# SayanoAI/Comfy-RVC

Measured on AMD Instinct MI355X. Metric: audio-sec/wall-sec (xRT), 40k_v2 end-to-end VC, higher is better.
Workload: dtype f32; 1 GPU; Full VC 40k_v2 (HuBERT -> RMVPE -> SynthesizerTrnMs768NSFsid), 30 s 16 kHz clips, 12 per GPU per step (3 in flight), vc_single host array in -> int16 host array out (BASELINE.json configs[2]); clips_in_flight_per_gpu=3, weights=procedural (comfy-rvc_amd/synthetic.py), noise=device generator, seeded per clip, parallelism=clip-per-GPU x1 (3 lanes each), one RCCL gather of the step's int16 waveforms

## Files before the change

comfy-rvc_amd/_lib.py:

```python
import ctypes as C
import os

_HERE = os.path.dirname(os.path.abspath(__file__))
LIB_PATH = os.environ.get("RVC_HIP_LIB") or os.path.join(_HERE, "csrc", "librvc_hip.so")


class RvcHipError(RuntimeError):
    pass


def _load():
    if not os.path.isfile(LIB_PATH):
        raise RvcHipError(
            f"{LIB_PATH} is missing: build it with `python -c 'import __graft_entry__ as g; g.build()'` "
            "(or `make -C comfy-rvc_amd/csrc`).  There is no CPU fallback.")
    return C.CDLL(LIB_PATH)


lib = _load()

c_void_p, c_int, c_int64, c_float, c_char_p = C.c_void_p, C.c_int, C.c_int64, C.c_float, C.c_char_p
P = C.POINTER


# ... 147 lines not shown
    "rvc_synth_infer_window_halo": (c_int, [c_void_p, c_void_p, c_void_p, c_int, c_void_p, c_void_p, c_int, c_void_p, c_void_p, c_int64,
                                            c_void_p, P(SynthTaps), c_int64, c_int64, c_int]),
    "rvc_vc_segment_window": (c_int, [c_void_p, c_void_p, c_void_p, c_void_p, c_int64, c_int, c_void_p, c_void_p, c_int, c_float, c_int,
                                      c_void_p, c_void_p, c_void_p, c_int64, c_int64]),
    "rvc_vc_segment_feats_window": (c_int, [c_void_p, c_void_p, c_void_p, c_void_p, c_int64, c_int, c_void_p, c_void_p, c_int, c_float, c_int, c_void_p,
                                            c_void_p, c_void_p, c_int64, c_int64]),
    "rvc_vc_segment": (c_int, [c_void_p, c_void_p, c_void_p, c_void_p, c_int64, c_int, c_void_p, c_void_p, c_int, c_float, c_int,
                               c_void_p, c_void_p, c_void_p]),
    "rvc_vc_segment_feats": (c_int, [c_void_p, c_void_p, c_void_p, c_void_p, c_int64, c_int, c_void_p, c_void_p, c_int, c_float, c_int, c_void_p,
                                     c_void_p, c_void_p]),
    "rvc_index_create": (c_int, [c_void_p, c_void_p, c_int64, c_int, P(c_void_p)]),
    "rvc_index_create_ivf": (c_int, [c_void_p, c_void_p, c_int64, c_int, c_void_p, c_int, c_void_p, c_int, P(c_void_p)]),
    "rvc_index_nprobe": (c_int, [c_void_p]),
    "rvc_index_destroy": (c_int, [c_void_p]),
    "rvc_index_ntotal": (c_int64, [c_void_p]),
    "rvc_index_search": (c_int, [c_void_p, c_void_p, c_void_p, c_int64, c_void_p, c_void_p]),
    "rvc_index_blend": (c_int, [c_void_p, c_void_p, c_void_p, c_void_p, c_int64, c_float, c_void_p]),
    "rvc_kmeans_assign": (c_int, [c_void_p, c_void_p, c_void_p, c_int64, c_int, c_void_p, c_int, c_void_p, c_void_p]),
    "rvc_kmeans_update": (c_int, [c_void_p, c_void_p, c_void_p, c_int64, c_int, c_int, c_void_p, c_void_p]),
    "rvc_index_train": (c_int, [c_void_p, c_void_p, c_void_p, c_int64, c_int, c_void_p, c_int, c_int, c_void_p, c_void_p, c_void_p]),
    "rvc_preprocess": (c_int, [c_void_p, c_void_p, c_int, c_int64, c_void_p, c_void_p, c_void_p, c_int, c_void_p, c_void_p,
                             c_void_p, c_int, c_void_p, c_void_p]),
    "rvc_postprocess": (c_int, [c_void_p, c_void_p, c_int64, c_void_p, c_int, c_int, c_float, c_void_p]),
    "rvc_lfilter_hp": (c_int, [c_void_p, c_void_p, c_int, c_int64, c_void_p, c_void_p]),
    "rvc_frame_rms": (c_int, [c_void_p, c_void_p, c_int64, c_int, c_int, c_void_p, c_int64]),
    "rvc_slice_tags": (c_int, [c_void_p, c_int64, c_int64, C.c_double, c_int64, c_int64, c_int64, c_void_p, c_int64, P(c_int64)]),
    "rvc_cut_windows": (c_int, [c_void_p, c_void_p, c_int64, c_void_p, c_int, c_int, c_int, c_void_p, c_int, c_int, c_int, c_float, c_void_p, c_int64,
                                c_void_p, c_int64]),
    "rvc_gate_levels": (c_int, [c_void_p, c_void_p, c_int64, c_int, c_void_p, c_int64]),
    "rvc_gate_ranges": (c_int, [c_void_p, c_int64, c_int64, c_int64, c_int64, c_int64, C.c_double, c_void_p, c_int64, P(c_int64)]),
    "rvc_gate_apply": (c_int, [c_void_p, c_void_p, c_void_p, c_int64, c_void_p, c_int, c_int64]),
    "rvc_declick": (c_int, [c_void_p, c_void_p, c_int64, c_int, c_float, c_int, c_int, c_int, c_void_p, c_void_p]),
    "rvc_peak_normalize": (c_int, [c_void_p, c_void_p, c_int64, c_float, c_void_p]),
    "rvc_peak_limit": (c_int, [c_void_p, c_void_p, c_int64, c_float]),
    "rvc_merge_tracks": (c_int, [c_void_p, P(c_void_p), P(c_int64), c_int, c_int, c_void_p, c_int64]),
    "rvc_segment_energy": (c_int, [c_void_p, c_void_p, c_int64, c_int, c_void_p]),
    "rvc_spectrogram_batch": (c_int, [c_void_p, c_void_p, c_void_p, c_int64, c_void_p, c_int, c_int, c_int, c_float, c_int, c_void_p, c_int64]),
    "rvc_mel_filterbank_set": (c_int, [c_void_p, c_int, c_int, c_void_p, c_void_p, c_void_p]),
    "rvc_spec_to_mel_batch": (c_int, [c_void_p, c_void_p, c_void_p, c_int64, c_void_p, c_int, c_int, c_int, c_void_p, c_int64]),
    "rvc_spectrogram_batch_ms": (c_int, [c_void_p, c_void_p, c_void_p, c_int64, c_void_p, c_int, c_int, c_int, c_float, c_int, c_void_p, c_int64]),
    "rvc_mel_spectrogram_vjp": (c_int, [c_void_p, c_void_p, c_void_p, c_int64, c_void_p, c_int, c_int, c_int, c_float, c_int, c_int, c_void_p, c_int64,
                                        c_void_p]),
    "rvc_mel_spectrogram_vjp_launch_count": (c_int, []),
    "rvc_mel_loss_cotangents": (c_int, [c_void_p, c_int, P(c_void_p), P(c_void_p), P(c_int64), c_int, c_float, c_float, P(c_float), P(c_void_p)]),
    "rvc_multiscale_mel_loss": (c_int, [c_void_p, c_void_p, c_int, P(c_void_p), P(c_int64), P(c_int64), c_int, c_int64, P(C.c_int32), P(C.c_int32), c_int, c_int,
                                        c_void_p]),
    "rvc_hpss": (c_int, [c_void_p, c_void_p, c_int, c_int, c_int, c_void_p, c_void_p, c_int]),
    "rvc_hpss_l1": (c_int, [c_void_p, c_void_p, c_void_p, c_int, c_int, c_int, c_float, c_void_p]),
    "rvc_tsi_terms": (c_int, [c_void_p, c_void_p, c_void_p, c_int, c_int, c_int, c_float, c_void_p]),
    "rvc_op_gemm_split": (c_int, [c_void_p] * 7 + [c_int] * 4 + [c_float, c_int, c_float] + [c_int] * 5),
    "rvc_op_conv2d_split": (c_int, [c_void_p] * 7 + [c_int] * 9),
    "rvc_op_wn_in_gate_split": (c_int, [c_void_p] * 6 + [c_int] * 4),
    "rvc_op_gemm_split_qkv": (c_int, [c_void_p] * 6 + [c_int] * 4),
    "rvc_op_conv1d_s2_split": (c_int, [c_void_p] * 6 + [c_int] * 5),
    "rvc_op_conv1d_split": (c_int, [c_void_p] * 6 + [c_int] * 9),
    "rvc_op_conv1d": (c_int, [c_void_p, c_void_p, c_void_p, c_void_p, c_void_p, c_void_p] + [c_int] * 8 +
                      [c_int, c_float, c_int, c_float, c_int, c_float, c_int]),
    "rvc_op_conv_transpose1d": (c_int, [c_void_p, c_void_p, c_void_p, c_void_p, c_void_p] + [c_int] * 6 + [c_int, c_float, c_int]),
    "rvc_op_conv2d3x3": (c_int, [c_void_p, c_void_p, c_void_p, c_void_p, c_void_p, c_void_p] + [c_int] * 5),
    "rvc_op_conv_transpose2d": (c_int, [c_void_p, c_void_p, c_void_p, c_void_p, c_void_p] + [c_int] * 5),
    "rvc_op_gemm_tn": (c_int, [c_void_p, c_void_p, c_void_p, c_void_p] + [c_int] * 4),
    "rvc_conv1d_plan_create": (c_int, [c_void_p, c_void_p] + [c_int] * 7 + [P(c_void_p)]),
    "rvc_conv1d_plan_run": (c_int, [c_void_p, c_void_p, c_void_p, c_int, c_void_p, c_void_p, c_int, c_float, c_int, c_float]),
    "rvc_conv1d_plan_pair_run": (c_int, [c_void_p, c_void_p, c_void_p, c_void_p, c_int, c_void_p, c_float, c_int]),
    "rvc_conv1d_plan_resblock_run": (c_int, [P(c_void_p), c_void_p, c_void_p, c_int, c_void_p, c_float, c_int, P(c_int), c_void_p, c_void_p, c_void_p]),
    "rvc_conv1d_plan_pair_split_run": (c_int, [c_void_p, c_void_p, c_void_p, c_void_p, c_int, c_void_p, c_float, c_int]),
    "rvc_conv1d_plan_destroy": (c_int, [c_void_p]),
    "rvc_op_attention": (c_int, [c_void_p, c_void_p, c_void_p, c_void_p, c_void_p, c_void_p, c_int, c_int]),
    "rvc_op_attention_split": (c_int, [c_void_p] * 7 + [c_int, c_int]),
    "rvc_op_attention_split_rel": (c_int, [c_void_p] * 9 + [c_int, c_int, c_int]),
    "rvc_op_cbr2_small": (c_int, [c_void_p] * 7 + [c_int, c_int, c_int]),
    "rvc_op_layernorm_c_split": (c_int, [c_void_p] * 6 + [c_int, c_int]),
    "rvc_op_conv3_small": (c_int, [c_void_p] * 7 + [c_int] * 6),
    "rvc_op_gemm_split_swapped": (c_int, [c_void_p] * 4 + [c_int] * 5),
    "rvc_op_conv2d3x3_plus_1x1": (c_int, [c_void_p] * 7 + [c_int] * 6),
    "rvc_op_gemm_split_swapped_res": (c_int, [c_void_p] * 5 + [c_int] * 5),
    "rvc_op_attention_rel": (c_int, [c_void_p] * 8 + [c_int, c_int, c_void_p, c_void_p]),
    "rvc_op_layernorm_c": (c_int, [c_void_p] * 6 + [c_int, c_int]),
    "rvc_resample": (c_int, [c_void_p, c_void_p, c_int64, c_void_p, c_int, c_int, c_int, c_void_p, c_int64]),
    "rvc_set_conv_precision": (c_int, [c_int]),
    "rvc_set_pair_arithmetic": (c_int, [c_int]),
    "rvc_get_pair_arithmetic": (c_int, []),
    "rvc_conv1d_plan_pair_arithmetic": (c_int, [c_void_p, c_void_p, c_int]),
    "rvc_prof_dump_csv": (c_int, [c_char_p]),
    "rvc_prof_enable": (c_int, [c_int]),
    "rvc_prof_collect": (c_int, [P(C.c_double), P(C.c_double), P(c_int64)]),
    "rvc_prof_collect_ex": (c_int, [P(C.c_double), C.c_double, C.c_double]),
    "rvc_prof_cfg_name": (c_char_p, [c_int]),
    "rvc_op_disc_conv": (c_int, [c_void_p] * 5 + [c_int] * 8 + [c_float, P(c_int)]),
    "rvc_op_disc_conv_plan": (c_int, [c_int] * 8 + [P(c_int)]),
    "rvc_op_disc_conv_input_grad": (c_int, [c_void_p] * 6 + [c_int] * 7 + [c_float, P(c_int)]),
    "rvc_op_disc_conv_input_grad_plan": (c_int, [c_int] * 7 + [P(c_int)]),
    "rvc_op_disc_conv_weight_grad": (c_int, [c_void_p] * 4 + [c_int] * 8 + [P(c_int)]),
    "rvc_op_disc_conv_weight_grad_plan": (c_int, [c_int] * 8 + [P(c_int)]),
    "rvc_op_conv1d_input_grad": (c_int, [c_void_p] * 6 + [c_int] * 6 + [c_int64] * 4 + [c_float, c_float, c_int, P(c_int), P(c_int)]),
    "rvc_op_conv1d_input_grad_plan": (c_int, [c_int] * 6 + [c_int64, c_int64, P(c_int)]),
    "rvc_op_sine_source": (c_int, [c_void_p] * 5 + [c_int, c_int, c_float, c_float, c_float] + [c_void_p] * 3),
    "rvc_op_hubert_conv0": (c_int, [c_void_p, c_void_p, c_int64, c_void_p, c_void_p, c_void_p, c_int, c_int, c_void_p, c_void_p, c_int64]),
    "rvc_op_conv_to1": (c_int, [c_void_p, c_void_p, c_int64, c_void_p, c_int, c_int, c_int, c_int, c_float, c_int, c_void_p, P(c_int)]),
    "rvc_op_noise_add": (c_int, [c_void_p, c_void_p, c_int64, c_int, c_int, c_void_p, c_int64, c_int, c_int, c_int, c_void_p, c_void_p, P(c_int)]),
    "rvc_op_transpose": (c_int, [c_void_p, c_void_p, c_void_p, c_int, c_int, c_int64, c_int64, c_int, c_int64, c_int64]),
    "rvc_op_frames": (c_int, [c_void_p, c_void_p, c_void_p] + [c_int] * 6),
    "rvc_op_mel_to_unet": (c_int, [c_void_p, c_void_p, c_void_p, c_int, c_int, c_float, c_float]),
    "rvc_op_feats_prepare": (c_int, [c_void_p] * 5 + [c_int, c_int, c_int, c_float, c_int]),
    "rvc_op_wn_gate": (c_int, [c_void_p] * 5 + [c_int, c_int]),
    "rvc_op_pool2_pad": (c_int, [c_void_p, c_void_p, c_int64, c_int, c_int, c_int, c_int, c_void_p, c_void_p, c_int64]),
    "rvc_op_interleave2_pad": (c_int, [c_void_p, c_void_p, c_int64, c_int, c_int, c_int, c_void_p, c_int, c_void_p, c_int64]),
    "rvc_op_pad2d": (c_int, [c_void_p, c_void_p, c_int64, c_int, c_int, c_int, c_void_p, c_void_p, c_int64]),
    "rvc_op_unpad2d": (c_int, [c_void_p, c_void_p, c_int64, c_int, c_int, c_int, c_void_p, c_int64]),
    "rvc_op_gru_scan": (c_int, [c_void_p] * 6 + [c_int, P(c_int)]),
}

EXPERIMENT_SIGNATURES = {
    "rvc_debug_conv_timing": (c_int, [P(C.c_uint64), c_int]),
    "rvc_debug_x3p_check": (c_int, []),
    "rvc_debug_gemm_split_bench": (c_int, [c_void_p] + [c_int] * 8 + [P(c_float), c_int, c_int]),
}

for _name, (_res, _args) in SIGNATURES.items():
    _fn = getattr(lib, _name)
    _fn.restype = _res
    _fn.argtypes = _args
has_experiments = all(hasattr(lib, _n) for _n in EXPERIMENT_SIGNATURES)
if has_experiments:
    for _name, (_res, _args) in EXPERIMENT_SIGNATURES.items():
        _fn = getattr(lib, _name)
        _fn.restype = _res
        _fn.argtypes = _args


def require_experiments():
    if not has_experiments:
        raise RuntimeError(f"{LIB_PATH} is the product library: the rvc_debug_* hooks exist in -DRVC_EXPERIMENTS builds only - "
                           "bash tools/build_variant.sh exp && RVC_HIP_LIB=comfy-rvc_amd/csrc/variants/librvc_hip_exp.so python <tool>")


def check(status):
    if status != 0:
        raise RvcHipError(lib.rvc_last_error().decode("utf-8", "replace"))


def ptr(t):
    if t is None:
        return None
    if hasattr(t, "data_ptr"):
        return c_void_p(t.data_ptr())
    return c_void_p(t.ctypes.data)


class _DeviceSpan:

    def __init__(self, address, shape):
        self.__cuda_array_interface__ = {"shape": tuple(int(v) for v in shape), "typestr": "<f4", "data": (int(address), False), "version": 2, "strides": None}


def device_view(address, shape, device):
    import torch
    with torch.cuda.device(device):
        return torch.as_tensor(_DeviceSpan(address, shape), device=device).clone()


def current_stream():
    import torch
    return c_void_p(torch.cuda.current_stream().cuda_stream)


# ... 27 lines not shown
```

comfy-rvc_amd/csrc/conv_kernels.h:

```cpp
#pragma once
#include "rvc_internal.h"
#include <hip/hip_ext.h>

namespace rvc {

typedef float f32x16 __attribute__((ext_vector_type(16)));
typedef unsigned int u32x4 __attribute__((ext_vector_type(4)));

struct ConvArgsX : ConvArgs {
  long long ldW;
  int Wcols;
  int Wrows;
  int ksplit; float* partial; long long ldP;
  unsigned magRP, magPW;
  int ni; unsigned magNI;
  const unsigned char* Wx; int CoPx; int xbufs; int NC; int kreal; long long wxBatch;
  const unsigned char* Wx2; const float* bias1; int fuse_p2; float fuse_slope;
  const unsigned char* Xs; long long xsTp;
  unsigned char* Ys; long long ysTp; float ys_slope;
  int wbufs;
  int xcd_remap;
  int h2;
};

__device__ __forceinline__ __amdgpu_buffer_rsrc_t make_rsrc(const void* base, unsigned bytes) {
  return __builtin_amdgcn_make_buffer_rsrc(const_cast<void*>(base), 0, (int)bytes, 0x00020000);
}
constexpr unsigned kOOB = 0x80000000u;
__device__ __forceinline__ float buf_load(__amdgpu_buffer_rsrc_t r, unsigned voff, unsigned soff = 0) {
  return __uint_as_float(__builtin_amdgcn_raw_buffer_load_b32(r, (int)voff, (int)soff, 0));
}
__device__ __forceinline__ void buf_dma(__amdgpu_buffer_rsrc_t rs, unsigned char* lds_dst, int voffset, int soffset) {
  __builtin_amdgcn_raw_ptr_buffer_load_lds(rs, (__attribute__((address_space(3))) void*)lds_dst, 16, voffset, soffset, 0, 0);
}

template <int WM, int WN, int AM, int AN, int G, bool HAS_R, bool HAS_ACC>
__device__ __forceinline__ void dense_epilogue_t(const ConvArgsX& p, f32x16 (&acc)[AM][AN], int z, int co0, int n0, int wm, int wn, int li, int lh) {
  const float* __restrict__ bias = p.bias ? p.bias + (long long)z * p.bBatch : nullptr;
  const float* R = HAS_R ? p.R + (long long)z * p.rBatch : nullptr;
  float* Y = p.Y + (long long)z * p.yBatch;
  const float lslope = p.act == ACT_NONE ? 1.f : (p.act == ACT_RELU ? 0.f : p.act_slope);
  const float oscale = p.out_scale;
  const bool plain = p.orows == p.Co;
  const __amdgpu_buffer_rsrc_t yrs = make_rsrc(Y, (unsigned)p.orows * (unsigned)p.ldY * 4u);
  const __amdgpu_buffer_rsrc_t rrs = make_rsrc(HAS_R ? R : Y, HAS_R ? (unsigned)p.orows * (unsigned)p.ldR * 4u : 0u);
  const bool abr = p.act_before_res != 0;
  constexpr bool need_loads = HAS_R || HAS_ACC;
  auto row_info = [&](int am, int r, bool& mok, float& bv, unsigned& yrow, unsigned& rrow) {
    const int m = co0 + (wm * AM + am) * 32 + (r & 3) + 8 * (r >> 2) + 4 * lh;
    mok = m < p.Co;
    const int co = plain ? m : m % p.orows;
    bv = (bias && mok) ? bias[co] : 0.f;
    yrow = (unsigned)co * (unsigned)p.ldY; rrow = (unsigned)co * (unsigned)p.ldR;
  };
  static_assert(16 % G == 0, "group size");
#pragma unroll
  for (int am = 0; am < AM; ++am) {
    float rv[G][AN], yv[G][AN], rvn[G][AN], yvn[G][AN];
#pragma unroll
    for (int j = 0; j < G; ++j)
#pragma unroll
      for (int an = 0; an < AN; ++an) { rv[j][an] = 0.f; yv[j][an] = 0.f; rvn[j][an] = 0.f; yvn[j][an] = 0.f; }
    auto load_group = [&](int r0, float (&rr)[G][AN], float (&yy)[G][AN]) {
#pragma unroll
      for (int j = 0; j < G; ++j) {
        bool mok; float bv; unsigned yrow, rrow;
        row_info(am, r0 + j, mok, bv, yrow, rrow);
#pragma unroll
        for (int an = 0; an < AN; ++an) {
          const int n = n0 + (wn * AN + an) * 32 + li;
          const bool ok = mok && n < p.Tout;
          if constexpr (HAS_R) rr[j][an] = buf_load(rrs, ok ? (rrow + (unsigned)n) * 4u : kOOB);
          if constexpr (HAS_ACC) yy[j][an] = buf_load(yrs, ok ? (yrow + (unsigned)n) * 4u : kOOB);
        }
      }
    };
    if constexpr (need_loads) load_group(0, rv, yv);
#pragma unroll
    for (int r0 = 0; r0 < 16; r0 += G) {
      if constexpr (need_loads) { if (r0 + G < 16) load_group(r0 + G, rvn, yvn); }
#pragma unroll
      for (int j = 0; j < G; ++j) {
        bool mok; float bv; unsigned yrow, rrow;
        row_info(am, r0 + j, mok, bv, yrow, rrow);
#pragma unroll
        for (int an = 0; an < AN; ++an) {
          const int n = n0 + (wn * AN + an) * 32 + li;
          const bool ok = mok && n < p.Tout;
          float v = acc[am][an][r0 + j] + bv;
          if (abr) v = fmaxf(v, v * lslope) + rv[j][an];
          else { v += rv[j][an]; v = fmaxf(v, v * lslope); }
          v = v * oscale + yv[j][an];
          __builtin_amdgcn_raw_buffer_store_b32(__float_as_uint(v), yrs, (int)(ok ? (yrow + (unsigned)n) * 4u : kOOB), 0, 0);
        }
      }
#pragma unroll
      for (int j = 0; j < G; ++j)
#pragma unroll
        for (int an = 0; an < AN; ++an) { rv[j][an] = rvn[j][an]; yv[j][an] = yvn[j][an]; }
    }
  }
}
template <int WM, int WN, int AM, int AN, int G = 1>
__device__ __forceinline__ void dense_epilogue(const ConvArgsX& p, f32x16 (&acc)[AM][AN], int z, int co0, int n0, int wm, int wn, int li, int lh) {
  const bool has_r = p.R != nullptr, has_acc = p.accumulate != 0;
  if (has_r && has_acc) dense_epilogue_t<WM, WN, AM, AN, G, true, true>(p, acc, z, co0, n0, wm, wn, li, lh);
  else if (has_r) dense_epilogue_t<WM, WN, AM, AN, (AM * AN >= 8 ? 2 * G : G) <= 16 ? (AM * AN >= 8 ? 2 * G : G) : 16, true, false>(p, acc, z, co0, n0, wm, wn, li, lh);
  else if (has_acc) dense_epilogue_t<WM, WN, AM, AN, G, false, true>(p, acc, z, co0, n0, wm, wn, li, lh);
  else dense_epilogue_t<WM, WN, AM, AN, G, false, false>(p, acc, z, co0, n0, wm, wn, li, lh);
}

struct TileCfg { int WM, WN, AM, AN; };
TileCfg choose_tile(int M, long long N, int batch);
int tile_cfg_id(const TileCfg& t);

constexpr int kProfCfgs = 24;
struct ProfTicket { hipEvent_t a = nullptr, b = nullptr; bool on = false; };
ProfTicket conv_prof_begin(hipStream_t s);
struct ProfKernelEvents { hipEvent_t ka = nullptr, kb = nullptr; bool armed = false; int launches = 0; };
ProfKernelEvents& prof_kernel_events();
template <class K, class A>
inline void conv_launch(K kern, dim3 grid, dim3 block, size_t lds, hipStream_t s, const A& a) {
  ProfKernelEvents& pe = prof_kernel_events();
  if (pe.armed && pe.launches++ == 0) hipExtLaunchKernelGGL(kern, grid, block, lds, s, pe.ka, pe.kb, 0, a);
  else hipLaunchKernelGGL(kern, grid, block, lds, s, a);
}
void conv_prof_end(ProfTicket& t, hipStream_t s, double flops, int cfg, double bytes = 0.0, const ConvArgsX* shape = nullptr, long long blocks = 0,
                   int fused = 0);
int conv_prof_dump_csv(const char* path);
double conv_alg_bytes(const ConvArgsX& a, int batch);
int conv_prof_collect_ex(double* out , double ridge_fp32, double ridge_x3);

void splitk_reduce_launch(const ConvArgsX& a, int S, int batch, hipStream_t s);

int device_cu_count();
inline int x3_xcd_remap() { static const int v = exp_int("RVC_X3_XCD", 1); return v; }
typedef void (*ConvLaunchFn)(const ConvArgsX&, dim3, size_t, hipStream_t);
struct ConvPlan {
  ConvArgsX a;
  long long plan_T = 0;
  ConvLaunchFn launch = nullptr;
  dim3 grid; size_t lds = 0;
  int prof_cfg = 0, prof_fused = 0;
  double alg_bytes = 0.0, flops = 0.0;
};
bool conv_x3_plan(const ConvArgsX& a0, int batch, long long Tplan, ConvPlan& p);
void conv_plan_launch(const ConvPlan& p, hipStream_t s);
bool conv_x3p_plan(ConvPlan& p, int AM, int AN);
int conv_x3p_check_read();
bool conv_x3q_plan(ConvPlan& p, int AM, int AN);
bool conv_x3g_plan(ConvPlan& p);
bool conv_x3pf_plan(ConvPlan& p);
bool conv_rbh_plan(ConvPlan& p);
bool conv_x3_pair_plan(const ConvLayer& c1, const ConvLayer& c2, const float* X, long long ldX, int T, long long Tplan, float* Y, long long ldY,
                       const ConvEpilogue& e2, int h2, ConvPlan& p);

struct Rb3Args {
  const float* X; long long ldX; float* Y; long long ldY;
  const unsigned char* W[6];
  const float* B[6];
  int CoPx;
  int T, halo, NO;
  float pre_slope, mid_slope, out_scale;
  const float* nsrc; const float* nw; const float* nb;
};
struct Rb3Plan {
  Rb3Args a; void (*launch)(const Rb3Args&, dim3, size_t, hipStream_t) = nullptr; dim3 grid; size_t lds = 0;
  int C = 0, k = 0, accumulate = 0;
};
bool conv_rb3_plan(const ConvLayer* const* c1, const ConvLayer* const* c2, const float* X, long long ldX, int T, long long Tplan, float* Y, long long ldY,
                   float pre_slope, float out_scale, int accumulate, int h2, const float* nsrc, const float* nw, const float* nb, Rb3Plan& p);
void conv_rb3_launch(const Rb3Plan& p, hipStream_t s);

}
```

comfy-rvc_amd/csrc/conv_mfma.hip:

```cpp
#include "conv_kernels.h"
#include "phase_timing.h"
#include <atomic>
#include <tuple>

#ifndef RVC_EPI_TWOPHASE
#define RVC_EPI_TWOPHASE 0
#endif

namespace rvc {

RVC_PHASE_TABLE_REGISTER;

constexpr int kWSlots = 32;
__host__ __device__ constexpr int x_slots(int BN, int MODE) {
  return MODE == 2 ? (BN >= 512 ? 26 : (BN >= 256 ? 18 : 14)) : (BN >= 512 ? 36 : (BN >= 256 ? 20 : (BN >= 128 ? 32 : 16)));
}

template <int WM, int WN, int AM, int AN, int MODE>
__global__ __launch_bounds__(256) void conv_mfma_kernel(const ConvArgsX p) {
  constexpr int BM = WM * AM * 32, BN = WN * AN * 32;
  constexpr int XS = x_slots(BN, MODE);
  extern __shared__ __attribute__((aligned(16))) float smem[];
  const int CK = p.CK, WROW = p.WROW;
  float* Xs = smem;
// ... 271 lines not shown
  int blocks = (int)((n + 255) / 256); if (blocks > 8192) blocks = 8192;
  hipLaunchKernelGGL(act_res_kernel, dim3(blocks), dim3(256), 0, s, y, r, rows, T, ldY, ldR, act, slope, act_before_res);
}

__global__ void splitk_reduce_kernel(const float* __restrict__ P, int S, int batch, int M, int N, long long ldP, const float* __restrict__ bias, int bBatch,
                                     const float* __restrict__ R, long long ldR, long long rBatch, float* __restrict__ Y, long long ldY, long long yBatch,
                                     int orows, float lslope, int abr, float oscale, int accumulate) {
  const long long total = (long long)batch * M * N;
  long long i = (long long)blockIdx.x * blockDim.x + threadIdx.x;
  const long long st = (long long)gridDim.x * blockDim.x;
  for (; i < total; i += st) {
    const int n = (int)(i % N); const long long t = i / N; const int m = (int)(t % M); const int z = (int)(t / M);
    float v = 0.f;
    for (int k = 0; k < S; ++k) v += P[(((long long)z * S + k) * M + m) * ldP + n];
    const int co = m % orows;
    if (bias) v += bias[(long long)z * bBatch + co];
    const float rv = R ? R[(long long)z * rBatch + (long long)co * ldR + n] : 0.f;
    if (abr) v = fmaxf(v, v * lslope) + rv; else { v += rv; v = fmaxf(v, v * lslope); }
    const long long o = (long long)z * yBatch + (long long)co * ldY + n;
    v *= oscale;
    if (accumulate) v += Y[o];
    Y[o] = v;
  }
}

void splitk_reduce_launch(const ConvArgsX& a, int S, int batch, hipStream_t s) {
  const long long total = (long long)batch * a.Co * a.Tout;
  int blocks = (int)((total + 255) / 256); if (blocks > 4096) blocks = 4096;
  const float lslope = a.act == ACT_NONE ? 1.f : (a.act == ACT_RELU ? 0.f : a.act_slope);
  { ProfKernelEvents& pe = prof_kernel_events(); if (pe.armed) ++pe.launches; }
  hipLaunchKernelGGL(splitk_reduce_kernel, dim3(blocks), dim3(256), 0, s, a.partial, S, batch, a.Co, a.Tout, a.ldP, a.bias, a.bBatch, a.R, a.ldR,
                     a.rBatch, a.Y, a.ldY, a.yBatch, a.orows, lslope, a.act_before_res, a.out_scale, a.accumulate);
}

std::vector<PhaseTableReader>& phase_table_readers() { static std::vector<PhaseTableReader> v; return v; }
void conv_timing_read(unsigned long long* out8, bool reset) {
  for (int i = 0; i < 8; ++i) out8[i] = 0;
  for (PhaseTableReader read : phase_table_readers()) {
    unsigned long long t[8]; read(t, reset);
    for (int i = 0; i < 8; ++i) out8[i] += t[i];
  }
}
void* dev_alloc(size_t bytes) {
  void* d = nullptr;
  RVC_HIP_CHECK(hipMalloc(&d, bytes));
  return d;
}
void* dev_upload(const void* host, size_t bytes) {
  void* d = dev_alloc(bytes ? bytes : sizeof(float));
  if (bytes) {
    const hipError_t e = hipMemcpy(d, host, bytes, hipMemcpyHostToDevice);
    if (e != hipSuccess) { dev_free(d); RVC_HIP_CHECK(e); }
  }
  return d;
}
void dev_free(void* p) { if (p) (void)hipFree(p); }

namespace {
struct ScratchBuf { void* p = nullptr; size_t cap = 0; };
using ScratchKey = std::tuple<int, hipStream_t, int>;
std::map<ScratchKey, ScratchBuf>& scratch_pool() { static std::map<ScratchKey, ScratchBuf> pool; return pool; }
std::mutex& scratch_mu() { static std::mutex mu; return mu; }
struct Scratch { void* p; bool grew; };
Scratch scratch_get(hipStream_t s, int slot, size_t bytes, size_t grow_to) {
  int dev = 0;
  RVC_HIP_CHECK(hipGetDevice(&dev));
  ScratchBuf* b;
  { std::lock_guard<std::mutex> lk(scratch_mu()); b = &scratch_pool()[ScratchKey{dev, s, slot}]; }
  if (bytes <= b->cap) return {b->p, false};
  RVC_HIP_CHECK(hipStreamSynchronize(s));
  if (b->p) (void)hipFree(b->p);
  b->p = nullptr; b->cap = 0;
  RVC_HIP_CHECK(hipMalloc(&b->p, grow_to));
  b->cap = grow_to;
  return {b->p, true};
}
}
void* stream_scratch(hipStream_t s, int slot, size_t bytes) { return scratch_get(s, slot, bytes, bytes + bytes / 4 + (1 << 20)).p; }
void* stream_scratch_zeroed(hipStream_t s, int slot, size_t bytes, bool* fresh) {
  const Scratch r = scratch_get(s, slot, bytes, bytes);
  if (r.grew) RVC_HIP_CHECK(hipMemsetAsync(r.p, 0, bytes, s));
  if (fresh) *fresh = r.grew;
  return r.p;
}
void stream_scratch_release(int device) {
  std::lock_guard<std::mutex> lk(scratch_mu());
  auto& pool = scratch_pool();
  for (auto it = pool.begin(); it != pool.end();) {
    if (std::get<0>(it->first) == device) { if (it->second.p) (void)hipFree(it->second.p); it = pool.erase(it); } else ++it;
  }
}

void Arena::ensure(size_t bytes) {
  if (bytes <= cap) return;
  if (base) { RVC_HIP_CHECK(hipDeviceSynchronize()); (void)hipFree(base); base = nullptr; cap = 0; }
  size_t want = bytes + bytes / 8 + (1 << 20);
  RVC_HIP_CHECK(hipMalloc(&base, want));
  cap = want; ++gen;
}
void Arena::release() { if (base) (void)hipFree(base); base = nullptr; cap = 0; ++gen; }

static int pick_ck(int V, int ktaps, int stride) {
  int ck = ktaps >= 4 ? 8 : (ktaps >= 2 ? 16 : 64);
  if (stride > 1) { ck = ((ck + stride - 1) / stride) * stride; if (ck & 1) ck *= 2; }
  if (V < ck) { ck = stride > 1 ? ((V + stride - 1) / stride) * stride : V; if (ck & 1) ck += (stride > 1 ? stride : 1); if (ck < 2) ck = 2; }
  return ck;
}

static void upload_layer(ConvLayer& L, const std::vector<float>& packed, const float* bias, int nbias) {
  L.Wd_ = dev_upload(packed.data(), packed.size());
  L.bd_ = bias ? dev_upload(bias, nbias) : nullptr;
}

static uint16_t bf16_rne(float f) {
  uint32_t u; memcpy(&u, &f, 4);
  if ((u & 0x7fffffffu) > 0x7f800000u) return (uint16_t)((u >> 16) | 0x40);
  return (uint16_t)((u + 0x7fffu + ((u >> 16) & 1u)) >> 16);
}
static float bf16_to_f32(uint16_t h) { uint32_t u = (uint32_t)h << 16; float f; memcpy(&f, &u, 4); return f; }
static thread_local bool g_x3_default = false;
static thread_local int g_precision = 1;
bool conv_x3_set_default(bool on) { const bool prev = g_x3_default; g_x3_default = on; return prev; }
int conv_set_precision(int mode) { const int prev = g_precision; if (mode >= 0) g_precision = mode; return prev; }
static void pack_x3_grouped(ConvLayer& L, const float* w , int groups, int Cog, int Cig, int k) {
  L.CoPx = (Cog + 63) & ~63;
  const int nch = Cig / 16;
  L.wxBatch = (long long)nch * k * 2 * L.CoPx * 16;
  std::vector<uint16_t> P((size_t)groups * L.wxBatch, 0);
  for (int g = 0; g < groups; ++g)
    for (int co = 0; co < Cog; ++co)
      for (int ci = 0; ci < Cig; ++ci)
        for (int u = 0; u < k; ++u) {
          const float v = w[((size_t)(g * Cog + co) * Cig + ci) * k + u];
          const uint16_t hi = bf16_rne(v), lo = bf16_rne(v - bf16_to_f32(hi));
          const int chunk = ci >> 4, c16 = ci & 15;
          const size_t base = (((size_t)chunk * k + u) * 2 * 2 + (size_t)(c16 >> 3)) * L.CoPx + co;
          uint16_t* Q = P.data() + (size_t)g * L.wxBatch;
          Q[base * 8 + (c16 & 7)] = hi;
          Q[(base + 2 * (size_t)L.CoPx) * 8 + (c16 & 7)] = lo;
        }
  RVC_HIP_CHECK(hipMalloc(&L.Wx_, P.size() * sizeof(uint16_t)));
  RVC_HIP_CHECK(hipMemcpy(L.Wx_, P.data(), P.size() * sizeof(uint16_t), hipMemcpyHostToDevice));
}
void x3_weight_image(const float* w, int Co, int Ci, int k, int CoPx, std::vector<uint16_t>& P) {
  P.assign((size_t)(Ci / 16) * k * 2 * CoPx * 16, 0);
  for (int co = 0; co < Co; ++co)
    for (int ci = 0; ci < Ci; ++ci)
      for (int u = 0; u < k; ++u) {
        const float v = w[((size_t)co * Ci + ci) * k + u];
        const uint16_t hi = bf16_rne(v), lo = bf16_rne(v - bf16_to_f32(hi));
        const int chunk = ci >> 4, c16 = ci & 15;
        const size_t base = (((size_t)chunk * k + u) * 2 * 2 + (size_t)(c16 >> 3)) * CoPx + co;
        P[base * 8 + (c16 & 7)] = hi;
        P[(base + 2 * (size_t)CoPx) * 8 + (c16 & 7)] = lo;
      }
}
static void pack_x3(ConvLayer& L, const float* w, int Co, int Ci, int k) {
  L.CoPx = (Co + 127) & ~127;
  const int nch = Ci / 16;
  L.wxBatch = (long long)nch * k * 2 * L.CoPx * 16;
  std::vector<uint16_t> P;
  x3_weight_image(w, Co, Ci, k, L.CoPx, P);
  RVC_HIP_CHECK(hipMalloc(&L.Wx_, P.size() * sizeof(uint16_t)));
  RVC_HIP_CHECK(hipMemcpy(L.Wx_, P.data(), P.size() * sizeof(uint16_t), hipMemcpyHostToDevice));
}

// ... 389 lines not shown
      const long long total = (long long)batch * a.Co * a.Tout;
      (void)total;
      splitk_reduce_launch(a, S, batch, s);
    }
    conv_prof_end(rec, s, flops, cfg_id, conv_alg_bytes(a, batch), &a, (long long)grid.x * grid.y * grid.z);
  };
#define RVC_LAUNCH(ID_, WM_, WN_, AM_, AN_)                                                     \
  if (t.WM == WM_ && t.WN == WN_ && t.AM == AM_ && t.AN == AN_) {                               \
    cfg_id = ID_ + (mode == 2 ? 7 : 0);                                                         \
    rec = conv_prof_begin(s);                                                                   \
    if (mode == 2) launch_cfg<WM_, WN_, AM_, AN_, 2>(a, grid, lds, s);                          \
    else if (a.stride > 1) launch_cfg<WM_, WN_, AM_, AN_, 3>(a, grid, lds, s);                  \
    else launch_cfg<WM_, WN_, AM_, AN_, 1>(a, grid, lds, s);                                    \
    finish();                                                                                   \
    return;                                                                                     \
  }
  RVC_LAUNCH(0, 1, 4, 1, 4)
  RVC_LAUNCH(1, 1, 4, 1, 2)
  RVC_LAUNCH(2, 1, 4, 1, 1)
  RVC_LAUNCH(3, 2, 2, 2, 2)
  RVC_LAUNCH(4, 2, 2, 1, 4)
  RVC_LAUNCH(5, 2, 2, 1, 2)
  RVC_LAUNCH(6, 2, 2, 1, 1)
#undef RVC_LAUNCH
  throw Error("no tile configuration matched");
}

static bool simple_act(int act) { return act == ACT_NONE || act == ACT_LRELU || act == ACT_RELU; }
static ConvEpilogue split_epilogue(const ConvEpilogue& e, bool& post) {
  post = !simple_act(e.act);
  if (!post) return e;
  RVC_REQUIRE(e.out_scale == 1.f && !e.accumulate, "GELU/tanh/sigmoid/log epilogues do not combine with scale/accumulate");
  ConvEpilogue c = e;
  c.act = ACT_NONE; c.act_slope = 0.f; c.R = nullptr; c.ldR = 0;
  return c;
}
static void fill_epilogue(ConvArgsX& a, const ConvEpilogue& e) {
  a.R = e.R; a.ldR = e.ldR; a.pre_act = e.pre_act; a.pre_slope = e.pre_slope; a.act = e.act; a.act_slope = e.act_slope;
  a.act_before_res = e.act_before_res; a.out_scale = e.out_scale; a.accumulate = e.accumulate;
  a.Xs = e.xs_in; a.xsTp = e.xs_tp; a.Ys = e.ys_out; a.ysTp = e.ys_tp; a.ys_slope = e.ys_slope;
}

int conv1d_out_len(const ConvLayer& L, int Tin) {
  if (L.tconv_u > 0) return (Tin - 1) * L.tconv_u - 2 * L.pad + L.k;
  return (Tin + 2 * L.pad - L.dil * (L.k - 1) - 1) / L.stride + 1;
}

void conv1d_run(const ConvLayer& L, hipStream_t s, const float* X, long long ldX, int Tin, float* Y, long long ldY,
                const ConvEpilogue& e0) {
  RVC_REQUIRE(L.mode == 1 && L.Wd_, "conv1d_run on an uninitialised / non-1D layer");
  bool post; const ConvEpilogue e = split_epilogue(e0, post);
  ConvArgsX a{};
  a.X = X; a.W = L.Wd_; a.bias = L.bd_; a.Y = Y;
  fill_epilogue(a, e);
  a.Ci = L.Ci; a.Co = L.Co; a.CoP = L.CoP; a.Tin = Tin; a.Wd = 0; a.ktaps = L.ktaps; a.dil = L.dil; a.stride = L.stride;
  a.CK = L.CK; a.nchunk = L.nchunk;
  a.ldX = ldX; a.ldY = ldY; a.up2 = 0;
  a.ldW = L.CoP; a.Wcols = L.CoP; a.Wrows = L.nchunk * L.ktaps * L.CK;
  if (e.bias_override) a.bias = e.bias_override;
  int Tout = conv1d_out_len(L, Tin);
  if (e.tout_limit > 0 && e.tout_limit < Tout) { RVC_REQUIRE(L.tconv_u == 0, "tout_limit on a transposed conv"); Tout = e.tout_limit; }
  auto gemm_cols = [&](int tout) { return L.tconv_u > 0 ? (tout + L.tconv_u - 1) / L.tconv_u : tout; };
  a.Tout = gemm_cols(Tout);
  RVC_REQUIRE(e.plan_tin == 0 || (e.plan_tin >= Tin && !e.tout_limit), "plan_tin is the input length of the whole sequence this launch is a column window of");
  const long long Tplan = e.plan_tin > 0 ? gemm_cols(conv1d_out_len(L, e.plan_tin)) : a.Tout;
  if (L.tconv_u > 0) {
    a.pad = L.conv_pad;
    a.ostride = L.tconv_u; a.orows = L.co_real;
    RVC_REQUIRE(ldY == Tout, "interleaved ConvTranspose1d store needs a dense output (ldY == Tout)");
    RVC_REQUIRE(e.R == nullptr, "residual not supported on the interleaved store");
  } else {
    a.pad = L.pad; a.ostride = 1; a.orows = L.Co;
  }
  a.xBatch = (long long)L.Ci * ldX; a.wBatch = L.wBatch; a.yBatch = (long long)L.Co * ldY; a.rBatch = (long long)L.Co * e.ldR;
  a.bBatch = L.Co;
  const double flops = L.tconv_u > 0 ? 2.0 * Tin * L.Ci * L.co_real * L.k
                                     : 2.0 * L.groups * (double)L.Co * a.Tout * L.Ci * L.k;
  a.Wx = reinterpret_cast<const unsigned char*>(L.Wx_); a.CoPx = L.CoPx; a.wxBatch = L.wxBatch; a.kreal = L.tconv_u > 0 ? L.ktaps : L.k;
  if (e.h2) {
    RVC_REQUIRE(L.Wh_ && (e.xs_in || e.ys_out), "fp16x2 arithmetic is for the two halves of a split-resident ResBlock pair (conv1d_pair_h2_eligible)");
    a.Wx = reinterpret_cast<const unsigned char*>(L.Wh_); a.h2 = 1;
  }
  ConvPlan p;
  if (L.Wx_ && conv_x3_plan(a, L.groups, Tplan, p)) { p.flops = flops; conv_plan_launch(p, s); }
  else {
    RVC_REQUIRE(!e.xs_in && !e.ys_out, "split-resident tensors need the bf16x3 kernel (check conv1d_split_eligible first)");
    run_conv(a, 1, L.groups, Tplan, s, flops);
  }
  if (post) {
    RVC_REQUIRE(L.tconv_u == 0, "post-activation on a transposed conv");
    act_res_inplace(s, Y, e0.R, L.groups * L.Co, Tout, ldY, e0.ldR, e0.act, e0.act_slope, e0.act_before_res);
  }
}

bool conv1d_pair_h2_eligible(const ConvLayer& c1, const ConvLayer& c2, int Tin, int h2) {
  if (!h2 || !c1.Wh_ || !c2.Wh_) return false;
  return conv1d_split_eligible(c1, Tin, SPLIT_PRODUCER, 1) && conv1d_split_eligible(c2, Tin, SPLIT_CONSUMER, 1);
}

static bool plan_split_role(const ConvLayer& L, int Tin, SplitRole role, int h2, ConvPlan& p) {
  if (L.mode != 1 || !L.Wx_ || (h2 && !L.Wh_) || L.tconv_u || L.stride != 1 || L.groups != 1 || (L.Co & 31) || (L.Ci & 15)) return false;
  if (conv1d_out_len(L, Tin) != Tin || L.pad > kSplitMargin) return false;
  ConvArgsX a{};
  a.Ci = L.Ci; a.Co = L.Co; a.CoP = L.CoP; a.Tin = Tin; a.Wd = 0; a.ktaps = L.ktaps; a.dil = L.dil; a.stride = 1; a.pad = L.pad;
  a.Tout = conv1d_out_len(L, Tin); a.ostride = 1; a.orows = L.Co; a.ldX = Tin; a.ldY = a.Tout; a.ldR = a.Tout;
  a.Wx = reinterpret_cast<const unsigned char*>(L.Wx_); a.CoPx = L.CoPx; a.kreal = L.k; a.h2 = h2;
  if (role == SPLIT_CONSUMER) a.R = reinterpret_cast<const float*>(L.Wx_);
  if (role == SPLIT_PRODUCER) { a.Ys = reinterpret_cast<unsigned char*>(L.Wx_); a.ysTp = split_image_tp(Tin); a.pre_act = ACT_LRELU; a.pre_slope = 0.1f; }
  else { a.Xs = reinterpret_cast<const unsigned char*>(L.Wx_); a.xsTp = split_image_tp(Tin); }
  return conv_x3_plan(a, 1, a.Tout, p);
}
bool conv1d_split_eligible(const ConvLayer& L, int Tin, SplitRole role, int h2) { ConvPlan p; return plan_split_role(L, Tin, role, h2, p); }

int conv1d_residual_period(const ConvLayer& L, int Tin, int h2) {
  ConvPlan p;
  if (!plan_split_role(L, Tin, SPLIT_CONSUMER, h2, p) || (p.prof_fused >> 4) != 6) return 1;
  const int id = p.prof_cfg - 14;
  return id == 3 ? 128 : 256;
}

void gemm_tn_run(hipStream_t s, const float* A, long long ldA, long long aBatch, const float* B, long long ldB, long long bBatch,
                 float* Y, long long ldY, long long yBatch, int M, int N, int K, int batch, const float* bias, int biasBatch,
                 const ConvEpilogue& e) {
  RVC_REQUIRE(simple_act(e.act), "gemm_tn_run supports identity / ReLU / leaky ReLU epilogues");
  ConvArgsX a{};
  a.X = B; a.W = A; a.bias = bias; a.Y = Y;
  fill_epilogue(a, e);
  a.Ci = K; a.Co = M; a.CoP = M; a.Tin = N; a.Tout = N; a.Wd = 0; a.ktaps = 1; a.dil = 1; a.stride = 1; a.pad = 0;
  a.CK = K >= 64 ? 64 : ((K + 1) & ~1); a.nchunk = (K + a.CK - 1) / a.CK;
  a.ldX = ldB; a.ldY = ldY; a.up2 = 0; a.ostride = 1; a.orows = M;
  a.ldW = ldA; a.Wcols = M; a.Wrows = K;
  a.xBatch = bBatch; a.wBatch = aBatch; a.yBatch = yBatch; a.rBatch = 0; a.bBatch = biasBatch;
  run_conv(a, 1, batch, N, s, 2.0 * M * (double)N * K * batch);
}

void conv2d_run(const ConvLayer& L, hipStream_t s, const float* X, long long ldX, int H, int Wd, float* Y, long long ldY,
                const ConvEpilogue& e) {
  RVC_REQUIRE(simple_act(e.act), "conv2d_run supports identity / ReLU / leaky ReLU epilogues");
  RVC_REQUIRE(L.mode == 2 && L.Wd_, "conv2d_run on an uninitialised / non-2D layer");
  RVC_REQUIRE((Wd & (Wd - 1)) == 0 && Wd >= 2, "width must be a power of two");
  ConvArgsX a{};
  a.X = X; a.W = L.Wd_; a.bias = L.bd_; a.Y = Y;
  fill_epilogue(a, e);
  a.Ci = L.Ci; a.Co = L.Co; a.CoP = L.CoP; a.Tin = H; a.Tout = H * Wd; a.Wd = Wd; a.ktaps = 9; a.dil = 1; a.stride = 1; a.pad = 1;
  a.CK = L.CK; a.nchunk = L.nchunk;
  a.ldX = ldX; a.ldY = ldY; a.up2 = L.up2; a.ostride = 1; a.orows = L.up2 ? L.co_real : L.Co;
  a.ldW = L.CoP; a.Wcols = L.CoP; a.Wrows = L.nchunk * 9 * L.CK;
  a.xBatch = 0; a.wBatch = 0; a.yBatch = 0; a.rBatch = 0; a.bBatch = 0;
  const double flops = 2.0 * H * (double)Wd * 9 * L.Ci * (L.up2 ? L.co_real : L.Co);
  a.Wx = reinterpret_cast<const unsigned char*>(L.Wx_); a.CoPx = L.CoPx; a.wxBatch = L.wxBatch; a.kreal = 9;
  if (L.up2 && L.Wx_ && !e.R && !e.accumulate) {
    ConvArgsX d = a;
    float* tmp = (float*)stream_scratch(s, 4, (size_t)L.Co * H * Wd * sizeof(float));
    d.Y = tmp; d.ldY = (long long)H * Wd; d.up2 = 0; d.orows = L.Co; d.bias = L.bd4_;
    ConvPlan p;
    if (conv_x3_plan(d, 1, d.Tout, p)) {
      p.flops = flops; conv_plan_launch(p, s);
      const long long n = (long long)L.Co * H * Wd;
      int blocks = (int)((n + 255) / 256); if (blocks > 8192) blocks = 8192;
      hipLaunchKernelGGL(interleave2x2_kernel, dim3(blocks), dim3(256), 0, s, tmp, Y, L.co_real, H, Wd);
      return;
    }
  }
  ConvPlan p;
  if (L.Wx_ && !L.up2 && conv_x3_plan(a, 1, a.Tout, p)) { p.flops = flops; conv_plan_launch(p, s); }
  else run_conv(a, 2, 1, a.Tout, s, flops);
}

}
```

comfy-rvc_amd/csrc/conv_x3.hip:

```cpp
#include "conv_x3_dev.h"

#ifndef RVC_X3_SCHED
#define RVC_X3_SCHED 0
#endif

namespace rvc {

RVC_PHASE_TABLE_REGISTER;

template <int WM, int WN, int AM, int AN, bool FUSE = false, bool XSPLIT = false, bool YSPLIT = false>
__global__ __launch_bounds__(WM * WN * 64, WM * WN == 8 ? 1 : ((WM == 2 && WN == 2 && AM == 2 && AN == 2 && !FUSE) ? 3 : 2)) void conv_x3_kernel(const ConvArgsX p) {
  constexpr int NW = WM * WN, NT = NW * 64;
  constexpr int BM = WM * AM * 32, BN = WN * AN * 32, XS = XSPLIT ? 1 : ((FUSE && BM == 64) ? 7 : (FUSE ? 5 : x3_slots(BN, NW))), RB = BM / 32;
  extern __shared__ __attribute__((aligned(1024))) unsigned char smem3[];
  const int P = p.WROW;
  const int NC = p.NC;
  const int st = p.stride;
  const int Pm = XSPLIT ? ((P + 63) & ~63) : (P + st - 1) / st;
  const int xplane = st * Pm * 32;
  const int xhalf = xplane >> 1;
  const int xbuf = NC * 2 * xplane;
  const int wbuf = NC * p.KT * 2 * BM * 32;
  unsigned char* Xs = smem3;
  unsigned char* Ws = smem3 + ((p.xbufs * xbuf + 1023) & ~1023);
// ... 324 lines not shown
    const __amdgpu_buffer_rsrc_t prs = make_rsrc(Pp, (unsigned)p.Co * (unsigned)p.ldP * 4u);
#pragma unroll
    for (int am = 0; am < AM; ++am)
#pragma unroll
      for (int r = 0; r < 16; ++r) {
        const int m = co0 + (wm * AM + am) * 32 + (r & 3) + 8 * (r >> 2) + 4 * lh;
#pragma unroll
        for (int an = 0; an < AN; ++an) {
          const int n = n0 + (wn * AN + an) * 32 + li;
          const bool ok = m < p.Co && n < p.Tout;
          __builtin_amdgcn_raw_buffer_store_b32(__float_as_uint(acc[am][an][r]), prs, (int)(ok ? ((unsigned)m * (unsigned)p.ldP + (unsigned)n) * 4u : kOOB), 0, 0);
        }
      }
  } else if (YSPLIT) {
    ysplit_epilogue<WM, WN, AM, AN>(p, acc, co0, n0, wm, wn, li, lh);
  } else if (p.ostride == 1) {
    if constexpr (FUSE) {
      ConvArgsX pe = p;
      pe.Tout = min(p.Tout, n0 + BN - 2 * P2);
      dense_epilogue<WM, WN, AM, AN, (AM * AN >= 8 ? 4 : 8)>(pe, acc, z, co0, n0, wm, wn, li, lh);
    } else {
      dense_epilogue<WM, WN, AM, AN, (AM * AN >= 8 ? (AN >= 8 ? 2 : 4) : (XSPLIT ? 4 : 8))>(p, acc, z, co0, n0, wm, wn, li, lh);
    }
  } else {
    const float* __restrict__ bias = p.bias;
    float* Y = p.Y;
    const float lslope = p.act == ACT_NONE ? 1.f : (p.act == ACT_RELU ? 0.f : p.act_slope);
#pragma unroll
    for (int am = 0; am < AM; ++am) {
#pragma unroll
      for (int r = 0; r < 16; ++r) {
        const int m = co0 + (wm * AM + am) * 32 + (r & 3) + 8 * (r >> 2) + 4 * lh;
        if (m >= p.Co) continue;
        const int co = m / p.ostride, ph = m - co * p.ostride;
        const float bv = bias ? bias[co] : 0.f;
#pragma unroll
        for (int an = 0; an < AN; ++an) {
          const int n = n0 + (wn * AN + an) * 32 + li;
          const long long to = (long long)n * p.ostride + ph;
          if (n >= p.Tout || to >= p.ldY) continue;
          const long long oidx = (long long)co * p.ldY + to;
          float v = acc[am][an][r] + bv;
          v = fmaxf(v, v * lslope) * p.out_scale;
          if (p.accumulate) v += Y[oidx];
          Y[oidx] = v;
        }
      }
    }
  }
  tm.lap(5); tm.add(0, 1); tm.flush();
}

template <int WM, int WN, int AM, int AN, bool FUSE = false, bool XSPLIT = false, bool YSPLIT = false>
static void launch_x3(const ConvArgsX& a, dim3 grid, size_t lds, hipStream_t s) {
  auto kern = conv_x3_kernel<WM, WN, AM, AN, FUSE, XSPLIT, YSPLIT>;
  RVC_ALLOW_BIG_LDS(kern);
  conv_launch(kern, grid, dim3(WM * WN * 64), lds, s, a);
}

template <int AM, int AN>
static ConvLaunchFn select_x3_io(const ConvArgsX& a) {
  if (a.Xs) return &launch_x3<2, 2, AM, AN, false, true>;
  if (a.Ys) return &launch_x3<2, 2, AM, AN, false, false, true>;
  return &launch_x3<2, 2, AM, AN>;
}
static ConvLaunchFn select_x3(const ConvArgsX& a, int id) {
  switch (id) {
    case 0: return &launch_x3<1, 4, 1, 4>;
    case 1: return &launch_x3<1, 4, 1, 2>;
    case 2: return &launch_x3<1, 4, 1, 1>;
    case 3: return select_x3_io<2, 2>(a);
    case 4: return select_x3_io<1, 4>(a);
    case 5: return &launch_x3<2, 2, 1, 2>;
    case 7: return select_x3_io<2, 4>(a);
    default: return &launch_x3<2, 2, 1, 1>;
  }
}

void conv_plan_launch(const ConvPlan& p, hipStream_t s) {
  ConvArgsX a = p.a;
  if (a.Xs) RVC_REQUIRE(a.xsTp >= split_image_tp(a.Tin), "split-resident input image is shorter than split_image_tp(T)");
  if (a.Ys) RVC_REQUIRE(a.ysTp >= split_image_tp(a.Tout), "split-resident output image is shorter than split_image_tp(T)");
  if (a.ksplit > 1) a.partial = (float*)stream_scratch(s, 0, (size_t)a.ksplit * a.Co * a.ldP * sizeof(float));
  ProfTicket tk = conv_prof_begin(s);
  p.launch(a, p.grid, p.lds, s);
  if (a.ksplit > 1) splitk_reduce_launch(a, a.ksplit, 1, s);
  conv_prof_end(tk, s, p.flops, p.prof_cfg, p.alg_bytes, &a, (long long)p.grid.x * p.grid.y * p.grid.z, p.prof_fused);
}

bool conv_x3_plan(const ConvArgsX& a0, int batch, long long Tplan, ConvPlan& p) {
  if (!a0.Wx) return false;
  const bool xs = a0.Xs != nullptr;
  if ((xs || a0.Ys) && (a0.Wd > 0 || a0.stride != 1 || a0.ostride != 1 || (a0.Co & 31) || batch != 1)) return false;
  if (xs && a0.pre_act != ACT_NONE) return false;
  if ((xs || a0.Ys) && (a0.pad > kSplitMargin || a0.Tout != a0.Tin)) return false;
  const int KH2 = a0.KW > 0 ? a0.KH : 3, KW2 = a0.KW > 0 ? a0.KW : 3;
  if (a0.Wd > 0 && (a0.ktaps != KH2 * KW2 || a0.stride != 1)) return false;
  if ((a0.stride != 1 && a0.dil != 1) || a0.up2 || (a0.ostride != 1 && a0.R) || (a0.Ci & 15) || batch != 1) return false;
  if (!(a0.act == ACT_NONE || a0.act == ACT_LRELU || a0.act == ACT_RELU) || !(a0.pre_act == ACT_NONE || a0.pre_act == ACT_LRELU)) return false;
  if ((double)a0.orows * (double)a0.ldY * 4.0 >= 2147483648.0 || (double)a0.orows * (double)a0.ldR * 4.0 >= 2147483648.0 ||
      (double)a0.Ci * (double)a0.ldX * 4.0 >= 2147483648.0) return false;
  p = ConvPlan{};
  p.plan_T = Tplan;
  ConvArgsX& a = p.a;
  a = a0;
  if (a.Wd == 0) a.ktaps = a0.kreal;
  auto planned = [&](int cfg, int fused) { p.prof_cfg = cfg; p.prof_fused = fused; p.alg_bytes = conv_alg_bytes(a, batch); return true; };
  if (batch == 1 && a.up2 == 0 && !a.h2) {
    if (conv_x3g_plan(p)) return planned(14 + ((a.Co > 64 && a.Ci * a.ktaps > 1024) ? 3 : 5), 2 << 4);
  }
  TileCfg t = choose_tile(a.Co, Tplan, batch);
  {
    static const int wide_blk = exp_int("RVC_X3_WIDE", 600);
    auto blocks = [&](int bm, int bn) { return (long long)((a.Co + bm - 1) / bm) * ((Tplan + bn - 1) / bn); };
    if (wide_blk > 0 && a.stride == 1 && a.Wd == 0) {
      static const int wide_xs7 = exp_int("RVC_X3_WIDE_XS7", 1);
      static const int wide_k3 = exp_int("RVC_X3_WIDE_K3", 2);
      if (a.Co > 64 && blocks(128, 256) >= wide_blk && (a.ktaps > 3 || (wide_k3 >= 1 && a.ostride == 1)) &&
          !(xs && a.ktaps <= 7 && !(a.ktaps <= 3 && wide_k3 >= 2) && !(a.ktaps == 7 && wide_xs7))) t = TileCfg{2, 2, 2, 4};
    }
  }
  int id = tile_cfg_id(t);
  if (t.WM == 2 && t.WN == 2 && t.AM == 2 && t.AN == 4) id = 7;
  const int NW = t.WM * t.WN;
  if (id < 0) return false;
  if ((xs || a0.Ys) && !(id == 3 || id == 4 || id == 7)) return false;
  if (xs && a0.Ys) return false;
  const int BM = t.WM * t.AM * 32, BN = t.WN * t.AN * 32;
  const long long nblk = ((Tplan + BN - 1) / BN) * ((a.Co + BM - 1) / BM);
  static const int min_blk = exp_int("RVC_X3_MINBLK", 250);
  static const int min_blk2d = exp_int("RVC_X3_MINBLK2D", 20);
  if (nblk < (a.Wd > 0 ? min_blk2d : min_blk)) return false;
  if (t.WM == 2 && t.WN == 2 && batch == 1) {
    const bool s2_up = a.stride == 2 && a.ktaps == 3 && a.Co >= 128 && !(t.AM == 2 && t.AN == 2) &&
                       (long long)((a.Co + 127) / 128) * ((Tplan + 127) / 128) >= 150;
    const int pam = s2_up ? 2 : t.AM, pan = s2_up ? 2 : t.AN;
    if (!s2_up && conv_x3q_plan(p, t.AM, t.AN)) return planned(14 + id, 6 << 4);
    if (a.h2) return false;
    if (conv_x3p_plan(p, pam, pan)) return planned(14 + (s2_up ? 3 : id), 1 << 4);
  }
  if (a.h2) return false;
  static const int x3_split_blk = exp_int("RVC_X3_SPLITK_BLK", 600);
  int P = (BN - 1) * a.stride + (a.ktaps - 1) * a.dil + 1;
  if (a.Wd > 0) {
    a.BWd = BN < a.Wd ? BN : a.Wd; a.BH = BN < a.Wd ? 1 : BN / a.Wd; a.PW = a.BWd + KW2 - 1;
    P = (a.BH + KH2 - 1) * a.PW;
    a.magPW = (unsigned)((0x100000000ULL + a.PW - 1) / a.PW);
  }
  const int Pm = xs ? ((P + 63) & ~63) : (P + a.stride - 1) / a.stride;
  a.ni = (P + 63) / 64;
  const int nchunk = a.Ci / 16;
  int NC = a.ktaps == 1 ? 4 : (a.ktaps <= 3 ? 2 : 1);
  while (NC > 1 && (nchunk % NC != 0 || (!xs && (NC * 2 * a.ni + NW - 1) / NW > x3_slots(BN, NW)))) NC >>= 1;
  if (!xs && (NC * 2 * a.ni + NW - 1) / NW > x3_slots(BN, NW)) return false;
  static const int budget_kb = exp_int("RVC_X3_LDS_KB", 53);
  const int budget = budget_kb * 1024;
  static const int wbufs_env = exp_int("RVC_X3_WBUFS", 2);
  int NS = wbufs_env < 2 ? 2 : (wbufs_env > 4 ? 4 : wbufs_env);
  int xbufs = 2, xbytes = 0, ktmax = 0;
  for (;;) {
    const int per_tap = NS * NC * 2 * BM * 32;
    xbufs = 2; xbytes = (xbufs * NC * 2 * a.stride * Pm * 32 + 1023) & ~1023;
    ktmax = (budget - xbytes) / per_tap;
    if (!xs && ktmax < 2 && a.ktaps > ktmax && a.ktaps > 1) { xbufs = 1; xbytes = (NC * 2 * a.stride * Pm * 32 + 1023) & ~1023; ktmax = (budget - xbytes) / per_tap; }
    if (ktmax >= 1) break;
    if (NS > 2) { --NS; continue; }
// ... 87 lines not shown
```

comfy-rvc_amd/csrc/conv_x3q.hip:

```cpp
#include "conv_x3_dev.h"

namespace rvc {

RVC_PHASE_TABLE_REGISTER;
RVC_X3P_CHECK_REGISTER;

struct QTile { int co0, n0, bx; bool edge, valid; };
template <bool SWAP, bool H2 = false>
__device__ __forceinline__ f32x16 q_mfma(const u32x4& w, const u32x4& x, const f32x16& c) {
  if constexpr (H2) return __builtin_amdgcn_mfma_f32_32x32x16_f16(__builtin_bit_cast(f16x8, w), __builtin_bit_cast(f16x8, x), c, 0, 0, 0);
  else if constexpr (SWAP) return __builtin_amdgcn_mfma_f32_32x32x16_bf16(__builtin_bit_cast(bf16x8, x), __builtin_bit_cast(bf16x8, w), c, 0, 0, 0);
  else return __builtin_amdgcn_mfma_f32_32x32x16_bf16(__builtin_bit_cast(bf16x8, w), __builtin_bit_cast(bf16x8, x), c, 0, 0, 0);
}
typedef float f32x4q __attribute__((ext_vector_type(4)));

template <int AM, int AN, int KT, int R, bool XSPLIT, bool YSPLIT, bool RADD, bool H2>
__global__ __launch_bounds__(256, (AM * AN >= 8) ? 2 : 3) void conv_x3q_kernel(const ConvArgsX p) {
  static_assert(!(YSPLIT && RADD), "an image output has no residual");
  static_assert(XSPLIT != YSPLIT, "c1 of a pair (fp32 in, image out) or c2 (image in, fp32 out)");
  constexpr int WM = 2, WN = 2, NW = 4;
  constexpr int BM = WM * AM * 32, BN = WN * AN * 32, RB = BM / 32;
  constexpr int XS = 3;
  constexpr int NPW = H2 ? 1 : 2 * RB / NW;
  constexpr int NPX = (BN + 64) / 64;
  constexpr int wslot = (H2 ? 1 : 2) * BM * 32;
  constexpr int NBLK = AM * AN;
  constexpr int TR = KT / 2;
  static_assert(KT >= XS && (RB == 2 || RB == 4), "geometry");
  struct Q {
    static constexpr int nA(int t) { return XSPLIT ? 0 : 8 * x3_cv(t, KT, XS); }
    static constexpr int nD(int t) { return (XSPLIT && tap_mod(t, KT) == KT - 1) ? NPX : 0; }
    static constexpr int nE(int t) { return (RADD && tap_mod(t, KT) == TR) ? 16 : 0; }
    static constexpr int tot(int t) { return nA(t) + NPW + nD(t) + nE(t); }
    static constexpr int sum() { int n = 0; for (int t = 0; t < KT; ++t) n += tot(t); return n; }
    static constexpr int w(int t) { int n = nD(t - (R - 2)) + nE(t - (R - 2)); for (int j = 1; j <= R - 3; ++j) n += tot(t - (R - 2) + j); return n + nA(t); }
  };
  constexpr int EP = (YSPLIT || RADD) ? 4 * AM * AN : 16 * AM * AN;

  extern __shared__ __attribute__((aligned(1024))) unsigned char smemq[];
  const int P = p.WROW;
  const int Pm = (P + 7) & ~7;
  const int xplane = Pm * 32, xhalf = xplane >> 1, xbuf = 2 * xplane;
  unsigned char* Xs = smemq;
  unsigned char* Ws = smemq + ((2 * xbuf + 1023) & ~1023);
  float* Bs = reinterpret_cast<float*>(Ws + R * wslot);
  unsigned char* Ss = reinterpret_cast<unsigned char*>(Bs) + ((p.Co * 4 + 255) & ~255);

  const int tid0 = threadIdx.x;
  int lane = tid0 & 63;
  const int wave = __builtin_amdgcn_readfirstlane(tid0 >> 6);
  const int wm = wave / WN, wn = wave % WN;
  const int li = lane & 31, lh = lane >> 5;
  const int nck = p.nchunk;
  const int ni = p.ni;
  const int dil16 = p.dil * 16;
  const float pre_slope = p.pre_act == ACT_LRELU ? p.pre_slope : 1.f;
  const __amdgpu_buffer_rsrc_t xrs = make_rsrc(p.X, XSPLIT ? 0u : (unsigned)p.Ci * (unsigned)p.ldX * 4u);
  const __amdgpu_buffer_rsrc_t rrs = make_rsrc(RADD ? (const void*)p.R : (const void*)p.Y, RADD ? (unsigned)p.Co * (unsigned)p.ldR * 4u : 0u);

  const unsigned nty = (unsigned)(p.Co / BM), ntiles = (unsigned)((p.Tout + BN - 1) / BN) * nty;
  auto geom = [&](int it) -> QTile {
    const unsigned L = blockIdx.x + (unsigned)it * gridDim.x;
    QTile t;
    t.valid = L < ntiles;
    const unsigned tile = !t.valid ? 0u : (p.xcd_remap ? xcd_tile(L, ntiles) : L);
    const int tx = (int)(tile / nty), ty = (int)(tile - (unsigned)tx * nty);
    t.co0 = ty * BM; t.n0 = tx * BN; t.bx = t.n0 - p.pad;
    t.edge = XSPLIT && (t.bx < 0 || t.bx + P > p.Tin);
    return t;
  };
  const int nit = (int)((ntiles - blockIdx.x + gridDim.x - 1) / gridDim.x);

  PhaseTimer<PhaseClock::cycle> tm;
#ifdef RVC_X3P_CHECK
  int issued = 0, mk_w[8] = {0, 0, 0, 0, 0, 0, 0, 0}, mk_x[XS] = {0, 0, 0}, mk_r = 0, uwc = 0, mk_xs[2] = {0, 0};
#endif

  for (int m = tid0; m < p.Co; m += NW * 64) Bs[m] = p.bias ? p.bias[m] : 0.f;

  const int NU = nck * KT;
  const unsigned wstep = (unsigned)p.CoPx * (H2 ? 32u : 64u);
  const __amdgpu_buffer_rsrc_t wrs = make_rsrc(p.Wx, (unsigned)NU * wstep);
  const int wrow_h2 = RB == 4 ? wave * 64 + lane : wave * 32 + (lane & 31);
  const int wvoff = H2 ? ((wrow_h2 / BM) * p.CoPx + (wrow_h2 % BM)) * 16
                       : ((wave / RB) * p.CoPx * 32) + (((((wave % RB) * 64 + lane) / BM) * p.CoPx + (((wave % RB) * 64 + lane) % BM)) * 16);
  QTile cur = geom(0), nxt = geom(1);
  unsigned wsoff = (unsigned)cur.co0 * 16u;
  int slw = 0, uw = 0;
  int wtile_co0_next = nxt.valid ? nxt.co0 : cur.co0;
  auto issue_w = [&]() {
    if constexpr (H2) {
      unsigned char* dst = Ws + slw * wslot + wave * (RB == 4 ? 1024 : 512);
      if (RB == 4 || lane < 32)
        buf_dma(wrs, dst, wvoff, (int)wsoff);
    } else {
      unsigned char* dst = Ws + slw * wslot + wave * 1024;
      buf_dma(wrs, dst, wvoff, (int)wsoff);
      if constexpr (RB == 4)
        buf_dma(wrs, dst + NW * 1024, wvoff, (int)(wsoff + (unsigned)p.CoPx * 32u));
    }
    ++uw;
    if (uw == NU) { uw = 0; wsoff = (unsigned)wtile_co0_next * 16u; } else wsoff += wstep;
    slw = slw + 1 == R ? 0 : slw + 1;
    X3P_ISSUED(NPW);
#ifdef RVC_X3P_CHECK
    mk_w[uwc & 7] = issued; ++uwc;
#endif
  };

  float xr[XS][8];
  auto slot_geom = [&](int s, int& hb, int& q) -> bool {
    const int t = wave + NW * s;
    hb = t >= ni ? 1 : 0;
    q = (t - hb * ni) * 64 + lane;
    return t < 2 * ni && q < P;
  };
  auto load_slot = [&](int s, const QTile& tl, int chunk) {
    int hb, q;
    const bool ok = slot_geom(s, hb, q) && tl.valid;
    const int x = tl.bx + q;
    const unsigned voff = (ok && x >= 0 && x < p.Tin) ? (unsigned)x * 4u : kOOB;
    const unsigned c0 = (unsigned)(chunk * 16 + hb * 8);
#pragma unroll
    for (int j = 0; j < 8; ++j) xr[s][j] = buf_load(xrs, voff, (c0 + j) * (unsigned)p.ldX * 4u);
    X3P_ISSUED(8);
#ifdef RVC_X3P_CHECK
    mk_x[s] = issued;
#endif
  };
  auto store_slot = [&](int s, int xb) {
    int hb, q;
    if (slot_geom(s, hb, q)) {
      u32x4 hi, lo;
#pragma unroll
      for (int j = 0; j < 4; ++j) {
        const float a = xr[s][2 * j], b = xr[s][2 * j + 1];
        unsigned h_, l_;
        if constexpr (H2) split2h(fmaxf(a, a * pre_slope), fmaxf(b, b * pre_slope), h_, l_);
        else split2(fmaxf(a, a * pre_slope), fmaxf(b, b * pre_slope), h_, l_);
        hi[j] = h_; lo[j] = l_;
      }
      unsigned char* d = Xs + xb * xbuf + hb * xhalf + q * 16;
      *reinterpret_cast<u32x4*>(d) = hi;
      *reinterpret_cast<u32x4*>(d + xplane) = lo;
    }
  };
  const __amdgpu_buffer_rsrc_t xsr = make_rsrc(XSPLIT ? (const void*)p.Xs : (const void*)p.Wx, XSPLIT ? (unsigned)((long long)(p.Ci / 16) * 4 * p.xsTp * 16) : 0u);
  auto issue_x = [&](const QTile& tl, int chunk, int xb) {
    constexpr int pph = (BN + 64) / 64;
#pragma unroll
    for (int i = 0; i < NPX; ++i) {
      const int pi = wave + NW * i;
      const int hp = pi / pph, j = pi - hp * pph;
      const unsigned row = (unsigned)((chunk * 4 + hp) * (int)p.xsTp + (tl.bx + kSplitMargin) + j * 64);
      unsigned char* dst = Xs + xb * xbuf + hp * xhalf + j * 1024;
      if (j * 64 + lane < Pm)
        buf_dma(xsr, dst, lane * 16, (int)(row * 16u));
    }
    X3P_ISSUED(NPX);
#ifdef RVC_X3P_CHECK
    mk_xs[xb] = issued;
#endif
  };
  auto zero_edges = [&](const QTile& tl, int xb) {
    for (int q = tid0; q < P; q += NW * 64) {
      const int t = tl.bx + q;
      if (t >= 0 && t < p.Tin) continue;
#pragma unroll
      for (int pl = 0; pl < 2; ++pl) {
        unsigned char* r = Xs + xb * xbuf + pl * xplane + q * 16;
        *reinterpret_cast<u32x4*>(r) = u32x4{0u, 0u, 0u, 0u}; *reinterpret_cast<u32x4*>(r + xhalf) = u32x4{0u, 0u, 0u, 0u};
      }
    }
  };
  float rst[16];
  auto load_res = [&](const QTile& tl, int b) {
    if constexpr (RADD) {
      const int am = b / AN, an = b - am * AN;
      const int n = tl.n0 + (wn * AN + an) * 32 + li;
      const int mb = tl.co0 + (wm * AM + am) * 32 + 4 * lh;
      const unsigned voff = (tl.valid && b < NBLK && n < p.Tout) ? ((unsigned)mb * (unsigned)p.ldR + (unsigned)n) * 4u : kOOB;
#pragma unroll
      for (int r = 0; r < 16; ++r) rst[r] = buf_load(rrs, voff, (unsigned)((r & 3) + 8 * (r >> 2)) * (unsigned)p.ldR * 4u);
      X3P_ISSUED(16);
#ifdef RVC_X3P_CHECK
      mk_r = issued;
#endif
    }
  };

  const int aoff = lh * (BM * 16) + ((wm * AM) * 32 + li) * 16;
  const int boff = lh * xhalf + ((wn * AN) * 32 + li) * 16;

  if constexpr (XSPLIT) {
    issue_x(cur, 0, 0);
    issue_x(cur, 1, 1);
  } else {
#pragma unroll
    for (int s = 0; s < XS; ++s) load_slot(s, cur, 0);
    wait_vmcnt<0>();
#pragma unroll
    for (int s = 0; s < XS; ++s) store_slot(s, 0);
#pragma unroll
    for (int s = 0; s < XS; ++s) load_slot(s, cur, 1);
  }
#pragma unroll
  for (int i = 0; i < R - 1; ++i) issue_w();
  load_res(cur, 0);
  wait_vmcnt<0>();
#pragma unroll
  for (int s = 0; s < XS; ++s)
#pragma unroll
    for (int j = 0; j < 8; ++j) asm volatile("" : "+v"(xr[s][j]));
  lds_barrier();
  if (XSPLIT && cur.edge) { zero_edges(cur, 0); lds_barrier(); }

  f32x16 acc[AM][AN];
  u32x4 ah[AM], al[AM], bh[AN], bl[AN];
  {
    const unsigned char* wa = Ws + aoff;
    const unsigned char* xa = Xs + boff;
#pragma unroll
    for (int am = 0; am < AM; ++am) ah[am] = *reinterpret_cast<const u32x4*>(wa + am * 512);
#pragma unroll
    for (int an = 0; an < AN; ++an) bl[an] = *reinterpret_cast<const u32x4*>(xa + xplane + an * 512);
  }

  int sl = 0, xb = 0;
  tm.lap(1);
  for (int it = 0; it < nit; ++it) {
#pragma unroll
    for (int am = 0; am < AM; ++am) {
      f32x4q bv[4];
#pragma unroll
      for (int g = 0; g < 4; ++g) bv[g] = RADD ? *reinterpret_cast<const f32x4q*>(Bs + cur.co0 + (wm * AM + am) * 32 + 4 * lh + 8 * g) : f32x4q{0.f, 0.f, 0.f, 0.f};
#pragma unroll
      for (int an = 0; an < AN; ++an)
#pragma unroll
        for (int r = 0; r < 16; ++r) acc[am][an][r] = bv[r >> 2][r & 3];
    }
    for (int c = 0; c < nck; ++c) {
      const bool c0 = c == 0;
      const bool in1 = c + 1 < nck, in2 = c + 2 < nck;
      const QTile& t1 = in1 ? cur : nxt;
      const QTile& t2 = in2 ? cur : nxt;
      const int ch2 = in2 ? c + 2 : c + 2 - nck;
      auto unit = [&](auto tc) {
        constexpr int T = decltype(tc)::value;
        constexpr bool last_tap = T + 1 == KT;
        {
          const unsigned char* xa = Xs + xb * xbuf + T * dil16 + boff;
#pragma unroll
          for (int an = 0; an < AN; ++an) bh[an] = *reinterpret_cast<const u32x4*>(xa + an * 512);
        }
        __builtin_amdgcn_sched_barrier(0);
#pragma unroll
        for (int am = 0; am < AM; ++am)
#pragma unroll
          for (int an = 0; an < AN; ++an)
            acc[am][an] = q_mfma<false, H2>(ah[am], bl[an], acc[am][an]);
        if constexpr (!H2) {
          const unsigned char* wa = Ws + sl * wslot + BM * 32 + aoff;
#pragma unroll
          for (int am = 0; am < AM; ++am) al[am] = *reinterpret_cast<const u32x4*>(wa + am * 512);
        }
        if constexpr (!XSPLIT) {
          auto stage = [&](auto sc) {
            constexpr int s = decltype(sc)::value;
            if constexpr ((s * KT) / XS == T) {
              constexpr int NS = Q::sum() - 8;
              if (c0) { if (it > 0) X3P_CHECK(vm6(NS + EP), issued - mk_x[s]); wait_vmcnt<vm6(NS + EP)>(); }
              else { X3P_CHECK(vm6(NS), issued - mk_x[s]); wait_vmcnt<vm6(NS)>(); }
              store_slot(s, xb ^ 1);
              load_slot(s, t2, ch2);
            }
          };
          static_for<0, XS>(stage);
        }
        __builtin_amdgcn_sched_barrier(0);
#pragma unroll
        for (int am = 0; am < AM; ++am)
#pragma unroll
          for (int an = 0; an < AN; ++an)
            acc[am][an] = q_mfma<false, H2>(ah[am], bh[an], acc[am][an]);
        __builtin_amdgcn_sched_barrier(0);
        {
          constexpr int NWT = Q::w(T);
#ifdef RVC_X3P_CHECK
          const int exact = issued - mk_w[(uwc - (R - 2)) & 7];
#endif
          tm.lap(2);
          if (c0 && T < R - 2) { if (it > 0) X3P_CHECK(vm6(NWT + EP), exact); wait_vmcnt<vm6(NWT + EP)>(); }
          else { X3P_CHECK(vm6(NWT), exact); wait_vmcnt<vm6(NWT)>(); }
          static_assert(!XSPLIT || R - 2 <= KT - 1, "weight ring deeper than a chunk: the input chunk's DMA would not be covered by the weight wait");
          if constexpr (XSPLIT && last_tap) { if (it > 0 || c > 0) X3P_CHECK(vm6(NWT), issued - mk_xs[xb ^ 1]); }
          tm.lap(3);
          lds_barrier();
          tm.lap(4);
          const int sn = sl + 1 == R ? 0 : sl + 1;
          if (XSPLIT && last_tap && t1.edge) { zero_edges(t1, xb ^ 1); lds_barrier(); }
          issue_w();
          if constexpr (XSPLIT && last_tap) issue_x(t2, ch2, xb);
          const unsigned char* wa = Ws + sn * wslot + aoff;
          const unsigned char* xa = Xs + (last_tap ? xb ^ 1 : xb) * xbuf + xplane + (last_tap ? 0 : (T + 1) * dil16) + boff;
#pragma unroll
          for (int am = 0; am < AM; ++am) ah[am] = *reinterpret_cast<const u32x4*>(wa + am * 512);
#pragma unroll
          for (int an = 0; an < AN; ++an) bl[an] = *reinterpret_cast<const u32x4*>(xa + an * 512);
          sl = sn;
        }
        if constexpr (RADD && T == TR) {
          constexpr int NR = Q::sum() - 16;
          if (c0) { if (it > 0) X3P_CHECK(vm6(NR + EP), issued - mk_r); wait_vmcnt<vm6(NR + EP)>(); }
          else { X3P_CHECK(vm6(NR), issued - mk_r); wait_vmcnt<vm6(NR)>(); }
          auto radd = [&](auto bc) {
            constexpr int b = decltype(bc)::value, am = b / AN, an = b % AN;
            f32x16& A = acc[am][an];
            float (&V)[16] = rst;
            const int cc = c;
#define X3Q_ADD8(o)                                                                                                                                   \
            asm volatile("s_cmp_lg_u32 %16, %17\n\ts_cbranch_scc1 .Lx3q_skip_%=\n\ts_nop 15\n\ts_nop 7\n\t"                                                 \
                         "v_add_f32 %0, %0, %8\n\tv_add_f32 %1, %1, %9\n\tv_add_f32 %2, %2, %10\n\tv_add_f32 %3, %3, %11\n\t"                              \
                         "v_add_f32 %4, %4, %12\n\tv_add_f32 %5, %5, %13\n\tv_add_f32 %6, %6, %14\n\tv_add_f32 %7, %7, %15\n\ts_nop 3\n.Lx3q_skip_%=:"      \
                         : "+v"(A[o + 0]), "+v"(A[o + 1]), "+v"(A[o + 2]), "+v"(A[o + 3]), "+v"(A[o + 4]), "+v"(A[o + 5]), "+v"(A[o + 6]), "+v"(A[o + 7])    \
                         : "v"(V[o + 0]), "v"(V[o + 1]), "v"(V[o + 2]), "v"(V[o + 3]), "v"(V[o + 4]), "v"(V[o + 5]), "v"(V[o + 6]), "v"(V[o + 7]),           \
                           "s"(cc), "n"(b) : "scc")
            X3Q_ADD8(0);
            X3Q_ADD8(8);
#undef X3Q_ADD8
          };
          static_for<0, NBLK>(radd);
          load_res(t1, in1 ? c + 1 : 0);
        }
        __builtin_amdgcn_sched_barrier(0);
        if constexpr (!H2) {
#pragma unroll
          for (int am = 0; am < AM; ++am)
#pragma unroll
            for (int an = 0; an < AN; ++an)
              acc[am][an] = q_mfma<false>(al[am], bh[an], acc[am][an]);
        }
      };
      static_for<0, KT>(unit);
      xb ^= 1;
    }

    tm.lap(2);
    if constexpr (YSPLIT) {
      const float sl2 = p.ys_slope;
      const __amdgpu_buffer_rsrc_t ysr = make_rsrc(p.Ys, (unsigned)((long long)(p.Co / 16) * 4 * p.ysTp * 16));
#pragma unroll
      for (int am = 0; am < AM; ++am)
#pragma unroll
        for (int an = 0; an < AN; ++an) {
          const int n = cur.n0 + (wn * AN + an) * 32 + li;
          const int mb = cur.co0 + (wm * AM + am) * 32;
          const long long pos = (long long)n + kSplitMargin;
#pragma unroll
          for (int g2 = 0; g2 < 2; ++g2) {
            const f32x4q ba = *reinterpret_cast<const f32x4q*>(Bs + mb + 16 * g2 + 4 * lh);
            const f32x4q bb = *reinterpret_cast<const f32x4q*>(Bs + mb + 16 * g2 + 4 * lh + 8);
            unsigned hA[2], lA[2], hB[2], lB[2];
#pragma unroll
            for (int e2 = 0; e2 < 2; ++e2) {
              float a0 = acc[am][an][8 * g2 + 2 * e2] + ba[2 * e2], a1 = acc[am][an][8 * g2 + 2 * e2 + 1] + ba[2 * e2 + 1];
              float b0 = acc[am][an][8 * g2 + 4 + 2 * e2] + bb[2 * e2], b1 = acc[am][an][8 * g2 + 5 + 2 * e2] + bb[2 * e2 + 1];
              if constexpr (H2) {
                split2h(fmaxf(a0, a0 * sl2), fmaxf(a1, a1 * sl2), hA[e2], lA[e2]);
                split2h(fmaxf(b0, b0 * sl2), fmaxf(b1, b1 * sl2), hB[e2], lB[e2]);
              } else {
                split2(fmaxf(a0, a0 * sl2), fmaxf(a1, a1 * sl2), hA[e2], lA[e2]);
                split2(fmaxf(b0, b0 * sl2), fmaxf(b1, b1 * sl2), hB[e2], lB[e2]);
              }
            }
            u32x4 hi, lo;
#pragma unroll
            for (int e2 = 0; e2 < 2; ++e2) {
              typedef unsigned u32x2_t __attribute__((ext_vector_type(2)));
              const u32x2_t sh = __builtin_amdgcn_permlane32_swap(hA[e2], hB[e2], false, false);
              const u32x2_t sl3 = __builtin_amdgcn_permlane32_swap(lA[e2], lB[e2], false, false);
              hi[e2] = sh.x; hi[2 + e2] = sh.y; lo[e2] = sl3.x; lo[2 + e2] = sl3.y;
            }
            const long long chunk = (mb >> 4) + g2;
            const unsigned off = n < p.Tout ? (unsigned)(((chunk * 4 + lh) * p.ysTp + pos) * 16) : kOOB;
            __builtin_amdgcn_raw_buffer_store_b128(hi, ysr, (int)off, 0, 0);
            __builtin_amdgcn_raw_buffer_store_b128(lo, ysr, (int)off, (int)(unsigned)(p.ysTp * 32), 0);
          }
        }
      X3P_ISSUED(4 * AM * AN);
    } else if constexpr (RADD) {
      const __amdgpu_buffer_rsrc_t yrs = make_rsrc(p.Y, (unsigned)p.Co * (unsigned)p.ldY * 4u);
      const float oscale = p.out_scale;
      const bool has_acc = p.accumulate != 0;
      float* stg = reinterpret_cast<float*>(Ss + wave * 1024);
      const int rl = lane >> 3, cq = lane & 7;
#pragma unroll
      for (int am = 0; am < AM; ++am)
#pragma unroll
        for (int an = 0; an < AN; ++an) {
          const int n = cur.n0 + (wn * AN + an) * 32 + 4 * cq;
#pragma unroll
          for (int g = 0; g < 4; ++g) {
#pragma unroll
            for (int e = 0; e < 4; ++e) stg[(4 * lh + e) * 32 + li] = acc[am][an][4 * g + e] * oscale;
            const int m = cur.co0 + (wm * AM + am) * 32 + 8 * g + rl;
            const unsigned row = (unsigned)m * (unsigned)p.ldY;
            f32x4q v = *reinterpret_cast<const f32x4q*>(stg + rl * 32 + 4 * cq);
            if (has_acc) {
              const u32x4 y = __builtin_amdgcn_raw_buffer_load_b128(yrs, (int)(n < p.Tout ? (row + (unsigned)n) * 4u : kOOB), 0, 0);
#pragma unroll
              for (int e = 0; e < 4; ++e) v[e] += __uint_as_float(y[e]);
            }
            u32x4 o;
#pragma unroll
            for (int e = 0; e < 4; ++e) o[e] = __float_as_uint(v[e]);
            __builtin_amdgcn_raw_buffer_store_b128(o, yrs, (int)(n + 3 < p.Tout ? (row + (unsigned)n) * 4u : kOOB), 0, 0);
            if (n < p.Tout && n + 3 >= p.Tout) {
#pragma unroll
              for (int e = 0; e < 3; ++e)
                if (n + e < p.Tout) __builtin_amdgcn_raw_buffer_store_b32(o[e], yrs, (int)((row + (unsigned)(n + e)) * 4u), 0, 0);
            }
#ifdef RVC_X3P_CHECK
#pragma unroll
            for (int e = 0; e < 3; ++e) if (__ballot(n < p.Tout && n + 3 >= p.Tout && n + e < p.Tout)) X3P_ISSUED(1);
#endif
          }
        }
      X3P_ISSUED(4 * AM * AN + (p.accumulate ? 4 * AM * AN : 0));
    } else {
      dense_epilogue<WM, WN, AM, AN, 4>(p, acc, 0, cur.co0, cur.n0, wm, wn, li, lh);
      X3P_ISSUED(EP);
    }
    tm.lap(5); tm.add(0, 1);
    cur = nxt; nxt = geom(it + 2);
    wtile_co0_next = nxt.valid ? nxt.co0 : cur.co0;
  }
  wait_vmcnt<0>();
  tm.flush();
}


template <int AM, int AN, int KT, int R, bool XSPLIT, bool YSPLIT, bool RADD, bool H2>
static void launch_x3q(const ConvArgsX& a, dim3 grid, size_t lds, hipStream_t s) {
  auto kern = conv_x3q_kernel<AM, AN, KT, R, XSPLIT, YSPLIT, RADD, H2>;
  RVC_ALLOW_BIG_LDS(kern);
  conv_launch(kern, grid, dim3(256), lds, s, a);
}
template <int AM, int AN, int KT, int R>
static ConvLaunchFn select_x3q_io(const ConvArgsX& a, int mode) {
  constexpr bool c2_ok = R - 2 <= KT - 1;
  if (mode == 0) return a.h2 ? &launch_x3q<AM, AN, KT, R, false, true, false, true> : &launch_x3q<AM, AN, KT, R, false, true, false, false>;
  if constexpr (c2_ok) return a.h2 ? &launch_x3q<AM, AN, KT, R, true, false, true, true> : &launch_x3q<AM, AN, KT, R, true, false, true, false>;
  throw Error("conv_x3q: weight ring deeper than a chunk on an image-in launch");
}
template <int AM, int AN, int R>
static ConvLaunchFn select_x3q_k(const ConvArgsX& a, int mode) {
  if (a.ktaps == 3) return select_x3q_io<AM, AN, 3, R>(a, mode);
  if (a.ktaps == 7) return select_x3q_io<AM, AN, 7, R>(a, mode);
  return select_x3q_io<AM, AN, 11, R>(a, mode);
}
template <int AM, int AN>
static ConvLaunchFn select_x3q_r(const ConvArgsX& a, int R, int mode) {
  if (R >= 5) return select_x3q_k<AM, AN, 5>(a, mode);
  if constexpr (AM == 2 && AN == 4) return select_x3q_k<AM, AN, 4>(a, mode);
  else return R == 4 ? select_x3q_k<AM, AN, 4>(a, mode) : select_x3q_k<AM, AN, 3>(a, mode);
}

bool conv_x3q_plan(ConvPlan& p, int AM, int AN) {
  ConvArgsX& a = p.a;
  const bool xs = a.Xs != nullptr, ys = a.Ys != nullptr;
  if (a.Wd > 0 || (a.Ci & 15) || a.Ci < 48 || xs == ys || a.stride != 1 || a.ostride != 1 || a.orows != a.Co) return false;
  if (!(a.ktaps == 3 || a.ktaps == 7 || a.ktaps == 11)) return false;
  if (!((AM == 2 && AN == 4) || (AM == 1 && AN == 4) || (AM == 2 && AN == 2))) return false;
  const int BM = 64 * AM, BN = 64 * AN;
  if (a.Co % BM || a.Co > 1024) return false;
  if (xs && !(a.R != nullptr && a.act == ACT_NONE)) return false;
  if (ys && (a.R || a.accumulate)) return false;
  if ((double)(a.Co / 16) * 4.0 * (double)a.ysTp * 16.0 >= 2147483648.0 || (double)(a.Ci / 16) * 4.0 * (double)a.xsTp * 16.0 >= 2147483648.0) return false;
  const int mode = ys ? 0 : 1;
  const int P = BN + (a.ktaps - 1) * a.dil;
  if (P > 384 || P > BN + 64) return false;
  const int Pm = (P + 7) & ~7;
  const int xbytes = (2 * 2 * Pm * 32 + 1023) & ~1023;
  const int wslot = (a.h2 ? 1 : 2) * BM * 32;
  const int per_cu = AM * AN >= 8 ? 2 : 3;
  const size_t budget = (size_t)(160 * 1024 / per_cu) & ~(size_t)2047;
  const size_t fixed = (size_t)xbytes + (size_t)((a.Co * 4 + 255) & ~255) + (mode == 1 ? 4096 : 0);
  const int rmin = (AM == 2 && AN == 4) ? 4 : 3;
  int R = (mode == 1 && a.ktaps == 3) ? 4 : 5;
  while (R > rmin && fixed + (size_t)R * wslot > budget) --R;
  const size_t lds = fixed + (size_t)R * wslot;
  if (lds > budget) return false;
  const long long ntiles = (long long)((a.Tout + BN - 1) / BN) * (a.Co / BM);
  const int ncu = device_cu_count();
  static const int wg_env = exp_int("RVC_X3Q_WGS", 0);
  static const int min_rounds = exp_int("RVC_X3Q_MINROUNDS", 0);
  const long long slots = (long long)(wg_env > 0 ? wg_env : per_cu) * ncu;
  const long long ptiles = ((p.plan_T + BN - 1) / BN) * (a.Co / BM);
  if (ptiles < min_rounds * slots || ptiles < 8) return false;
  RVC_REQUIRE(ntiles >= 8, "column window too narrow for the kernel its whole sequence runs on");
  const long long G = ntiles <= slots ? ntiles : (slots & ~7LL);
  if (G < 8) return false;
  a.WROW = P; a.ni = (P + 63) / 64; a.nchunk = a.Ci / 16; a.NC = 1; a.KT = 1; a.xbufs = 2; a.ksplit = 1; a.partial = nullptr; a.wbufs = R;
  a.xcd_remap = x3_xcd_remap();
  p.grid = dim3((unsigned)G, 1, 1);
  p.lds = lds;
  if (AM == 2 && AN == 4) p.launch = select_x3q_r<2, 4>(a, R, mode);
  else if (AM == 1 && AN == 4) p.launch = select_x3q_r<1, 4>(a, R, mode);
  else p.launch = select_x3q_r<2, 2>(a, R, mode);
  return true;
}

}
```

comfy-rvc_amd/csrc/model_synth.hip:

```cpp
#include "model_encoder.h"
#include "models.h"
#include "conv_kernels.h"

namespace rvc {

static OwnedConvLayer make_conv1d(const TensorStore& ts, const std::string& p, int stride, int pad, int dil, bool wn, bool bias = true,
                             float wscale = 1.f, int row0 = 0, int rows = -1, std::vector<float>* keep = nullptr) {
  std::vector<float> w; std::vector<long long> shape;
  if (wn) { const HostTensor& v = ts.get(p + ".weight_v"); w = weight_norm0(v, ts.get(p + ".weight_g")); shape = v.shape; }
  else { const HostTensor& v = ts.get(p + ".weight"); w = v.data; shape = v.shape; }
  RVC_REQUIRE(shape.size() == 3, p + ": expected a [Co][Ci][k] weight");
  int Co = (int)shape[0], Ci = (int)shape[1], k = (int)shape[2];
  std::vector<float> b;
  if (bias) b = ts.get(p + ".bias").data;
  if (rows < 0) rows = Co;
  const size_t per = (size_t)Ci * k;
  std::vector<float> ws(w.begin() + row0 * per, w.begin() + (size_t)(row0 + rows) * per);
  if (wscale != 1.f) for (auto& x : ws) x *= wscale;
  std::vector<float> bs;
  if (bias) { bs.assign(b.begin() + row0, b.begin() + row0 + rows); if (wscale != 1.f) for (auto& x : bs) x *= wscale; }
  OwnedConvLayer L;
  conv1d_layer_init(L, ws.data(), bias ? bs.data() : nullptr, rows, Ci, k, stride, pad, dil, 1);
  if (keep) *keep = std::move(ws);
  return L;
}

struct WNStack {
  int n = 0;
  std::vector<OwnedConvLayer> in, res, skip;
  std::vector<OwnedConvLayer> in_gate;
  std::vector<OwnedConvLayer> rs;
  DevVec cond_w, cond_b;
};
struct FlowLayer {
  OwnedConvLayer pre, post;
  OwnedConvLayer post_neg;
  WNStack wn;
};
struct Posterior {
  bool built = false;
  int spec = 0, Kp = 0;
  OwnedConvLayer pre, proj;
  WNStack wn;
};
struct ResBlock { OwnedConvLayer c1[3], c2[3]; };
struct GenStage { OwnedConvLayer up, noise; DevVec noise_w, noise_b; int u = 1, k = 1, noise_k = 1, noise_s = 1; ResBlock rb[3]; };

struct GenHostWeights { std::vector<float> pre; std::vector<std::vector<float>> up, noise, c1, c2; };
struct GenBwdImages {
  bool built = false;
  DevBuf<uint16_t> pre; std::vector<DevBuf<uint16_t>> up, c1, c2; std::vector<DevVec> noise;
  size_t bytes = 0;
};
struct FlowHostWeights { std::vector<float> pre, post, in[3], rs[3]; };
struct FlowBwdImages { bool built = false; DevBuf<uint16_t> pre[4], post[4], in[4][3], rs[4][3]; size_t bytes = 0; };
struct GenKept { bool on = false; std::vector<DevVec> up_v, up_g, c1_v, c1_g, c2_v, c2_g; size_t bytes = 0; };
struct DecParam { std::string name; std::vector<long long> shape; };
struct SynthWeights {
  DevVec emb_phone_wT, emb_phone_b, emb_pitch, emb_g;
  std::vector<EncoderLayer> enc;
  OwnedConvLayer proj;
  FlowLayer flow[4];
  Posterior post_enc;
  OwnedConvLayer conv_pre;
  DevVec dec_cond_w, dec_cond_b, conv_post_w;
  std::vector<GenStage> stages;
  float lin_w = 1.f, lin_b = 0.f;
  GenHostWeights gen_host; GenBwdImages gen_bwd;
  FlowHostWeights flow_host[4]; FlowBwdImages flow_bwd;
  GenKept kept; std::vector<DecParam> dec_params; std::map<std::string, int> dec_index;
  ZeroedBlock imgs;
};
struct Synth : SynthWeights {
  Ctx* ctx = nullptr;
  Arena arena;
  TensorStore ts;
  bool ready = false;
  int inter = 192, hidden = 192, filt = 768, n_heads = 2, n_layers = 6, ksz = 3, gin = 256, n_spk = 1, sr = 40000, feat_dim = 768;
  int up_init = 512; std::vector<int> rb_k, up_rates, up_k; std::vector<std::vector<int>> rb_d;
  int upp = 1;
  int spec_channels = 0, segment = 0;
  bool keep_params = false;
  DevVec wgrad_part;
  bool f0 = true;
};

Synth* synth_create(Ctx* ctx, const SynthConfig& c) {
  std::unique_ptr<Synth> S(new Synth());
  S->ctx = ctx;
  S->inter = c.inter_channels; S->hidden = c.hidden_channels; S->filt = c.filter_channels; S->n_heads = c.n_heads;
  S->n_layers = c.n_layers; S->ksz = c.kernel_size; S->gin = c.gin_channels; S->n_spk = c.spk_embed_dim; S->sr = c.sr;
  S->feat_dim = c.feat_dim; S->up_init = c.upsample_initial_channel;
  S->spec_channels = c.spec_channels; S->segment = c.segment_size;
  RVC_REQUIRE(c.n_resblock_kernels == 3, "ResBlock1 x3 expected");
  for (int i = 0; i < 3; ++i) { S->rb_k.push_back(c.resblock_kernel_sizes[i]); S->rb_d.push_back({c.resblock_dilations[i][0], c.resblock_dilations[i][1], c.resblock_dilations[i][2]}); }
  S->upp = 1;
  for (int i = 0; i < c.n_upsamples; ++i) { S->up_rates.push_back(c.upsample_rates[i]); S->up_k.push_back(c.upsample_kernel_sizes[i]); S->upp *= c.upsample_rates[i]; }
  RVC_REQUIRE(S->hidden % S->n_heads == 0, "heads must divide hidden");
  RVC_REQUIRE(S->hidden / S->n_heads == 96, "hidden_channels / n_heads must be 96, got " + std::to_string(S->hidden / S->n_heads));
  return S.release();
}
void synth_destroy(Synth* S) { delete S; }
void synth_set_tensor(Synth* S, const char* name, const float* d, const long long* shape, int ndim) { S->ts.set(name, d, shape, ndim); }
int synth_upp(const Synth* S) { return S->upp; }
int synth_feat_dim(const Synth* S) { return S->feat_dim; }
bool synth_has_f0(const Synth* S) { return S->f0; }
bool synth_has_posterior(const Synth* S) { return S->ready && S->post_enc.built; }
void synth_keep_parameters(Synth* S, bool on) {
  RVC_REQUIRE(!S->ready, "synth_keep_parameters: set the switch before finalize");
  S->keep_params = on;
}

int synth_dec_halo_frames(const Synth* S) {
  long long h = 3;
  for (int i = (int)S->up_rates.size() - 1; i >= 0; --i) {
    long long rb = 0;
    for (size_t j = 0; j < S->rb_k.size(); ++j) {
      long long r = 0;
      for (int d : S->rb_d[j]) r += (long long)(S->rb_k[j] - 1) / 2 * d + (S->rb_k[j] - 1) / 2;
      rb = std::max(rb, r);
    }
    h += rb;
    const long long u = S->up_rates[i], ku = S->up_k[i], p = (ku - u) / 2;
    h = std::max((h + ku - 1 - p) / u, (h + p + u - 1) / u);
  }
  return (int)(h + 3);
}

static void make_wn(const TensorStore& ts, const std::string& p, int n, int C, WNStack& W, FlowHostWeights* keep = nullptr) {
  W.n = n;
  W.in.resize(n); W.in_gate.resize(n); W.skip.resize(n); W.res.resize(n - 1); W.rs.resize(n - 1);
  for (int i = 0; i < n; ++i) {
    W.in[i] = make_conv1d(ts, p + "in_layers." + std::to_string(i), 1, 2, 1, true, true, 1.f, 0, -1, keep ? &keep->in[i] : nullptr);
    if ((C & 15) == 0) {
      const std::string q = p + "in_layers." + std::to_string(i);
      const HostTensor& v = ts.get(q + ".weight_v");
      const std::vector<float> w = weight_norm0(v, ts.get(q + ".weight_g"));
      const std::vector<float>& b = ts.get(q + ".bias").data;
      const int Ci = (int)v.shape[1], k = (int)v.shape[2];
      RVC_REQUIRE((int)v.shape[0] == 2 * C, q + ": expected 2 H rows");
      std::vector<float> wp(w.size()), bp(b.size());
      for (int r = 0; r < 2 * C; ++r) {
        const int src = wn_gate_row_order(r, C);
        std::copy(w.begin() + (size_t)src * Ci * k, w.begin() + (size_t)(src + 1) * Ci * k, wp.begin() + (size_t)r * Ci * k);
        bp[r] = b[src];
      }
      conv1d_layer_init(W.in_gate[i], wp.data(), bp.data(), 2 * C, Ci, k, 1, 2, 1, 1);
    }
    const std::string rs = p + "res_skip_layers." + std::to_string(i);
    if (i < n - 1) {
      W.res[i] = make_conv1d(ts, rs, 1, 0, 1, true, true, 1.f, 0, C);
      W.skip[i] = make_conv1d(ts, rs, 1, 0, 1, true, true, 1.f, C, C);
      W.rs[i] = make_conv1d(ts, rs, 1, 0, 1, true, true, 1.f, 0, -1, keep ? &keep->rs[i] : nullptr);
    } else {
      W.skip[i] = make_conv1d(ts, rs, 1, 0, 1, true, true, 1.f, 0, -1, keep ? &keep->rs[i] : nullptr);
    }
  }
  W.cond_w.upload(weight_norm0(ts.get(p + "cond_layer.weight_v"), ts.get(p + "cond_layer.weight_g")));
  W.cond_b.upload(ts.get(p + "cond_layer.bias").data);
  RVC_REQUIRE(W.cond_b.n == (size_t)2 * C * n, p + "cond_layer: expected 2 H n rows");
}

void synth_finalize(Synth* S) {
  S->ready = false; static_cast<SynthWeights&>(*S) = {};
  const TensorStore& ts = S->ts;
// ... 233 lines not shown
  return stats;
}

struct WnBufs { float* hw; float* xin; float* acts; unsigned char* hw_s; unsigned char* acts_s; };
struct WnRecord { float* x[3]; float* a[3]; };
static void wn_run_record(hipStream_t s, const WNStack& W, const float* gcond, bool gs, const WnBufs& b, int C, int T, const WnRecord& rec) {
  const long long tp = split_image_tp(T);
  float* h = b.hw; float* wo = b.hw + (size_t)C * T;
  unsigned char* wo_s = gs ? b.hw_s + split_image_bytes(C, T) : nullptr;
  ConvEpilogue E0;
  RVC_REQUIRE(W.n == 3, "a recorded WaveNet stack has 3 layers");
  if (gs) fill(s, wo, 0.f, (long long)C * T);
  for (int i = 0; i < W.n; ++i) {
    RVC_HIP_CHECK(hipMemcpyAsync(rec.x[i], h, (size_t)C * T * sizeof(float), hipMemcpyDeviceToDevice, s));
    if (gs) conv_x3s_run(W.in[i], s, b.hw_s, tp, T, rec.a[i], T, E0); else conv1d_run(W.in[i], s, h, T, T, rec.a[i], T, E0);
    wn_gate_record(s, rec.a[i], gcond + (size_t)i * 2 * C, gs ? nullptr : b.acts, gs ? b.acts_s : nullptr, tp, kSplitMargin, C, T);
    if (gs) {
      if (i < W.n - 1) { ConvEpilogue Ea; Ea.R = b.hw; Ea.ldR = T; Ea.ys_out = b.hw_s; Ea.ys_tp = tp; conv_x3s_run(W.rs[i], s, b.acts_s, tp, T, b.hw, T, Ea); }
      else { ConvEpilogue Ea; Ea.R = wo; Ea.ldR = T; Ea.ys_out = wo_s; Ea.ys_tp = tp; conv_x3s_run(W.skip[i], s, b.acts_s, tp, T, wo, T, Ea); }
    } else {
      ConvEpilogue Es; Es.accumulate = (i > 0);
      conv1d_run(W.skip[i], s, b.acts, T, T, wo, T, Es);
      if (i < W.n - 1) { ConvEpilogue Er; Er.R = h; Er.ldR = T; conv1d_run(W.res[i], s, b.acts, T, T, h, T, Er); }
    }
  }
}
static void wn_run(hipStream_t s, const WNStack& W, const float* gcond, bool gs, const WnBufs& b, int C, int T, const WnRecord* rec = nullptr) {
  if (rec) return wn_run_record(s, W, gcond, gs, b, C, T, *rec);
  const long long tp = split_image_tp(T);
  float* h = b.hw; float* wo = b.hw + (size_t)C * T;
  ConvEpilogue E0;
  if (gs) {
    unsigned char* wo_s = b.hw_s + split_image_bytes(C, T);
    fill(s, wo, 0.f, (long long)C * T);
    for (int i = 0; i < W.n; ++i) {
      if (W.in_gate[i].Wx_ && conv_x3s_eligible(W.in_gate[i])) {
        ConvEpilogue Eg; Eg.ys_out = b.acts_s; Eg.ys_tp = tp; Eg.gate_h = C; Eg.gate_g = gcond + (size_t)i * 2 * C;
        conv_x3s_run(W.in_gate[i], s, b.hw_s, tp, T, nullptr, T, Eg);
      } else {
        conv_x3s_run(W.in[i], s, b.hw_s, tp, T, b.xin, T, E0);
        wn_gate_split(s, b.xin, gcond + (size_t)i * 2 * C, b.acts_s, tp, kSplitMargin, C, T);
      }
      if (i < W.n - 1) { ConvEpilogue Ea; Ea.R = b.hw; Ea.ldR = T; Ea.ys_out = b.hw_s; Ea.ys_tp = tp; conv_x3s_run(W.rs[i], s, b.acts_s, tp, T, b.hw, T, Ea); }
      else { ConvEpilogue Ea; Ea.R = wo; Ea.ldR = T; Ea.ys_out = wo_s; Ea.ys_tp = tp; conv_x3s_run(W.skip[i], s, b.acts_s, tp, T, wo, T, Ea); }
    }
    return;
  }
  for (int i = 0; i < W.n; ++i) {
    conv1d_run(W.in[i], s, h, T, T, b.xin, T, E0);
    wn_gate(s, b.xin, gcond + (size_t)i * 2 * C, b.acts, C, T);
    ConvEpilogue Es; Es.accumulate = (i > 0);
    conv1d_run(W.skip[i], s, b.acts, T, T, wo, T, Es);
    if (i < W.n - 1) { ConvEpilogue Er; Er.R = h; Er.ldR = T; conv1d_run(W.res[i], s, b.acts, T, T, h, T, Er); }
  }
}

static void coupling_run(Synth* S, hipStream_t s, FlowLayer& F, const float* gcond, bool gs, const SplitImgs& im, const WnBufs& b, float* cur, int T, bool reverse,
                         const WnRecord* rec = nullptr) {
  const int C = S->hidden, half = S->inter / 2;
  const long long tp = split_image_tp(T);
  float* h = b.hw; float* wo = b.hw + (size_t)C * T;
  float* x1 = cur + (size_t)half * T;
  ConvEpilogue E0;
  if (gs) {
    split_image_from_f32(s, cur, T, half, T, im.x0_s, tp);
    unsigned char* wo_s = b.hw_s + split_image_bytes(C, T);
    ConvEpilogue Eh; Eh.ys_out = b.hw_s; Eh.ys_tp = tp;
    conv_x3s_run(F.pre, s, im.x0_s, tp, T, h, T, Eh);
    wn_run(s, F.wn, gcond, gs, b, C, T, rec);
    ConvEpilogue Ep; Ep.R = x1; Ep.ldR = T;
    conv_x3s_run(reverse ? F.post_neg : F.post, s, wo_s, tp, T, x1, T, Ep);
    return;
  }
  conv1d_run(F.pre, s, cur, T, T, h, T, E0);
  wn_run(s, F.wn, gcond, gs, b, C, T, rec);
  ConvEpilogue Ep; Ep.out_scale = reverse ? -1.f : 1.f; Ep.accumulate = 1;
  conv1d_run(F.post, s, wo, T, T, x1, T, Ep);
}

static void gen_tail(Synth* S, hipStream_t s, Arena& A, bool gs, unsigned char* z_s, const float* z, const float* har, const float* pre_bias, int T, int g0, int W,
                     int h2, float* out, const SynthTaps* taps) {
  const int IC = S->inter;
  const bool dry = A.dry;
  auto plan_tin = [&](int tin_full) { return W != T ? tin_full : 0; };
  const long long Nw = (long long)W * S->upp;
  const float* har_w = har ? har + (size_t)g0 * S->upp : nullptr;
  float* zw = (!gs && W != T) ? A.alloc<float>((size_t)IC * W) : nullptr;
  float* cur = A.alloc<float>((size_t)S->up_init * W);
  if (!dry) {
    ConvEpilogue Eb; Eb.bias_override = pre_bias;
    const long long tpw = split_image_tp(W);
    Eb.plan_tin = plan_tin(T);
    if (gs) { split_image_from_f32(s, z + g0, T, IC, W, z_s, tpw); conv_x3s_run(S->conv_pre, s, z_s, tpw, W, cur, W, Eb); }
    else if (zw) {
      RVC_HIP_CHECK(hipMemcpy2DAsync(zw, (size_t)W * sizeof(float), z + g0, (size_t)T * sizeof(float), (size_t)W * sizeof(float), IC, hipMemcpyDeviceToDevice, s));
      conv1d_run(S->conv_pre, s, zw, W, W, cur, W, Eb);
    } else conv1d_run(S->conv_pre, s, z, T, T, cur, T, Eb);
  }
  int Tc = W, Tfull_c = T;
  const int nu = (int)S->stages.size();
  for (int i = 0; i < nu; ++i) {
    GenStage& st = S->stages[i];
    const int Cc = S->up_init >> (i + 1);
    const int Tn = Tc * st.u, Tfull_n = Tfull_c * st.u;
    float* up = A.alloc<float>((size_t)Cc * Tn);
    float* t1 = A.alloc<float>((size_t)Cc * Tn);
    float* ya = A.alloc<float>((size_t)Cc * Tn);
    float* yb = A.alloc<float>((size_t)Cc * Tn);
    float* xs = A.alloc<float>((size_t)Cc * Tn);
    float* fr = (S->f0 && st.noise_k > 1) ? A.alloc<float>((size_t)st.noise_k * Tn) : nullptr;
    const GenPairs gp = gen_stage_pairs(st, Tfull_n, h2);
    unsigned char* t1s = gp.any_split ? A.alloc<unsigned char>(split_image_bytes(Cc, Tn)) : nullptr;
    if (!dry) {
      RVC_REQUIRE(conv1d_out_len(st.up, Tc) == Tn, "ConvTranspose1d geometry must give T_out = u * T_in");
      ConvEpilogue Eu; Eu.plan_tin = plan_tin(Tfull_c); Eu.pre_act = ACT_LRELU; Eu.pre_slope = 0.1f;
      conv1d_run(st.up, s, cur, Tc, Tc, up, Tn, Eu);
      ConvEpilogue En; En.plan_tin = plan_tin(Tfull_n); En.accumulate = 1;
      bool noise_in_rb3 = S->f0 && st.noise_k == 1 && st.noise_w.p != nullptr && Nw == (long long)Tn && !(taps && i == 0);
      Rb3Plan rb3[3]; bool rb3_ok[3];
      auto plan_rb3 = [&](bool noise) {
        bool all = true;
        for (int j = 0; j < 3; ++j) {
          const ConvLayer* r1[3] = {&st.rb[j].c1[0], &st.rb[j].c1[1], &st.rb[j].c1[2]};
          const ConvLayer* r2[3] = {&st.rb[j].c2[0], &st.rb[j].c2[1], &st.rb[j].c2[2]};
          rb3_ok[j] = conv_rb3_plan(r1, r2, up, Tn, Tn, Tfull_n, xs, Tn, 0.1f, 1.f / 3.f, j > 0, h2, noise ? har_w : nullptr, noise ? st.noise_w.p : nullptr,
                                    noise ? st.noise_b.p : nullptr, rb3[j]);
          all = all && rb3_ok[j];
        }
        return all;
      };
      if (!plan_rb3(noise_in_rb3) && noise_in_rb3) { noise_in_rb3 = false; plan_rb3(false); }
      if (noise_in_rb3) {
      } else if (!S->f0) {
      } else if (st.noise_w.p && noise_add(s, up, Tn, Cc, Tn, har_w, Nw, st.noise_k, st.noise_s, st.noise_k > 1 ? st.noise_s / 2 : 0, st.noise_w.p, st.noise_b.p)) {
      } else if (st.noise_k > 1) {
        frames(s, har_w, fr, (int)Nw, st.noise_k, st.noise_s, st.noise_s / 2, Tn, 0);
        conv1d_run(st.noise, s, fr, Tn, Tn, up, Tn, En);
      } else {
        conv1d_run(st.noise, s, har_w, Tn, Tn, up, Tn, En);
      }
      if (taps && i == 0) tap(A, s, taps->gen_ups0, up, (size_t)Cc * Tn);
      for (int j = 0; j < 3; ++j) {
        const float* in = up;
        if (rb3_ok[j]) { conv_rb3_launch(rb3[j], s); continue; }
        for (int m = 0; m < 3; ++m) {
          ConvEpilogue E2; E2.plan_tin = plan_tin(Tfull_n); E2.pre_act = ACT_LRELU; E2.pre_slope = 0.1f; E2.R = in; E2.ldR = Tn;
          float* dst = (m == 0) ? ya : (m == 1 ? yb : xs);
          if (m == 2) { E2.out_scale = 1.f / 3.f; E2.accumulate = (j > 0); }
          ConvPlan pp;
          if (conv_x3_pair_plan(st.rb[j].c1[m], st.rb[j].c2[m], in, Tn, Tn, Tfull_n, dst, Tn, E2, h2, pp)) conv_plan_launch(pp, s);
          else {
            ConvEpilogue E1; E1.plan_tin = plan_tin(Tfull_n); E1.pre_act = ACT_LRELU; E1.pre_slope = 0.1f;
            if (gp.split_pair[j][m]) {
              E1.ys_out = t1s; E1.ys_tp = split_image_tp(Tn); E1.ys_slope = E2.pre_slope;
              E1.h2 = gp.h2_pair[j][m] ? 1 : 0;
              conv1d_run(st.rb[j].c1[m], s, in, Tn, Tn, nullptr, Tn, E1);
              ConvEpilogue E2s = E2; E2s.pre_act = ACT_NONE; E2s.xs_in = t1s; E2s.xs_tp = E1.ys_tp; E2s.h2 = E1.h2;
              conv1d_run(st.rb[j].c2[m], s, nullptr, Tn, Tn, dst, Tn, E2s);
            } else {
              conv1d_run(st.rb[j].c1[m], s, in, Tn, Tn, t1, Tn, E1);
              conv1d_run(st.rb[j].c2[m], s, t1, Tn, Tn, dst, Tn, E2);
            }
          }
          in = dst;
        }
      }
      if (taps && i == nu - 1) tap(A, s, taps->gen_last, xs, (size_t)Cc * Tn);
    }
    cur = xs; Tc = Tn; Tfull_c = Tfull_n;
  }
  if (!dry) conv_to1(s, cur, Tc, S->conv_post_w.p, S->up_init >> nu, 7, 3, Tc, 0.01f, 1, out + (size_t)g0 * S->upp);
}

struct GenTape {
  struct Tensor { size_t off; int rows; long long cols; bool flow = false; };
  const Synth* S = nullptr; int seg = 0; bool recorded = false;
  bool backward_done = false;
  std::map<std::string, Tensor> t;
  DevVec mem; float* fr = nullptr;
  DevVec flow_mem; int flow_T = 0; bool flow_recorded = false; int flow_fwd_marks = 0, flow_bwd_marks = 0;
  bool timing = false; std::vector<hipEvent_t> ev; int fwd_marks = 0, bwd_marks = 0, wgrad_marks = 0;
  GenTape() = default;
  GenTape(const GenTape&) = delete; GenTape& operator=(const GenTape&) = delete;
  ~GenTape() { for (hipEvent_t e : ev) (void)hipEventDestroy(e); }
  void mark(hipStream_t s, int slot) {
    if (!timing) return;
    while ((int)ev.size() <= slot) { hipEvent_t e; RVC_HIP_CHECK(hipEventCreate(&e)); ev.push_back(e); }
    RVC_HIP_CHECK(hipEventRecord(ev[slot], s));
  }
  float* ptr(const std::string& name) const {
    auto it = t.find(name);
    RVC_REQUIRE(it != t.end(), "the tape holds no tensor '" + name + "'");
    return (it->second.flow ? flow_mem.p : mem.p) + it->second.off;
  }
};
constexpr int kFlowMark0 = 32;
constexpr int kWgradMark0 = 16;
static std::string rb_name(int i, int j, const char* what, int m) { return "rb" + std::to_string(i) + "." + std::to_string(j) + "." + what + std::to_string(m); }
static void tape_check(const Synth* S, const GenTape* tape) {
  RVC_REQUIRE(tape->S == S, "the tape was created from another synthesizer handle");
  RVC_REQUIRE(tape->seg == S->segment && S->gen_bwd.built, "the tape was created for another segment_size (the handle was finalized again)");
}

void gen_bwd_conv_image(const float* w, int Co, int Ci, int k, std::vector<uint16_t>& P) {
  RVC_REQUIRE(Co >= 16 && Co % 16 == 0 && Ci >= 1 && k >= 1 && k <= 16, "decoder convolution does not fit the data-gradient kernel");
  std::vector<float> wt((size_t)Co * Ci * k);
  for (int co = 0; co < Co; ++co)
    for (int ci = 0; ci < Ci; ++ci)
      for (int t = 0; t < k; ++t) wt[((size_t)ci * Co + co) * k + t] = w[((size_t)co * Ci + ci) * k + (k - 1 - t)];
  x3_weight_image(wt.data(), Ci, Co, k, (Ci + 127) & ~127, P);
}
void gen_bwd_up_image(const float* w, int Cin, int Cout, int k, std::vector<uint16_t>& P) {
  RVC_REQUIRE(Cout >= 16 && Cout % 16 == 0 && Cin >= 1 && k >= 1 && k <= 16, "up-sampler does not fit the data-gradient kernel");
  x3_weight_image(w, Cin, Cout, k, (Cin + 127) & ~127, P);
}

static void gen_bwd_build(Synth* S) {
  GenBwdImages& B = S->gen_bwd; GenHostWeights& H = S->gen_host;
  if (B.built) return;
  const int nu = (int)S->stages.size();
  RVC_REQUIRE(!H.pre.empty() && (int)H.up.size() == nu, "the decoder's folded weights were not kept (no posterior was loaded at finalize)");
  GenBwdImages N;
  auto conv_image = [&](const std::vector<float>& w, int Co, int Ci, int k, DevBuf<uint16_t>& img) {
    RVC_REQUIRE(w.size() == (size_t)Co * Ci * k, "decoder convolution: weight size");
    std::vector<uint16_t> P;
    gen_bwd_conv_image(w.data(), Co, Ci, k, P);
    img.upload(P); N.bytes += P.size() * sizeof(uint16_t);
  };
  conv_image(H.pre, S->up_init, S->inter, 7, N.pre);
  N.up.resize(nu); N.noise.resize(nu); N.c1.resize((size_t)nu * 9); N.c2.resize((size_t)nu * 9);
  for (int i = 0; i < nu; ++i) {
    const GenStage& st = S->stages[i];
    const int cin = S->up_init >> i, cout = S->up_init >> (i + 1);
    RVC_REQUIRE(H.up[i].size() == (size_t)cin * cout * st.k, "up-sampler: weight size");
    std::vector<uint16_t> P;
    gen_bwd_up_image(H.up[i].data(), cin, cout, st.k, P);
    N.up[i].upload(P); N.bytes += P.size() * sizeof(uint16_t);
    if (S->f0) { N.noise[i].upload(H.noise[i]); N.bytes += H.noise[i].size() * sizeof(float); }
    for (int j = 0; j < 3; ++j)
      for (int m = 0; m < 3; ++m) {
// ... 674 lines not shown
```

comfy-rvc_amd/csrc/rvc_api.hip:

```cpp
#include "models.h"
#include "conv_kernels.h"

namespace rvc {
static thread_local std::string g_err;
void set_error(const std::string& msg) { g_err = msg; }
}

using namespace rvc;

struct rvc_ctx { Ctx c; };
static std::mutex g_ctx_mu;
static std::map<int, int> g_ctx_count;
struct rvc_hubert { Hubert* m; rvc_ctx* ctx; };
struct rvc_rmvpe { Rmvpe* m; rvc_ctx* ctx; };
struct rvc_synth { Synth* m; rvc_ctx* ctx; };
struct rvc_conv1d_plan { OwnedConvLayer L; };

#define RVC_TRY try {
#define RVC_CATCH                                                            \
  return 0;                                                                  \
  }                                                                          \
  catch (const std::exception& e) { rvc::set_error(e.what()); return 1; }    \
  catch (...) { rvc::set_error("unknown error"); return 2; }

// ... 1364 lines not shown
  ConvEpilogue e; e.act = relu ? ACT_RELU : ACT_NONE;
  conv2d_run(L, (hipStream_t)stream, x, (long long)H * W, H, W, y, 4LL * H * W, e);
  check_launch();
  RVC_HIP_CHECK(hipStreamSynchronize((hipStream_t)stream));
  RVC_CATCH
}
int rvc_op_gemm_tn(void* stream, const float* a, const float* b, float* y, int M, int N, int K, int batch) {
  RVC_TRY
  ConvEpilogue e;
  gemm_tn_run((hipStream_t)stream, a, M, (long long)K * M, b, N, (long long)K * N, y, N, (long long)M * N, M, N, K, batch, nullptr, 0, e);
  check_launch();
  RVC_CATCH
}
int rvc_conv1d_plan_create(const float* w, const float* bias, int Ci, int Co, int k, int stride, int pad, int dil, int groups,
                           rvc_conv1d_plan** out) {
  RVC_TRY
  std::unique_ptr<rvc_conv1d_plan> p(new rvc_conv1d_plan());
  conv1d_layer_init(p->L, w, bias, Co, Ci, k, stride, pad, dil, groups);
  *out = p.release();
  RVC_CATCH
}
int rvc_conv1d_plan_run(rvc_conv1d_plan* p, void* stream, const float* x, int Tin, const float* res, float* y, int pre_act, float pre_slope,
                        int act, float act_slope) {
  RVC_TRY
  RVC_REQUIRE(p, "null argument");
  ConvEpilogue e; e.pre_act = pre_act; e.pre_slope = pre_slope; e.act = act; e.act_slope = act_slope;
  const int Tout = conv1d_out_len(p->L, Tin);
  e.R = res; e.ldR = Tout;
  conv1d_run(p->L, (hipStream_t)stream, x, Tin, Tin, y, Tout, e);
  check_launch();
  RVC_CATCH
}
int rvc_conv1d_plan_pair_run(rvc_conv1d_plan* c1, rvc_conv1d_plan* c2, void* stream, const float* x, int T, float* y, float out_scale,
                             int accumulate) {
  RVC_TRY
  RVC_REQUIRE(c1 && c2 && x && y, "null argument");
  ConvEpilogue e; e.pre_act = ACT_LRELU; e.pre_slope = 0.1f; e.R = x; e.ldR = T; e.out_scale = out_scale; e.accumulate = accumulate;
  ConvPlan p;
  RVC_REQUIRE(conv_x3_pair_plan(c1->L, c2->L, x, T, T, T, y, T, e, conv_set_pair_arithmetic(-1), p),
              "this pair of layers is not eligible for the fused ResBlock kernel (needs bf16x3 images, C = 32, equal odd k, long T)");
  conv_plan_launch(p, (hipStream_t)stream);
  check_launch();
  RVC_CATCH
}
int rvc_conv1d_plan_resblock_run(rvc_conv1d_plan* const* plans6, void* stream, const float* x, int T, float* y, float out_scale, int accumulate,
                                 int* ran_out, const float* noise_src, const float* noise_w, const float* noise_b) {
  RVC_TRY
  RVC_REQUIRE(plans6 && x && y && ran_out, "null argument");
  const ConvLayer* c1[3]; const ConvLayer* c2[3];
  for (int i = 0; i < 3; ++i) {
    RVC_REQUIRE(plans6[2 * i] && plans6[2 * i + 1], "null plan");
    c1[i] = &plans6[2 * i]->L; c2[i] = &plans6[2 * i + 1]->L;
  }
  Rb3Plan p;
  *ran_out = conv_rb3_plan(c1, c2, x, T, T, T, y, T, 0.1f, out_scale, accumulate, conv_set_pair_arithmetic(-1), noise_src, noise_w, noise_b, p) ? 1 : 0;
  if (*ran_out) conv_rb3_launch(p, (hipStream_t)stream);
  check_launch();
  RVC_CATCH
}
int rvc_conv1d_plan_pair_split_run(rvc_conv1d_plan* c1, rvc_conv1d_plan* c2, void* stream, const float* x, int T, float* y, float out_scale,
                                   int accumulate) {
  RVC_TRY
  RVC_REQUIRE(c1 && c2 && x && y, "null argument");
  RVC_REQUIRE(conv1d_split_eligible(c1->L, T, SPLIT_PRODUCER) && conv1d_split_eligible(c2->L, T, SPLIT_CONSUMER), "layers not eligible for split-resident tensors at this length");
  hipStream_t s = (hipStream_t)stream;
  unsigned char* img = (unsigned char*)stream_scratch(s, 5, split_image_bytes(c1->L.Co, T));
  ConvEpilogue E1; E1.pre_act = ACT_LRELU; E1.pre_slope = 0.1f; E1.ys_out = img; E1.ys_tp = split_image_tp(T); E1.ys_slope = 0.1f;
  E1.h2 = conv1d_pair_h2_eligible(c1->L, c2->L, T, conv_set_pair_arithmetic(-1)) ? 1 : 0;
  conv1d_run(c1->L, s, x, T, T, nullptr, T, E1);
  ConvEpilogue E2; E2.R = x; E2.ldR = T; E2.out_scale = out_scale; E2.accumulate = accumulate; E2.xs_in = img; E2.xs_tp = E1.ys_tp; E2.h2 = E1.h2;
  conv1d_run(c2->L, s, nullptr, T, T, y, T, E2);
  check_launch();
  RVC_CATCH
}
int rvc_conv1d_plan_pair_arithmetic(rvc_conv1d_plan* c1, rvc_conv1d_plan* c2, int T) {
  if (!c1 || !c2) return -1;
  try {
    const int h2 = conv_set_pair_arithmetic(-1);
    if (conv1d_pair_h2_eligible(c1->L, c2->L, T, h2)) return 1;
    ConvEpilogue e; e.pre_act = ACT_LRELU; e.pre_slope = 0.1f; e.ldR = T;
    ConvPlan p;
    return conv_x3_pair_plan(c1->L, c2->L, nullptr, T, T, T, nullptr, T, e, h2, p) && p.a.h2 ? 1 : 0;
  } catch (...) { return -1; }
}
int rvc_conv1d_plan_destroy(rvc_conv1d_plan* p) { delete p; return 0; }
int rvc_op_attention(void* stream, const float* q, const float* k, const float* v_rm, const float* bv, float* out, int heads, int T) {
  RVC_TRY
  attention_fused((hipStream_t)stream, q, k, T, v_rm, (long long)heads * 64, bv, out, T, heads, 64, T);
  check_launch();
  RVC_CATCH
}
int rvc_op_attention_rel(void* stream, const float* q, const float* k, const float* v_rm, const float* bv, const float* rel, float* pb,
                         float* out, int heads, int T, const float* ek, const float* ev) {
  RVC_TRY
  attention_rel_fused((hipStream_t)stream, q, k, T, v_rm, (long long)heads * 96, bv, rel, pb, 10, out, T, heads, 96, T, ek, ev);
  check_launch();
  RVC_CATCH
}
int rvc_op_layernorm_c(void* stream, const float* x, const float* res, const float* gamma, const float* beta, float* y, int C, int T) {
  RVC_TRY
  layernorm_c((hipStream_t)stream, x, res, gamma, beta, y, C, T, T, 1e-5f);
  check_launch();
  RVC_CATCH
}
int rvc_op_layernorm_c_split(void* stream, const float* x, const float* gamma, const float* beta, float* y, float* y_img_f32, int C, int T) {
  RVC_TRY
  RVC_REQUIRE(x && gamma && beta && y_img_f32 && C > 0 && (C & 15) == 0 && T > 0, "bad argument");
  hipStream_t s = (hipStream_t)stream;
  DevBytes img;
  const long long tp = split_image_tp(T);
  img.alloc(split_image_bytes(C, T));
  layernorm_c_split(s, x, gamma, beta, y, img.p, tp, kSplitMargin, C, T, T, 1e-5f);
  split_image_to_f32(s, img.p, tp, C, T, y_img_f32, T);
  check_launch();
  RVC_HIP_CHECK(hipStreamSynchronize(s));
  RVC_CATCH
}
int rvc_op_sine_source(void* stream, const float* f0, const float* noise, float* har, float* sine, int T, int upp, float sr, float lw, float lb,
                       float* rad_out, float* tmp_out, float* phase_out) {
  RVC_TRY
  hipStream_t st = (hipStream_t)stream;
  const long long N = (long long)T * upp;
  RVC_REQUIRE(T > 0 && upp > 0, "bad argument");
  const size_t nb = (size_t)((N + 1023) / 1024);
  const size_t tb = ((size_t)T * sizeof(float) + 255) & ~size_t(255);
  char* scr = (char*)stream_scratch(st, 2, 2 * tb + nb * sizeof(double));
  float* rad = (float*)scr; float* tmp = (float*)(scr + tb); double* bsum = (double*)(scr + 2 * tb);
  sine_source(st, f0, noise, har, sine, rad, tmp, bsum, T, upp, sr, lw, lb, phase_out);
  if (rad_out) RVC_HIP_CHECK(hipMemcpyAsync(rad_out, rad, T * sizeof(float), hipMemcpyDeviceToDevice, st));
  if (tmp_out) RVC_HIP_CHECK(hipMemcpyAsync(tmp_out, tmp, T * sizeof(float), hipMemcpyDeviceToDevice, st));
  RVC_HIP_CHECK(hipStreamSynchronize(st));
  check_launch();
  RVC_CATCH
}

struct Image2d { DevBytes b; long long tp = 0; int margin = 0; };
static Image2d image2d_alloc(hipStream_t s, int C, int H, int W) {
  Image2d im;
  im.margin = split_geom_2d(W).margin;
  im.tp = im.margin + (long long)H * (W + 2) + 704 + 64;
  const size_t bytes = (size_t)(C / 16) * 4 * im.tp * 16;
  im.b.alloc(bytes);
  RVC_HIP_CHECK(hipMemsetAsync(im.b.p, 0xff, bytes, s));
  return im;
}
static void image2d_to_f32(hipStream_t s, const Image2d& im, int C, long long P, float* y, long long ld) {
  split_image_to_f32(s, im.b.p + (size_t)(im.margin - kSplitMargin) * 16, im.tp, C, (int)P, y, ld);
}

int rvc_op_hubert_conv0(void* stream, const float* audio, int64_t L, const float* w, const float* gamma, const float* beta, int C, int T1, float* out, float* out_img_f32,
                        int64_t ld) {
  RVC_TRY
  RVC_REQUIRE(audio && w && gamma && beta && (out || out_img_f32) && C > 0 && T1 > 0 && L > 0 && ld >= T1, "bad argument");
  hipStream_t s = (hipStream_t)stream;
  DevBuf<double> partial; DevBuf<float> stat; DevBytes img;
  partial.alloc(hubert_conv0_scratch_doubles(C, T1)); stat.alloc((size_t)2 * C);
  if (out) hubert_conv0_gn_gelu(s, audio, L, w, gamma, beta, C, T1, 1e-5f, out, ld, partial.p, stat.p);
  if (out_img_f32) {
    RVC_REQUIRE((C & 15) == 0, "the image needs C % 16 == 0");
    const long long tp = split_s2_tp(T1); const int H = split_s2_h(T1);
    img.alloc(split_s2_bytes(C, T1));
    RVC_HIP_CHECK(hipMemsetAsync(img.p, 0xff, split_s2_bytes(C, T1), s));
    hubert_conv0_gn_gelu_img(s, audio, L, w, gamma, beta, C, T1, 1e-5f, img.p, tp, kSplitMargin, H, partial.p, stat.p);
    split_image_deint_to_f32(s, img.p, tp, H, C, T1, out_img_f32, ld);
  }
  check_launch();
// ... 218 lines not shown
```

comfy-rvc_amd/csrc/rvc_internal.h:

```cpp
#pragma once
#include <atomic>
#include <hip/hip_runtime.h>
#include <cstdint>
#include <cstdio>
#include <cstdlib>
#include <cmath>
#include <cstring>
#include <map>
#include <mutex>
#include <string>
#include <vector>
#include <stdexcept>

namespace rvc {

void set_error(const std::string& msg);
struct Error : std::runtime_error { using std::runtime_error::runtime_error; };

#define RVC_HIP_CHECK(expr)                                                                       \
  do {                                                                                            \
    hipError_t _e = (expr);                                                                       \
    if (_e != hipSuccess)                                                                         \
      throw rvc::Error(std::string(#expr) + " failed: " + hipGetErrorString(_e) + " (" + __FILE__ + \
                       ":" + std::to_string(__LINE__) + ")");                                     \
  } while (0)

#define RVC_REQUIRE(cond, msg)                                                                    \
  do {                                                                                            \
    if (!(cond)) throw rvc::Error(std::string("requirement failed: ") + #cond + " : " + (msg));   \
  } while (0)

inline int knob_int(const char* name, int def) { const char* e = getenv(name); return e ? atoi(e) : def; }
#ifdef RVC_EXPERIMENTS
inline int exp_int(const char* name, int def) { return knob_int(name, def); }
#define RVC_EXP_STR(name) getenv(name)
#else
#define exp_int(name, def) (def)
#define RVC_EXP_STR(name) ((const char*)nullptr)
#endif

enum Act : int { ACT_NONE = 0, ACT_LRELU = 1, ACT_RELU = 2, ACT_GELU = 3, ACT_TANH = 4, ACT_SIGMOID = 5, ACT_LOGCLAMP = 6 };

struct ConvArgs {
  const float* X; const float* W; const float* bias; const float* R; float* Y;
  int Ci;
  int Co;
  int CoP;
  int Tin;
  int Tout;
  int Wd;
  int ktaps;
  int dil, stride, pad;
  int CK;
  int KT;
  int nchunk;
  int WROW;
  int PW, BWd, BH;
  long long xBatch, wBatch, yBatch, rBatch; int bBatch;
  long long ldX, ldY, ldR;
  int pre_act; float pre_slope;
  int act; float act_slope;
  int act_before_res;
  float out_scale; int accumulate;
  int ostride, orows;
  int up2;
  int KH, KW, PH, PWL;
};

struct ConvLayer {
  float* Wd_ = nullptr;
  float* bd_ = nullptr;
  float* bd4_ = nullptr;
  int mode = 1;
  int Ci = 0, Co = 0, CoP = 0, groups = 1;
  int k = 1, stride = 1, dil = 1, pad = 0;
  int ktaps = 1, CK = 8, KT = 1, nchunk = 1;
  int tconv_u = 0;
  int co_real = 0;
  int up2 = 0;
  int conv_pad = 0;
  long long wBatch = 0;
  int kh = 3, kw = 3, ph = 1, pwl = 1;
  uint16_t* Wx_ = nullptr;
  int CoPx = 0; long long wxBatch = 0;
  uint16_t* Wh_ = nullptr;
  int seg2_chunks = 0;
};

struct ConvEpilogue {
  const float* R = nullptr; long long ldR = 0;
  int pre_act = ACT_NONE; float pre_slope = 0.f;
  int act = ACT_NONE; float act_slope = 0.f;
  int act_before_res = 0;
  float out_scale = 1.f; int accumulate = 0;
  const float* bias_override = nullptr;
  int tout_limit = 0;
  int plan_tin = 0;
  const unsigned char* xs_in = nullptr; long long xs_tp = 0;
  unsigned char* ys_out = nullptr; long long ys_tp = 0; float ys_slope = 1.f;
  unsigned char* vt_out = nullptr; long long vt_tp = 0; int vt_row0 = 0;
  int gate_h = 0; const float* gate_g = nullptr;
  int ys_deint_h = 0;
  int h2 = 0;
};
constexpr int kSplitMargin = 64;
inline long long split_image_tp(long long T) { return (T + kSplitMargin + 704 + 63) & ~63LL; }
inline size_t split_image_bytes(int C, long long T) { return (size_t)(C / 16) * 2 * (size_t)split_image_tp(T) * 32; }
enum SplitRole : int { SPLIT_CONSUMER = 0, SPLIT_PRODUCER = 1 };
bool conv1d_split_eligible(const ConvLayer& L, int Tin, SplitRole role = SPLIT_CONSUMER, int h2 = 0);
bool conv1d_pair_h2_eligible(const ConvLayer& c1, const ConvLayer& c2, int Tin, int h2);
int conv1d_residual_period(const ConvLayer& L, int Tin, int h2);
int conv_set_pair_arithmetic(int mode);


void conv1d_layer_init(ConvLayer& L, const float* w , const float* bias, int Co, int Ci, int k,
                       int stride, int pad, int dil, int groups);
void tconv1d_layer_init(ConvLayer& L, const float* w , const float* bias, int Ci, int Co, int k, int u, int pad);
void conv2d3x3_layer_init(ConvLayer& L, const float* w , const float* bias, int Co, int Ci);
void conv2d1x1_layer_init(ConvLayer& L, const float* w , const float* bias, int Co, int Ci);
void tconv2d_layer_init(ConvLayer& L, const float* w , const float* bias, int Ci, int Co);
void conv2d_kx_layer_init(ConvLayer& L, const float* w , const float* bias, int Co, int Ci, int KH, int KW, int PH, int PWL);
bool conv_x3_set_default(bool on);
int conv_set_precision(int mode);
struct ConvBuildScope {
  int prev_mode; bool prev_default;
  explicit ConvBuildScope(int precision) : prev_mode(conv_set_precision(-1)), prev_default(conv_x3_set_default(true)) {
    if (precision >= 0) conv_set_precision(precision);
  }
  ~ConvBuildScope() { conv_x3_set_default(prev_default); conv_set_precision(prev_mode); }
  ConvBuildScope(const ConvBuildScope&) = delete; ConvBuildScope& operator=(const ConvBuildScope&) = delete;
};

int conv1d_out_len(const ConvLayer& L, int Tin);
void conv1d_run(const ConvLayer& L, hipStream_t s, const float* X, long long ldX, int Tin, float* Y, long long ldY,
                const ConvEpilogue& e);
void gemm_tn_run(hipStream_t s, const float* A, long long ldA, long long aBatch, const float* B, long long ldB, long long bBatch,
                 float* Y, long long ldY, long long yBatch, int M, int N, int K, int batch, const float* bias, int biasBatch,
                 const ConvEpilogue& e);
void conv2d_run(const ConvLayer& L, hipStream_t s, const float* X, long long ldX, int H, int Wd, float* Y, long long ldY,
                const ConvEpilogue& e);

struct SplitGeom { int ktaps = 1; int toff[16] = {0}; int padw = 0; int margin = kSplitMargin;
                   long long seg2_off = 0;
                   int s2_h = 0; };
void conv_layer_append_x3(ConvLayer& dst, const ConvLayer& extra);
SplitGeom split_geom_2d(int Wd, int KH = 3, int KW = 3, int PH = 1, int PWL = 1);
inline int split_s2_h(long long Tin) { return (int)(((Tin + 1) / 2 + 64 + 63) & ~63LL); }
inline long long split_s2_tp(long long Tin) { return (kSplitMargin + 2LL * split_s2_h(Tin) + 704 + 63) & ~63LL; }
inline size_t split_s2_bytes(int C, long long Tin) { return (size_t)(C / 16) * 2 * (size_t)split_s2_tp(Tin) * 32; }
SplitGeom split_geom_s2(int k, long long Tin);
bool conv_x3s_s2_eligible(const ConvLayer& L);
inline int wn_gate_row_order(int p, int H) { const int b = p >> 5, q = p & 31; return q < 16 ? 16 * b + q : H + 16 * b + (q - 16); }
void split_image_deint_from_f32(hipStream_t s, const float* X, long long ldX, int C, int T, unsigned char* img, long long tp, int H);
void split_image_deint_to_f32(hipStream_t s, const unsigned char* img, long long tp, int H, int C, int T, float* Y, long long ldY);
bool conv_x3s_eligible(const ConvLayer& L);
void conv_x3s_run(const ConvLayer& L, hipStream_t s, const unsigned char* Xs, long long xsTp, int T, float* Y, long long ldY, const ConvEpilogue& e,
                  const SplitGeom* geom = nullptr);
void conv_x3s_run_swapped(const ConvLayer& L, int row0, int rows, hipStream_t s, const unsigned char* Xs, long long xsTp, int T, unsigned char* Ys, long long ysTp,
                          float* Yrm = nullptr, long long ldYrm = 0,
                          const float* Rrm = nullptr, long long ldRrm = 0);
void split_image_from_tm(hipStream_t s, const float* x, int C, int T, int M, unsigned char* img, long long tp);
void conv_x3s_force(int ksplit, int am, int an);
void x3_weight_image(const float* w, int Co, int Ci, int k, int CoPx, std::vector<uint16_t>& P);
struct ConvX3dArgs {
  const float* X; const unsigned char* Wx; const float* bias; float* Y;
  int Ci, Co, CoPx, H, Hout, p, k, stride, pad, S; float slope;
};
struct ConvX3dPlan { ConvX3dArgs a; dim3 grid; int units = 1; size_t lds = 0; double flops = 0.0; };
bool conv_x3d_plan(const ConvX3dArgs& a, ConvX3dPlan& p);
void conv_x3d_launch(const ConvX3dPlan& p, hipStream_t s);
struct ConvX3dBwdArgs {
  const float* D; const unsigned char* Wx[3]; const float* Cot; const float* A; float* Y;
  int R, RPx, Ck, Hd, H, p, ostride, off0, nph, S; int nt[3]; int Hj[3]; int tile0[4]; float slope;
};
struct ConvX3dBwdPlan { ConvX3dBwdArgs a; dim3 grid; int units = 1; size_t lds = 0; double flops = 0.0; };
bool conv_x3d_bwd_plan(const ConvX3dBwdArgs& a, ConvX3dBwdPlan& p);
void conv_x3d_bwd_launch(const ConvX3dBwdPlan& p, hipStream_t s);
int disc_bwd_weight_images(const float* w, int Co, int Ci, int k, int stride, int pad, std::vector<uint16_t> (&img)[3], int (&nt)[3]);
void disc_bwd_geometry(ConvX3dBwdArgs& a, int Ci, int Co, int k, int stride, int pad, int H, int Hd, int p, int S, float slope);
struct ConvGenBwdArgs {
  const float* D; long long ldD; int Td; const unsigned char* Wx; const float* A; const float* Res; float* Y; long long ldY;
  int R, RPx, Ck, N, nt, cstride, tstep, off0; float slope, scale; int accumulate;
};
struct ConvGenBwdPlan { ConvGenBwdArgs a; dim3 grid; int bm = 128, units = 1; size_t lds = 0; double flops = 0.0; };
bool conv_gen_bwd_plan(const ConvGenBwdArgs& a, ConvGenBwdPlan& p);
void conv_gen_bwd_launch(const ConvGenBwdPlan& p, hipStream_t s);
void gen_bwd_conv_image(const float* w, int Co, int Ci, int k, std::vector<uint16_t>& P);
void gen_bwd_up_image(const float* w, int Cin, int Cout, int k, std::vector<uint16_t>& P);
void gen_tanh_bwd(hipStream_t s, const float* dy, const float* y, float* d, long long n);
void gen_post_bwd(hipStream_t s, const float* d, const float* w, const float* x, float* dx, int C, int k, int pad, long long T, float slope, float scale);
void gen_noise_bwd(hipStream_t s, const float* D, const float* w, float* dhar, float* out2, int C, int k, int stride, int pad, long long T, long long N, int accumulate);
void gen_row_sums(hipStream_t s, const float* D, int C, long long T, float* out, float* out2);
void gen_cond_bwd(hipStream_t s, const float* W, const float* dcond, int C, int G, float* out, float* out2);
struct ConvFlowBwdArgs {
  const float* D; long long ldD; int Td; const float* A; int H; const unsigned char* Wx; const float* Res; float* Y; long long ldY;
  int R, RPx, Ck, N, nt, off0, len;
};
struct ConvFlowBwdPlan { ConvFlowBwdArgs a; dim3 grid; int units = 1; size_t lds = 0; };
bool conv_flow_bwd_plan(const ConvFlowBwdArgs& a, ConvFlowBwdPlan& p);
void conv_flow_bwd_launch(const ConvFlowBwdPlan& p, hipStream_t s);
void flow_unflip(hipStream_t s, const float* x, float* y, float* dm, int C, int T, int len);
void flow_gate_bwd(hipStream_t s, const float* dacts, const float* a, float* da, float* dgc, int H, int T, int len);
void flow_cond_bwd(hipStream_t s, const float* const (&W)[4], const float* const (&dgc)[4], int C, int G, float* out, float* out2);
void wn_gate_record(hipStream_t s, float* a, const float* g, float* out, unsigned char* img, long long tp, int margin, int H, int T);
struct ConvX3dWgradArgs {
  const float* D; const float* X; float* part;
  int Ci, Co, H, Hout, p, k, stride, pad, S; int cps, per, total;
};
struct ConvX3dWgradPlan { ConvX3dWgradArgs a; dim3 grid; int splits = 1; size_t lds = 0, part_floats = 0; double flops = 0.0; };
bool conv_x3d_wgrad_plan(const ConvX3dWgradArgs& a, ConvX3dWgradPlan& p);
void conv_x3d_wgrad_launch(const ConvX3dWgradPlan& p, hipStream_t s);
struct DiscWgradFinishArgs { const float* part; const float* D; const float* v; const float* g; float* gw; float* gg; float* gb; long long pstride; int splits, S, Co, N, L; };
void disc_wgrad_finish(hipStream_t s, const DiscWgradFinishArgs& a);
constexpr int kGenWgradMaxItems = 16;
constexpr size_t kGenWgradPartFloats = (size_t)16 << 20;
struct GenItems { const float* p[kGenWgradMaxItems]; };
struct ConvGenWgradArgs {
  const float* P[kGenWgradMaxItems]; const float* G[kGenWgradMaxItems]; float* part;
  int B, R, C, k, N; long long ldP, ldG; int Tg, cstride, tstep, off0; float slopeP, slopeG; int cps, per, total;
};
struct ConvGenWgradPlan { ConvGenWgradArgs a; dim3 grid; int bm = 128, splits = 1; size_t lds = 0, part_floats = 0; double flops = 0.0; };
bool conv_gen_wgrad_plan(const ConvGenWgradArgs& a, ConvGenWgradPlan& p);
void conv_gen_wgrad_launch(const ConvGenWgradPlan& p, hipStream_t s);
struct GenWgradFinishArgs { const float* part; long long pstride; int splits, R, L; const float* v; const float* g; float* gw; float* gg; float* gb; GenItems D; int B, brows; long long N; };
void gen_wgrad_finish(hipStream_t s, const GenWgradFinishArgs& a);
void gen_wgrad_noise(hipStream_t s, const GenItems& D, const GenItems& H, int B, int C, long long T, long long Nh, int k, int stride, int pad, float* gw, float* gb);
void gen_wgrad_post(hipStream_t s, const GenItems& D, const GenItems& X, int B, int C, long long T, int k, int pad, float slope, float* gw);
void gen_wgrad_cond(hipStream_t s, const GenItems& DC, const GenItems& Gv, int B, int C, int G, float* gw, float* gb, float* gb2);
void gen_wgrad_msource(hipStream_t s, const GenItems& DH, const GenItems& H, const GenItems& Sn, int B, long long N, float* gw, float* gb);
bool cbr2_small_eligible(const ConvLayer& c1, const ConvLayer& c2);
void cbr2_small_run(const ConvLayer& c1, const ConvLayer& c2, hipStream_t s, const float* x, int H, int W, float* out);
bool conv3_small_eligible(const ConvLayer& L);
void conv3_small_run(const ConvLayer& L, hipStream_t s, const float* x, int H, int W, float* Y, float* Y2, int split_row, int relu_rows, const float* R);
void split_image_from_f32(hipStream_t s, const float* X, long long ldX, int C, int T, unsigned char* img, long long tp);
void split_image_to_f32(hipStream_t s, const unsigned char* img, long long tp, int C, int T, float* Y, long long ldY);

void attention_fused(hipStream_t s, const float* Q, const float* K, long long ldqk, const float* V, long long ldv, const float* bv,
                     float* out, long long ldo, int heads, int dhead, int T, unsigned char* out_img = nullptr, long long img_tp = 0);

long long attention_vt_tp(int channels);
size_t attention_vt_bytes(int channels, int T);
void attention_vt_clear_tail(hipStream_t s, unsigned char* vt_img, int channels, int T);
void attention_split(hipStream_t s, const unsigned char* qk_img, long long qk_tp, int qk_channels, int q_chunk0, int k_chunk0, const unsigned char* vt_img,
                     int heads, int dhead, int T, float scale, const float* bv, float* out, long long ldo, unsigned char* out_img, long long img_tp,
                     int win = 0, const unsigned char* ek_img = nullptr, const unsigned char* evt_img = nullptr);
void attention_split_force_kz(int kz);
void attention_rel_images(const float* ek, const float* ev, int D, int win, std::vector<uint16_t>& ek_img, std::vector<uint16_t>& evt_img);
void attention_rel_fused(hipStream_t s, const float* Q, const float* K, long long ldqk, const float* V, long long ldv, const float* bv,
                         const float* rel, float* pb, int win, float* out, long long ldo, int heads, int dhead, int T, const float* ek = nullptr,
                         const float* ev = nullptr);

void conv_prof_enable(bool on);
int conv_prof_collect(double* ms, double* flops, long long* launches);
const char* conv_prof_cfg_name(int i);
void conv_timing_read(unsigned long long* out8, bool reset);

void* dev_alloc(size_t bytes);
void* dev_upload(const void* host, size_t bytes);
template <typename T> T* dev_upload(const T* host, size_t n) { return static_cast<T*>(dev_upload(static_cast<const void*>(host), n * sizeof(T))); }
void dev_free(void* p);
void* stream_scratch(hipStream_t s, int slot, size_t bytes);
void* stream_scratch_zeroed(hipStream_t s, int slot, size_t bytes, bool* fresh = nullptr);
void stream_scratch_release(int device);

template <typename T> struct DevBuf {
  T* p = nullptr; size_t n = 0;
  DevBuf() = default;
  ~DevBuf() { dev_free(p); }
  DevBuf(DevBuf&& o) noexcept : p(o.p), n(o.n) { o.p = nullptr; o.n = 0; }
  DevBuf& operator=(DevBuf&& o) noexcept { if (this != &o) { dev_free(p); p = o.p; n = o.n; o.p = nullptr; o.n = 0; } return *this; }
  DevBuf(const DevBuf&) = delete; DevBuf& operator=(const DevBuf&) = delete;
  T* get() const { return p; }
  void reset() { dev_free(p); p = nullptr; n = 0; }
  void alloc(size_t cnt) { reset(); p = static_cast<T*>(dev_alloc(cnt * sizeof(T))); n = cnt; }
  void upload(const T* h, size_t cnt) { reset(); p = dev_upload(h, cnt); n = cnt; }
  void upload(const std::vector<T>& h) { upload(h.data(), h.size()); }
};

struct OwnedConvLayer : ConvLayer {
  OwnedConvLayer() = default;
  ~OwnedConvLayer() { free_weights(); }
  OwnedConvLayer(OwnedConvLayer&& o) noexcept : ConvLayer(o) { o.disown(); }
  OwnedConvLayer& operator=(OwnedConvLayer&& o) noexcept { if (this != &o) { free_weights(); ConvLayer::operator=(o); o.disown(); } return *this; }
  OwnedConvLayer(const OwnedConvLayer&) = delete; OwnedConvLayer& operator=(const OwnedConvLayer&) = delete;
  OwnedConvLayer(const ConvLayer&) = delete; OwnedConvLayer& operator=(const ConvLayer&) = delete;
 private:
  void disown() { Wd_ = bd_ = bd4_ = nullptr; Wx_ = Wh_ = nullptr; }
  void free_weights() { dev_free(Wd_); dev_free(bd_); dev_free(bd4_); dev_free(Wx_); dev_free(Wh_); }
};

#define RVC_ALLOW_BIG_LDS(kern)                                                                                                              \
  do {                                                                                                                                       \
    static std::atomic<unsigned long long> rvc_lds_mask_[4];                                                                                 \
    int rvc_dev_ = 0; (void)hipGetDevice(&rvc_dev_);                                                                                         \
    const unsigned long long rvc_bit_ = 1ull << (rvc_dev_ & 63);                                                                             \
    std::atomic<unsigned long long>& rvc_m_ = rvc_lds_mask_[(rvc_dev_ >> 6) & 3];                                                            \
    if (!(rvc_m_.load(std::memory_order_acquire) & rvc_bit_)) {                                                                              \
      RVC_HIP_CHECK(hipFuncSetAttribute(reinterpret_cast<const void*>(kern), hipFuncAttributeMaxDynamicSharedMemorySize, 160 * 1024));      \
      rvc_m_.fetch_or(rvc_bit_, std::memory_order_release);                                                                                  \
    }                                                                                                                                        \
  } while (0)

struct Arena {
  char* base = nullptr; size_t cap = 0, off = 0, peak = 0; bool dry = false;
  unsigned gen = 0;
  void reset() { off = 0; }
  template <typename T> T* alloc(size_t n) {
    size_t bytes = (n * sizeof(T) + 255) & ~size_t(255);
    size_t o = off; off += bytes; if (off > peak) peak = off;
    if (dry) return reinterpret_cast<T*>(uintptr_t(0x1000) + o);
    RVC_REQUIRE(off <= cap, "arena overflow");
    return reinterpret_cast<T*>(base + o);
  }
  void ensure(size_t bytes);
  void release();
  Arena() = default;
  ~Arena() { release(); }
  Arena(const Arena&) = delete; Arena& operator=(const Arena&) = delete;
};

template <typename F> void arena_passes(Arena& A, F&& graph) {
  struct Restore { Arena& a; ~Restore() { a.dry = false; } } restore{A};
  A.dry = true; A.reset(); A.peak = 0;
  graph();
  A.ensure(A.peak);
  A.dry = false; A.reset();
  graph();
}

struct ZeroedBlock {
  const void* base = nullptr; unsigned gen = 0; size_t bytes = 0; int key0 = -1, key1 = -1;
  bool stale(const void* b, unsigned g, size_t n, int k0, int k1) const { return base != b || gen != g || bytes != n || key0 != k0 || key1 != k1; }
  void remember(const void* b, unsigned g, size_t n, int k0, int k1) { base = b; gen = g; bytes = n; key0 = k0; key1 = k1; }
  void reset() { base = nullptr; }
  void ensure_zero(const Arena& A, size_t start, size_t n, int k0, int k1, hipStream_t s) {
    if (A.dry || !stale(A.base + start, A.gen, n, k0, k1)) return;
    RVC_HIP_CHECK(hipMemsetAsync(A.base + start, 0, n, s));
    remember(A.base + start, A.gen, n, k0, k1);
  }
};

}
```

include/rvc_hip.h:

```cpp
#ifndef RVC_HIP_H
#define RVC_HIP_H
#include <stdint.h>

#ifdef __cplusplus
extern "C" {
#endif

typedef struct rvc_ctx rvc_ctx;
typedef struct rvc_hubert rvc_hubert;
typedef struct rvc_rmvpe rvc_rmvpe;
typedef struct rvc_synth rvc_synth;

const char* rvc_last_error(void);
const char* rvc_version(void);

int rvc_ctx_create(int device_id, rvc_ctx** out);
int rvc_ctx_destroy(rvc_ctx* ctx);
int64_t rvc_ctx_workspace_bytes(rvc_ctx* ctx);
int rvc_ctx_set_conv_precision(rvc_ctx* ctx, int mode);

typedef struct rvc_hubert_taps {
  float* conv_stack;
  float* pos_conv;
  float* hidden_0;
// ... 211 lines not shown

int rvc_lfilter_hp(void* stream, const void* x_dev, int is_f64, int64_t n, const double* sos18_host, double* y_dev);
int rvc_frame_rms(void* stream, const double* x_dev, int64_t n, int win, int hop, double* rms_dev, int64_t n_frames);
int rvc_slice_tags(const double* rms_host, int64_t n_frames, int64_t n_samples, double threshold, int64_t min_length, int64_t min_interval,
                   int64_t max_sil_kept, int64_t* tags_host, int64_t cap, int64_t* n_tags);
int rvc_cut_windows(void* stream, const double* filt_dev, int64_t n, const int64_t* windows_dev, int n_windows, int sr, int target_sr,
                    const double* taps_dev, int half, int up, int down, float max_volume, float* gt_dev, int64_t total_gt, float* y16_dev,
                    int64_t total_16);

int rvc_gate_levels(void* stream, const float* x_dev, int64_t n, int win, double* ss_dev, int64_t n_windows);
int rvc_gate_ranges(const double* level_db_host, int64_t n_windows, int64_t n, int64_t win, int64_t min_size, int64_t fade, double threshold_db,
                    int64_t* ranges_host, int64_t cap, int64_t* n_ranges);
int rvc_gate_apply(void* stream, const float* x_dev, float* y_dev, int64_t n, const int64_t* ranges_dev, int n_ranges, int64_t fade);
int rvc_declick(void* stream, const float* x_dev, int64_t n, int size, float multiplier, int method, int kernel_size, int detect, float* y_dev,
                uint8_t* mask_dev);
int rvc_peak_normalize(void* stream, const float* x_dev, int64_t n, float gain, float* y_dev);
int rvc_peak_limit(void* stream, float* x_dev, int64_t n, float max_volume);
int rvc_merge_tracks(void* stream, const float* const* tracks_host, const int64_t* lens_host, int k, int mode, float* out_dev, int64_t n_out);
int rvc_segment_energy(void* stream, const int16_t* x_dev, int64_t n, int k, int64_t* out_dev);

int rvc_spectrogram_batch(rvc_ctx* ctx, void* stream, const float* audio_dev, int64_t n_audio, const int64_t* clips_host, int n_clips, int n_fft, int hop,
                          float eps, int clamp, float* out_dev, int64_t pitch);
int rvc_mel_filterbank_set(rvc_ctx* ctx, int n_fft, int n_mels, const int32_t* first_host, const int32_t* count_host, const float* weights_host);
int rvc_spec_to_mel_batch(rvc_ctx* ctx, void* stream, const float* spec_dev, int64_t spec_pitch, const int64_t* clips_host, int n_clips, int n_fft,
                          int n_mels, float* mel_dev, int64_t mel_pitch);
int rvc_spectrogram_batch_ms(rvc_ctx* ctx, void* stream, const float* audio_dev, int64_t n_audio, const int64_t* clips_host, int n_clips, int n_fft, int hop,
                             float eps, int clamp, float* out_dev, int64_t pitch);
int rvc_mel_spectrogram_vjp(rvc_ctx* ctx, void* stream, const float* audio_dev, int64_t n_audio, const int64_t* clips_host, int n_clips, int n_fft, int hop,
                            float eps, int clamp, int n_mels, const float* cot_mel_dev, int64_t pitch, float* d_audio_dev);
int rvc_mel_spectrogram_vjp_launch_count(void);
int rvc_mel_loss_cotangents(void* stream, int K, const float* const* a_dev, const float* const* b_dev, const int64_t* n, int loss, float log_weight,
                            float mag_weight, const float* scale, float* const* out_dev);
int rvc_multiscale_mel_loss(rvc_ctx* ctx, void* stream, int K, const float* const* spec_dev, const int64_t* pitch, const int64_t* row_stride, int B, int64_t nf,
                            const int32_t* n_fft, const int32_t* n_mels, int loss, int want_mag, double* out_dev);

int rvc_hpss(void* stream, const float* x_dev, int B, int F, int T, float* h_dev, float* p_dev, int medians);
int rvc_hpss_l1(void* stream, const float* org_dev, const float* gen_dev, int B, int F, int T, float eps, double* sums_dev);
int rvc_tsi_terms(void* stream, const float* org_dev, const float* gen_dev, int B, int F, int T, float eps, double* out_dev);

int rvc_op_conv1d(void* stream, const float* x_dev, const float* w_host, const float* bias_host, const float* res_dev, float* y_dev,
                  int Ci, int Co, int Tin, int k, int stride, int pad, int dil, int groups, int pre_act, float pre_slope, int act,
                  float act_slope, int act_before_res, float out_scale, int accumulate);
int rvc_op_disc_conv(void* stream, const float* x_dev, const float* w_host, const float* bias_host, float* y_dev, int S, int Ci, int Co, int H, int p, int k,
                     int stride, int pad, float slope, int* units_out);
int rvc_op_disc_conv_plan(int S, int Ci, int Co, int H, int p, int k, int stride, int pad, int* info);
int rvc_op_disc_conv_input_grad(void* stream, const float* d_dev, const float* w_host, const float* cot_dev, const float* a_dev, float* y_dev, int S, int Ci, int Co,
                                int H, int Hd, int p, int stride, float slope, int* units_out);
int rvc_op_disc_conv_input_grad_plan(int S, int Ci, int Co, int H, int Hd, int p, int stride, int* info);
int rvc_op_disc_conv_weight_grad(void* stream, const float* d_dev, const float* x_dev, float* dw_dev, int S, int Ci, int Co, int H, int p, int k, int stride, int pad,
                                 int* splits_out);
int rvc_op_disc_conv_weight_grad_plan(int S, int Ci, int Co, int H, int p, int k, int stride, int pad, int* info);
int rvc_op_conv1d_input_grad(void* stream, const float* d_dev, const float* w_host, const float* a_dev, const float* res_dev, float* y_dev, int transposed, int Ci,
                             int Co, int k, int step, int pad, int64_t N, int64_t Td, int64_t ldD, int64_t ldY, float slope, float scale, int accumulate,
                             int* bm_out, int* units_out);
int rvc_op_conv1d_input_grad_plan(int transposed, int Ci, int Co, int k, int step, int pad, int64_t N, int64_t Td, int* info);
int rvc_op_gemm_split(void* stream, const float* x_dev, const float* w_host, const float* bias_host, const float* res_dev, float* y_dev,
                      float* ysplit_f32_dev, int Ci, int Co, int T, int act, float act_slope, int act_before_res, float out_scale, int ksplit,
                      int am, int an, int k, int dil);
int rvc_op_conv1d_split(void* stream, const float* x_dev, const float* w_host, const float* bias_host, const float* res_dev, float* y_dev,
                        int Ci, int Co, int T, int k, int pad, int dil, int groups, int act, int act_before_res);
int rvc_op_conv1d_s2_split(void* stream, const float* x_dev, const float* w_host, const float* bias_host, float* y_dev, float* y_img_f32_dev, int Ci, int Co, int T, int k,
                           int act);
int rvc_op_conv2d_split(void* stream, const float* x_dev, const float* w_host, const float* bias_host, const float* res_dev, float* y_dev,
                        float* ysplit_f32_dev, int Ci, int Co, int H, int W, int act, int act_before_res, int ksplit, int am, int an);
int rvc_op_conv_transpose1d(void* stream, const float* x_dev, const float* w_host, const float* bias_host, float* y_dev, int Ci, int Co,
                            int Tin, int k, int u, int pad, int pre_act, float pre_slope, int accumulate);
int rvc_op_conv2d3x3(void* stream, const float* x_dev, const float* w_host, const float* bias_host, const float* res_dev, float* y_dev,
                     int Ci, int Co, int H, int W, int relu);
int rvc_op_conv_transpose2d(void* stream, const float* x_dev, const float* w_host, const float* bias_host, float* y_dev, int Ci, int Co,
                            int H, int W, int relu);
int rvc_op_gemm_tn(void* stream, const float* a_dev, const float* b_dev, float* y_dev, int M, int N, int K, int batch);
typedef struct rvc_conv1d_plan rvc_conv1d_plan;
int rvc_conv1d_plan_create(const float* w_host, const float* bias_host, int Ci, int Co, int k, int stride, int pad, int dil, int groups,
                           rvc_conv1d_plan** out);
int rvc_conv1d_plan_run(rvc_conv1d_plan* p, void* stream, const float* x_dev, int Tin, const float* res_dev, float* y_dev, int pre_act,
                        float pre_slope, int act, float act_slope);
int rvc_conv1d_plan_pair_split_run(rvc_conv1d_plan* c1, rvc_conv1d_plan* c2, void* stream, const float* x_dev, int T, float* y_dev,
                                   float out_scale, int accumulate);
int rvc_conv1d_plan_pair_run(rvc_conv1d_plan* c1, rvc_conv1d_plan* c2, void* stream, const float* x_dev, int T, float* y_dev, float out_scale,
                             int accumulate);
int rvc_conv1d_plan_resblock_run(rvc_conv1d_plan* const* plans6, void* stream, const float* x_dev, int T, float* y_dev, float out_scale, int accumulate,
                                 int* ran_out, const float* noise_src_dev, const float* noise_w_dev, const float* noise_b_dev);
int rvc_conv1d_plan_pair_arithmetic(rvc_conv1d_plan* c1, rvc_conv1d_plan* c2, int T);
int rvc_conv1d_plan_destroy(rvc_conv1d_plan* p);
int rvc_op_attention(void* stream, const float* q_dev, const float* k_dev, const float* v_rm_dev, const float* bv_dev, float* out_dev,
                     int heads, int T);
int rvc_op_attention_split(void* stream, const float* q_dev, const float* k_dev, const float* v_dev, const float* bv_dev, float* out_dev,
                           float* out_img_f32_dev, int heads, int T);
int rvc_op_attention_split_rel(void* stream, const float* q_dev, const float* k_dev, const float* v_dev, const float* bv_dev, const float* ek_host,
                               const float* ev_host, float* out_dev, float* out_img_f32_dev, int heads, int T, int kz);
int rvc_op_cbr2_small(void* stream, const float* x_dev, const float* w1_host, const float* b1_host, const float* w2_host, const float* b2_host,
                      float* y_dev, int C, int H, int W);
int rvc_op_layernorm_c_split(void* stream, const float* x_dev, const float* gamma_dev, const float* beta_dev, float* y_dev, float* y_img_f32_dev, int C, int T);
int rvc_op_conv3_small(void* stream, const float* x_dev, const float* w_host, const float* b_host, const float* res_dev, float* y_dev, float* y2_dev, int Ci, int Co,
                       int H, int W, int split_row, int relu_rows);
int rvc_op_wn_in_gate_split(void* stream, const float* x_dev, const float* w_host, const float* bias_host, const float* g_dev, float* y_dev, int Ci, int H, int T, int k);
int rvc_op_gemm_split_qkv(void* stream, const float* x_dev, const float* w_host, const float* bias_host, float* y_img_f32_dev, float* yt_dev, int Ci, int Co, int T,
                          int vt_row0);
int rvc_op_gemm_split_swapped(void* stream, const float* x_dev, const float* w_host, float* yt_dev, int Ci, int Co, int T, int row0, int rows);
int rvc_op_conv2d3x3_plus_1x1(void* stream, const float* x1_dev, const float* w1_host, const float* x2_dev, const float* w2_host, float* y_dev, float* y_img_f32_dev,
                              int Ci1, int Ci2, int Co, int H, int W, int ksplit);
int rvc_op_gemm_split_swapped_res(void* stream, const float* x_dev, const float* w_host, const float* res_dev, float* y_dev, int Ci, int Co, int T, int ld, int off);
int rvc_op_attention_rel(void* stream, const float* q_dev, const float* k_dev, const float* v_rm_dev, const float* bv_dev, const float* rel_dev,
                         float* pb_dev, float* out_dev, int heads, int T, const float* ek_dev, const float* ev_dev);
int rvc_op_layernorm_c(void* stream, const float* x_dev, const float* res_dev, const float* gamma_dev, const float* beta_dev, float* y_dev,
                       int C, int T);
int rvc_op_sine_source(void* stream, const float* f0_dev, const float* noise_dev, float* har_dev, float* sine_dev, int T, int upp, float sr,
                       float lin_w, float lin_b, float* rad_dev, float* tmp_dev, float* phase_dev);

int rvc_op_hubert_conv0(void* stream, const float* audio_dev, int64_t L, const float* w_dev, const float* gamma_dev, const float* beta_dev, int C, int T1,
                        float* out_dev, float* out_img_f32_dev, int64_t ld);
int rvc_op_conv_to1(void* stream, const float* x_dev, int64_t ldx, const float* w_dev, int Ci, int K, int pad, int T, float pre_slope, int act_tanh, float* y_dev,
                    int* kernel_out);
int rvc_op_noise_add(void* stream, float* x_dev, int64_t ld, int C, int T, const float* src_dev, int64_t L, int k, int stride, int pad, const float* w_dev,
                     const float* b_dev, int* ran_out);
int rvc_op_transpose(void* stream, const float* in_dev, float* out_dev, int R, int C, int64_t ldin, int64_t ldout, int batch, int64_t bin, int64_t bout);
int rvc_op_frames(void* stream, const float* src_dev, float* out_dev, int L, int k, int stride, int pad, int Tout, int reflect);
int rvc_op_mel_to_unet(void* stream, const float* mel_dev, float* x_dev, int n, int Tr, float a, float b);
int rvc_op_feats_prepare(void* stream, const float* f_dev, const float* f0_dev, const float* pitchf_dev, float* out_dev, int D, int Th, int T, float protect,
                         int do_protect);
int rvc_op_wn_gate(void* stream, const float* a_dev, const float* g_dev, float* out_dev, float* out_img_f32_dev, int H, int T);
int rvc_op_pool2_pad(void* stream, const float* x_dev, int64_t ldx, int x_padded, int C, int H, int W, float* y_dev, float* y_img_f32_dev, int64_t ldy);
int rvc_op_interleave2_pad(void* stream, const float* ph_dev, int64_t ldp, int Co, int H, int W, float* y_dev, int y_padded, float* y_img_f32_dev, int64_t ldy);
int rvc_op_pad2d(void* stream, const float* x_dev, int64_t ldx, int C, int H, int W, float* y_dev, float* y_img_f32_dev, int64_t ldy);
int rvc_op_unpad2d(void* stream, const float* x_dev, int64_t ldx, int C, int H, int W, float* y_dev, int64_t ldy);
int rvc_op_gru_scan(void* stream, const float* gi_dev, const float* b_ih_dev, const float* w_hh_dev, const float* b_hh_dev, float* out_dev, int T, int* err_out);

int rvc_resample(void* stream, const float* x_dev, int64_t n_in, const double* taps_dev, int half, int up, int down, float* y_dev, int64_t n_out);

int rvc_set_conv_precision(int mode);
int rvc_set_pair_arithmetic(int mode);
int rvc_get_pair_arithmetic(void);

#define RVC_PROF_CFGS 24
int rvc_prof_enable(int on);
int rvc_prof_collect(double* ms, double* flops, int64_t* launches);
int rvc_prof_collect_ex(double* out, double ridge_fp32, double ridge_bf16x3);
const char* rvc_prof_cfg_name(int i);
int rvc_prof_dump_csv(const char* path);
#ifdef RVC_EXPERIMENTS
int rvc_debug_conv_timing(uint64_t* out8, int reset);
int rvc_debug_x3p_check(void);
int rvc_debug_gemm_split_bench(void* stream, int Ci, int Co, int T, int ksplit, int am, int an, int split_out, int reps, float* us_out, int w2d,
                               int nlayers);

#endif

#ifdef __cplusplus
}
#endif
#endif
```

Baseline: 2416 audio-sec/wall-sec.

## Claim conv tiles dynamically via per-XCD atomic counters in persistent x3q kernel

When a persistent bf16x3 conv launch has more tiles than resident workgroup slots, workgroups now take their next tile from a per-XCD atomic counter instead of a fixed stride. The claimed index is published through LDS and read back before the next tile's weights are prefetched. The goal is to balance load across workgroups and avoid tail imbalance from static round-robin scheduling. In exchange it adds an atomic per tile, a ring of zeroed counter buffers with memsets, extra LDS, and a new template dimension.

Result: faster. 2442 audio-sec/wall-sec (median of 6 runs) (+1.1%).

```diff
diff --git a/comfy-rvc_amd/_lib.py b/comfy-rvc_amd/_lib.py
--- a/comfy-rvc_amd/_lib.py
+++ b/comfy-rvc_amd/_lib.py
@@ -253,6 +253,7 @@
     "rvc_set_pair_arithmetic": (c_int, [c_int]),
     "rvc_get_pair_arithmetic": (c_int, []),
     "rvc_conv1d_plan_pair_arithmetic": (c_int, [c_void_p, c_void_p, c_int]),
+    "rvc_conv1d_plan_pair_split_tiles": (c_int, [c_void_p, c_void_p, c_int, P(C.c_int64)]),
     "rvc_prof_dump_csv": (c_int, [c_char_p]),
     "rvc_prof_enable": (c_int, [c_int]),
     "rvc_prof_collect": (c_int, [P(C.c_double), P(C.c_double), P(c_int64)]),
diff --git a/comfy-rvc_amd/csrc/conv_kernels.h b/comfy-rvc_amd/csrc/conv_kernels.h
--- a/comfy-rvc_amd/csrc/conv_kernels.h
+++ b/comfy-rvc_amd/csrc/conv_kernels.h
@@ -21,6 +21,7 @@
   int wbufs;
   int xcd_remap;
   int h2;
+  unsigned* claim;
 };
 
 __device__ __forceinline__ __amdgpu_buffer_rsrc_t make_rsrc(const void* base, unsigned bytes) {
@@ -141,6 +142,9 @@
   long long plan_T = 0;
   ConvLaunchFn launch = nullptr;
   dim3 grid; size_t lds = 0;
+  long long tiles = 0;
+  bool claim = false;
+  ClaimRing* ring = nullptr;
   int prof_cfg = 0, prof_fused = 0;
   double alg_bytes = 0.0, flops = 0.0;
 };
diff --git a/comfy-rvc_amd/csrc/conv_mfma.hip b/comfy-rvc_amd/csrc/conv_mfma.hip
--- a/comfy-rvc_amd/csrc/conv_mfma.hip
+++ b/comfy-rvc_amd/csrc/conv_mfma.hip
@@ -377,6 +377,27 @@
   if (r.grew) RVC_HIP_CHECK(hipMemsetAsync(r.p, 0, bytes, s));
   if (fresh) *fresh = r.grew;
   return r.p;
+}
+void ClaimRing::begin(hipStream_t s) {
+  RVC_REQUIRE(buf, "ClaimRing without a buffer");
+  RVC_HIP_CHECK(hipMemsetAsync(buf, 0, kBytes, s));
+  next = 0;
+}
+unsigned* ClaimRing::take(hipStream_t s) {
+  if (next >= kLaunches) begin(s);
+  RVC_REQUIRE(buf && next >= 0 && next < kLaunches, "ClaimRing: no zeroed entry left");
+  return buf + (size_t)kXcds * next++;
+}
+unsigned* stream_claim_take(hipStream_t s) {
+  static std::map<std::pair<int, hipStream_t>, ClaimRing> rings;
+  int dev = 0;
+  RVC_HIP_CHECK(hipGetDevice(&dev));
+  ClaimRing* r;
+  { std::lock_guard<std::mutex> lk(scratch_mu()); r = &rings[{dev, s}]; }
+  bool fresh = false;
+  r->buf = (unsigned*)stream_scratch_zeroed(s, 27, ClaimRing::kBytes, &fresh);
+  if (fresh) r->next = 0;
+  return r->take(s);
 }
 void stream_scratch_release(int device) {
   std::lock_guard<std::mutex> lk(scratch_mu());
@@ -932,7 +953,7 @@
     a.Wx = reinterpret_cast<const unsigned char*>(L.Wh_); a.h2 = 1;
   }
   ConvPlan p;
-  if (L.Wx_ && conv_x3_plan(a, L.groups, Tplan, p)) { p.flops = flops; conv_plan_launch(p, s); }
+  if (L.Wx_ && conv_x3_plan(a, L.groups, Tplan, p)) { p.flops = flops; p.ring = e.claim_ring; conv_plan_launch(p, s); }
   else {
     RVC_REQUIRE(!e.xs_in && !e.ys_out, "split-resident tensors need the bf16x3 kernel (check conv1d_split_eligible first)");
     run_conv(a, 1, L.groups, Tplan, s, flops);
@@ -961,6 +982,12 @@
   return conv_x3_plan(a, 1, a.Tout, p);
 }
 bool conv1d_split_eligible(const ConvLayer& L, int Tin, SplitRole role, int h2) { ConvPlan p; return plan_split_role(L, Tin, role, h2, p); }
+bool conv1d_split_tiles(const ConvLayer& L, int Tin, SplitRole role, int h2, long long out[4]) {
+  ConvPlan p;
+  if (!plan_split_role(L, Tin, role, h2, p) || (p.prof_fused >> 4) != 6) return false;
+  out[0] = p.tiles; out[1] = p.grid.x; out[2] = p.claim ? 1 : 0; out[3] = conv1d_residual_period(L, Tin, h2);
+  return true;
+}
 
 int conv1d_residual_period(const ConvLayer& L, int Tin, int h2) {
   ConvPlan p;
diff --git a/comfy-rvc_amd/csrc/conv_x3.hip b/comfy-rvc_amd/csrc/conv_x3.hip
--- a/comfy-rvc_amd/csrc/conv_x3.hip
+++ b/comfy-rvc_amd/csrc/conv_x3.hip
@@ -430,6 +430,7 @@
   if (a.Xs) RVC_REQUIRE(a.xsTp >= split_image_tp(a.Tin), "split-resident input image is shorter than split_image_tp(T)");
   if (a.Ys) RVC_REQUIRE(a.ysTp >= split_image_tp(a.Tout), "split-resident output image is shorter than split_image_tp(T)");
   if (a.ksplit > 1) a.partial = (float*)stream_scratch(s, 0, (size_t)a.ksplit * a.Co * a.ldP * sizeof(float));
+  a.claim = !p.claim ? nullptr : (p.ring ? p.ring->take(s) : stream_claim_take(s));
   ProfTicket tk = conv_prof_begin(s);
   p.launch(a, p.grid, p.lds, s);
   if (a.ksplit > 1) splitk_reduce_launch(a, a.ksplit, 1, s);
diff --git a/comfy-rvc_amd/csrc/conv_x3q.hip b/comfy-rvc_amd/csrc/conv_x3q.hip
--- a/comfy-rvc_amd/csrc/conv_x3q.hip
+++ b/comfy-rvc_amd/csrc/conv_x3q.hip
@@ -14,7 +14,7 @@
 }
 typedef float f32x4q __attribute__((ext_vector_type(4)));
 
-template <int AM, int AN, int KT, int R, bool XSPLIT, bool YSPLIT, bool RADD, bool H2>
+template <int AM, int AN, int KT, int R, bool XSPLIT, bool YSPLIT, bool RADD, bool H2, bool CLAIM>
 __global__ __launch_bounds__(256, (AM * AN >= 8) ? 2 : 3) void conv_x3q_kernel(const ConvArgsX p) {
   static_assert(!(YSPLIT && RADD), "an image output has no residual");
   static_assert(XSPLIT != YSPLIT, "c1 of a pair (fp32 in, image out) or c2 (image in, fp32 out)");
@@ -45,6 +45,8 @@
   unsigned char* Ws = smemq + ((2 * xbuf + 1023) & ~1023);
   float* Bs = reinterpret_cast<float*>(Ws + R * wslot);
   unsigned char* Ss = reinterpret_cast<unsigned char*>(Bs) + ((p.Co * 4 + 255) & ~255);
+  typedef __attribute__((address_space(3))) volatile unsigned lds_word_t;
+  lds_word_t* Cw = (lds_word_t*)(Ss + (RADD ? NW * 1024 : 0));
 
   const int tid0 = threadIdx.x;
   int lane = tid0 & 63;
@@ -59,8 +61,7 @@
   const __amdgpu_buffer_rsrc_t rrs = make_rsrc(RADD ? (const void*)p.R : (const void*)p.Y, RADD ? (unsigned)p.Co * (unsigned)p.ldR * 4u : 0u);
 
   const unsigned nty = (unsigned)(p.Co / BM), ntiles = (unsigned)((p.Tout + BN - 1) / BN) * nty;
-  auto geom = [&](int it) -> QTile {
-    const unsigned L = blockIdx.x + (unsigned)it * gridDim.x;
+  auto geom_at = [&](unsigned L) -> QTile {
     QTile t;
     t.valid = L < ntiles;
     const unsigned tile = !t.valid ? 0u : (p.xcd_remap ? xcd_tile(L, ntiles) : L);
@@ -69,13 +70,29 @@
     t.edge = XSPLIT && (t.bx < 0 || t.bx + P > p.Tin);
     return t;
   };
+  auto geom = [&](int it) -> QTile { return geom_at(blockIdx.x + (unsigned)it * gridDim.x); };
   const int nit = (int)((ntiles - blockIdx.x + gridDim.x - 1) / gridDim.x);
-
   PhaseTimer<PhaseClock::cycle> tm;
 #ifdef RVC_X3P_CHECK
-  int issued = 0, mk_w[8] = {0, 0, 0, 0, 0, 0, 0, 0}, mk_x[XS] = {0, 0, 0}, mk_r = 0, uwc = 0, mk_xs[2] = {0, 0};
-#endif
-
+  int issued = 0, mk_w[8] = {0, 0, 0, 0, 0, 0, 0, 0}, mk_x[XS] = {0, 0, 0}, mk_r = 0, uwc = 0, mk_xs[2] = {0, 0}, mk_c = 0;
+#endif
+
+  unsigned cl_v = 0;
+  auto claim_issue = [&]() {
+    if (wave == 0) {
+      unsigned ci = blockIdx.x & 7u;
+      asm volatile("" : "+v"(ci));
+      if (lane == 0) cl_v = __hip_atomic_fetch_add(p.claim + ci, 1u, __ATOMIC_RELAXED, __HIP_MEMORY_SCOPE_AGENT);
+      X3P_ISSUED(1);
+#ifdef RVC_X3P_CHECK
+      mk_c = issued;
+#endif
+    }
+  };
+  auto claim_publish = [&](int par) {
+    if (wave == 0 && lane == 0) { unsigned v = cl_v; asm volatile("" : "+v"(v)); Cw[par] = (blockIdx.x & 7u) + 8u * ((gridDim.x >> 3) + v); }
+  };
+  auto claim_read = [&](int par) -> QTile { return geom_at((unsigned)__builtin_amdgcn_readfirstlane((int)Cw[par])); };
   for (int m = tid0; m < p.Co; m += NW * 64) Bs[m] = p.bias ? p.bias[m] : 0.f;
 
   const int NU = nck * KT;
@@ -84,7 +101,7 @@
   const int wrow_h2 = RB == 4 ? wave * 64 + lane : wave * 32 + (lane & 31);
   const int wvoff = H2 ? ((wrow_h2 / BM) * p.CoPx + (wrow_h2 % BM)) * 16
                        : ((wave / RB) * p.CoPx * 32) + (((((wave % RB) * 64 + lane) / BM) * p.CoPx + (((wave % RB) * 64 + lane) % BM)) * 16);
-  QTile cur = geom(0), nxt = geom(1);
+  QTile cur = geom(0), nxt = CLAIM ? cur : geom(1);
   unsigned wsoff = (unsigned)cur.co0 * 16u;
   int slw = 0, uw = 0;
   int wtile_co0_next = nxt.valid ? nxt.co0 : cur.co0;
@@ -228,7 +245,8 @@
 
   int sl = 0, xb = 0;
   tm.lap(1);
-  for (int it = 0; it < nit; ++it) {
+  for (int it = 0; CLAIM ? cur.valid : it < nit; ++it) {
+    if constexpr (CLAIM) claim_issue();
 #pragma unroll
     for (int am = 0; am < AM; ++am) {
       f32x4q bv[4];
@@ -295,8 +313,16 @@
           static_assert(!XSPLIT || R - 2 <= KT - 1, "weight ring deeper than a chunk: the input chunk's DMA would not be covered by the weight wait");
           if constexpr (XSPLIT && last_tap) { if (it > 0 || c > 0) X3P_CHECK(vm6(NWT), issued - mk_xs[xb ^ 1]); }
           tm.lap(3);
+          if constexpr (CLAIM && last_tap) {
+            constexpr int KC = [] { int n = Q::nA(KT - 1); for (int t = 0; t + 1 < KT; ++t) n += Q::tot(t); return n; }();
+            if (c0) { if (wave == 0) X3P_CHECK(vm6(KC), issued - mk_c); wait_vmcnt<vm6(KC)>(); claim_publish(it & 1); }
+          }
           lds_barrier();
           tm.lap(4);
+          if constexpr (CLAIM && last_tap) {
+            static_assert(2 * KT >= R - 1, "the weight requests would enter the next tile before it is claimed");
+            if (c0) { nxt = claim_read(it & 1); wtile_co0_next = nxt.valid ? nxt.co0 : cur.co0; }
+          }
           const int sn = sl + 1 == R ? 0 : sl + 1;
           if (XSPLIT && last_tap && t1.edge) { zero_edges(t1, xb ^ 1); lds_barrier(); }
           issue_w();
@@ -432,38 +458,39 @@
       X3P_ISSUED(EP);
     }
     tm.lap(5); tm.add(0, 1);
-    cur = nxt; nxt = geom(it + 2);
-    wtile_co0_next = nxt.valid ? nxt.co0 : cur.co0;
+    cur = nxt;
+    if constexpr (!CLAIM) { nxt = geom(it + 2); wtile_co0_next = nxt.valid ? nxt.co0 : cur.co0; }
   }
   wait_vmcnt<0>();
   tm.flush();
 }
 
 
-template <int AM, int AN, int KT, int R, bool XSPLIT, bool YSPLIT, bool RADD, bool H2>
+template <int AM, int AN, int KT, int R, bool XSPLIT, bool YSPLIT, bool RADD, bool H2, bool CLAIM>
 static void launch_x3q(const ConvArgsX& a, dim3 grid, size_t lds, hipStream_t s) {
-  auto kern = conv_x3q_kernel<AM, AN, KT, R, XSPLIT, YSPLIT, RADD, H2>;
+  RVC_REQUIRE(!CLAIM || (a.claim && grid.x % 8 == 0), "conv_x3q: a multi-round launch without its tile counters");
+  auto kern = conv_x3q_kernel<AM, AN, KT, R, XSPLIT, YSPLIT, RADD, H2, CLAIM>;
   RVC_ALLOW_BIG_LDS(kern);
   conv_launch(kern, grid, dim3(256), lds, s, a);
 }
-template <int AM, int AN, int KT, int R>
+template <int AM, int AN, int KT, int R, bool CLAIM>
 static ConvLaunchFn select_x3q_io(const ConvArgsX& a, int mode) {
   constexpr bool c2_ok = R - 2 <= KT - 1;
-  if (mode == 0) return a.h2 ? &launch_x3q<AM, AN, KT, R, false, true, false, true> : &launch_x3q<AM, AN, KT, R, false, true, false, false>;
-  if constexpr (c2_ok) return a.h2 ? &launch_x3q<AM, AN, KT, R, true, false, true, true> : &launch_x3q<AM, AN, KT, R, true, false, true, false>;
+  if (mode == 0) return a.h2 ? &launch_x3q<AM, AN, KT, R, false, true, false, true, CLAIM> : &launch_x3q<AM, AN, KT, R, false, true, false, false, CLAIM>;
+  if constexpr (c2_ok) return a.h2 ? &launch_x3q<AM, AN, KT, R, true, false, true, true, CLAIM> : &launch_x3q<AM, AN, KT, R, true, false, true, false, CLAIM>;
   throw Error("conv_x3q: weight ring deeper than a chunk on an image-in launch");
 }
 template <int AM, int AN, int R>
-static ConvLaunchFn select_x3q_k(const ConvArgsX& a, int mode) {
-  if (a.ktaps == 3) return select_x3q_io<AM, AN, 3, R>(a, mode);
-  if (a.ktaps == 7) return select_x3q_io<AM, AN, 7, R>(a, mode);
-  return select_x3q_io<AM, AN, 11, R>(a, mode);
+static ConvLaunchFn select_x3q_k(const ConvArgsX& a, int mode, bool claim) {
+  if (a.ktaps == 3) return claim ? select_x3q_io<AM, AN, 3, R, true>(a, mode) : select_x3q_io<AM, AN, 3, R, false>(a, mode);
+  if (a.ktaps == 7) return claim ? select_x3q_io<AM, AN, 7, R, true>(a, mode) : select_x3q_io<AM, AN, 7, R, false>(a, mode);
+  return claim ? select_x3q_io<AM, AN, 11, R, true>(a, mode) : select_x3q_io<AM, AN, 11, R, false>(a, mode);
 }
 template <int AM, int AN>
-static ConvLaunchFn select_x3q_r(const ConvArgsX& a, int R, int mode) {
-  if (R >= 5) return select_x3q_k<AM, AN, 5>(a, mode);
-  if constexpr (AM == 2 && AN == 4) return select_x3q_k<AM, AN, 4>(a, mode);
-  else return R == 4 ? select_x3q_k<AM, AN, 4>(a, mode) : select_x3q_k<AM, AN, 3>(a, mode);
+static ConvLaunchFn select_x3q_r(const ConvArgsX& a, int R, int mode, bool claim) {
+  if (R >= 5) return select_x3q_k<AM, AN, 5>(a, mode, claim);
+  if constexpr (AM == 2 && AN == 4) return select_x3q_k<AM, AN, 4>(a, mode, claim);
+  else return R == 4 ? select_x3q_k<AM, AN, 4>(a, mode, claim) : select_x3q_k<AM, AN, 3>(a, mode, claim);
 }
 
 bool conv_x3q_plan(ConvPlan& p, int AM, int AN) {
@@ -485,17 +512,18 @@
   const int wslot = (a.h2 ? 1 : 2) * BM * 32;
   const int per_cu = AM * AN >= 8 ? 2 : 3;
   const size_t budget = (size_t)(160 * 1024 / per_cu) & ~(size_t)2047;
-  const size_t fixed = (size_t)xbytes + (size_t)((a.Co * 4 + 255) & ~255) + (mode == 1 ? 4096 : 0);
+  const long long ntiles = (long long)((a.Tout + BN - 1) / BN) * (a.Co / BM);
+  const int ncu = device_cu_count();
+  static const int wg_env = exp_int("RVC_X3Q_WGS", 0);
+  const long long slots = (long long)(wg_env > 0 ? wg_env : per_cu) * ncu;
+  const bool claim = ntiles > slots;
+  const size_t fixed = (size_t)xbytes + (size_t)((a.Co * 4 + 255) & ~255) + (mode == 1 ? 4096 : 0) + (claim ? 256 : 0);
   const int rmin = (AM == 2 && AN == 4) ? 4 : 3;
   int R = (mode == 1 && a.ktaps == 3) ? 4 : 5;
   while (R > rmin && fixed + (size_t)R * wslot > budget) --R;
   const size_t lds = fixed + (size_t)R * wslot;
   if (lds > budget) return false;
-  const long long ntiles = (long long)((a.Tout + BN - 1) / BN) * (a.Co / BM);
-  const int ncu = device_cu_count();
-  static const int wg_env = exp_int("RVC_X3Q_WGS", 0);
   static const int min_rounds = exp_int("RVC_X3Q_MINROUNDS", 0);
-  const long long slots = (long long)(wg_env > 0 ? wg_env : per_cu) * ncu;
   const long long ptiles = ((p.plan_T + BN - 1) / BN) * (a.Co / BM);
   if (ptiles < min_rounds * slots || ptiles < 8) return false;
   RVC_REQUIRE(ntiles >= 8, "column window too narrow for the kernel its whole sequence runs on");
@@ -505,9 +533,10 @@
   a.xcd_remap = x3_xcd_remap();
   p.grid = dim3((unsigned)G, 1, 1);
   p.lds = lds;
-  if (AM == 2 && AN == 4) p.launch = select_x3q_r<2, 4>(a, R, mode);
-  else if (AM == 1 && AN == 4) p.launch = select_x3q_r<1, 4>(a, R, mode);
-  else p.launch = select_x3q_r<2, 2>(a, R, mode);
+  p.claim = claim; p.tiles = ntiles;
+  if (AM == 2 && AN == 4) p.launch = select_x3q_r<2, 4>(a, R, mode, claim);
+  else if (AM == 1 && AN == 4) p.launch = select_x3q_r<1, 4>(a, R, mode, claim);
+  else p.launch = select_x3q_r<2, 2>(a, R, mode, claim);
   return true;
 }
 
diff --git a/comfy-rvc_amd/csrc/model_synth.hip b/comfy-rvc_amd/csrc/model_synth.hip
--- a/comfy-rvc_amd/csrc/model_synth.hip
+++ b/comfy-rvc_amd/csrc/model_synth.hip
@@ -81,6 +81,7 @@
   int upp = 1;
   int spec_channels = 0, segment = 0;
   bool keep_params = false;
+  DevBuf<unsigned> claim_buf; ClaimRing claim;
   DevVec wgrad_part;
   bool f0 = true;
 };
@@ -480,6 +481,10 @@
                      int h2, float* out, const SynthTaps* taps) {
   const int IC = S->inter;
   const bool dry = A.dry;
+  if (!dry) {
+    if (!S->claim_buf.p) { S->claim_buf.alloc(ClaimRing::kBytes / sizeof(unsigned)); S->claim.buf = S->claim_buf.p; }
+    S->claim.begin(s);
+  }
   auto plan_tin = [&](int tin_full) { return W != T ? tin_full : 0; };
   const long long Nw = (long long)W * S->upp;
   const float* har_w = har ? har + (size_t)g0 * S->upp : nullptr;
@@ -552,8 +557,9 @@
             if (gp.split_pair[j][m]) {
               E1.ys_out = t1s; E1.ys_tp = split_image_tp(Tn); E1.ys_slope = E2.pre_slope;
               E1.h2 = gp.h2_pair[j][m] ? 1 : 0;
+              E1.claim_ring = &S->claim;
               conv1d_run(st.rb[j].c1[m], s, in, Tn, Tn, nullptr, Tn, E1);
-              ConvEpilogue E2s = E2; E2s.pre_act = ACT_NONE; E2s.xs_in = t1s; E2s.xs_tp = E1.ys_tp; E2s.h2 = E1.h2;
+              ConvEpilogue E2s = E2; E2s.claim_ring = &S->claim; E2s.pre_act = ACT_NONE; E2s.xs_in = t1s; E2s.xs_tp = E1.ys_tp; E2s.h2 = E1.h2;
               conv1d_run(st.rb[j].c2[m], s, nullptr, Tn, Tn, dst, Tn, E2s);
             } else {
               conv1d_run(st.rb[j].c1[m], s, in, Tn, Tn, t1, Tn, E1);
diff --git a/comfy-rvc_amd/csrc/rvc_api.hip b/comfy-rvc_amd/csrc/rvc_api.hip
--- a/comfy-rvc_amd/csrc/rvc_api.hip
+++ b/comfy-rvc_amd/csrc/rvc_api.hip
@@ -1470,6 +1470,16 @@
     ConvPlan p;
     return conv_x3_pair_plan(c1->L, c2->L, nullptr, T, T, T, nullptr, T, e, h2, p) && p.a.h2 ? 1 : 0;
   } catch (...) { return -1; }
+}
+int rvc_conv1d_plan_pair_split_tiles(rvc_conv1d_plan* c1, rvc_conv1d_plan* c2, int T, int64_t* out8) {
+  RVC_TRY
+  RVC_REQUIRE(c1 && c2 && out8, "null argument");
+  const int h2 = conv1d_pair_h2_eligible(c1->L, c2->L, T, conv_set_pair_arithmetic(-1)) ? 1 : 0;
+  long long o[8];
+  RVC_REQUIRE(conv1d_split_tiles(c1->L, T, SPLIT_PRODUCER, h2, o) && conv1d_split_tiles(c2->L, T, SPLIT_CONSUMER, h2, o + 4),
+              "this pair at this length does not run on the persistent kernel");
+  for (int i = 0; i < 8; ++i) out8[i] = o[i];
+  RVC_CATCH
 }
 int rvc_conv1d_plan_destroy(rvc_conv1d_plan* p) { delete p; return 0; }
 int rvc_op_attention(void* stream, const float* q, const float* k, const float* v_rm, const float* bv, float* out, int heads, int T) {
diff --git a/comfy-rvc_amd/csrc/rvc_internal.h b/comfy-rvc_amd/csrc/rvc_internal.h
--- a/comfy-rvc_amd/csrc/rvc_internal.h
+++ b/comfy-rvc_amd/csrc/rvc_internal.h
@@ -87,6 +87,7 @@
   int seg2_chunks = 0;
 };
 
+struct ClaimRing;
 struct ConvEpilogue {
   const float* R = nullptr; long long ldR = 0;
   int pre_act = ACT_NONE; float pre_slope = 0.f;
@@ -102,12 +103,14 @@
   int gate_h = 0; const float* gate_g = nullptr;
   int ys_deint_h = 0;
   int h2 = 0;
+  ClaimRing* claim_ring = nullptr;
 };
 constexpr int kSplitMargin = 64;
 inline long long split_image_tp(long long T) { return (T + kSplitMargin + 704 + 63) & ~63LL; }
 inline size_t split_image_bytes(int C, long long T) { return (size_t)(C / 16) * 2 * (size_t)split_image_tp(T) * 32; }
 enum SplitRole : int { SPLIT_CONSUMER = 0, SPLIT_PRODUCER = 1 };
 bool conv1d_split_eligible(const ConvLayer& L, int Tin, SplitRole role = SPLIT_CONSUMER, int h2 = 0);
+bool conv1d_split_tiles(const ConvLayer& L, int Tin, SplitRole role, int h2, long long out[4]);
 bool conv1d_pair_h2_eligible(const ConvLayer& c1, const ConvLayer& c2, int Tin, int h2);
 int conv1d_residual_period(const ConvLayer& L, int Tin, int h2);
 int conv_set_pair_arithmetic(int mode);
@@ -263,6 +266,15 @@
 void* stream_scratch_zeroed(hipStream_t s, int slot, size_t bytes, bool* fresh = nullptr);
 void stream_scratch_release(int device);
 
+struct ClaimRing {
+  static constexpr int kLaunches = 64, kXcds = 8;
+  static constexpr size_t kBytes = (size_t)kLaunches * kXcds * sizeof(unsigned);
+  unsigned* buf = nullptr; int next = 0;
+  void begin(hipStream_t s);
+  unsigned* take(hipStream_t s);
+};
+unsigned* stream_claim_take(hipStream_t s);
+
 template <typename T> struct DevBuf {
   T* p = nullptr; size_t n = 0;
   DevBuf() = default;
diff --git a/include/rvc_hip.h b/include/rvc_hip.h
--- a/include/rvc_hip.h
+++ b/include/rvc_hip.h
@@ -317,6 +317,7 @@
 int rvc_conv1d_plan_resblock_run(rvc_conv1d_plan* const* plans6, void* stream, const float* x_dev, int T, float* y_dev, float out_scale, int accumulate,
                                  int* ran_out, const float* noise_src_dev, const float* noise_w_dev, const float* noise_b_dev);
 int rvc_conv1d_plan_pair_arithmetic(rvc_conv1d_plan* c1, rvc_conv1d_plan* c2, int T);
+int rvc_conv1d_plan_pair_split_tiles(rvc_conv1d_plan* c1, rvc_conv1d_plan* c2, int T, int64_t* out8);
 int rvc_conv1d_plan_destroy(rvc_conv1d_plan* p);
 int rvc_op_attention(void* stream, const float* q_dev, const float* k_dev, const float* v_rm_dev, const float* bv_dev, float* out_dev,
                      int heads, int T);
```
